# 12334zq/optical-flow-1

Measured on AMD Instinct MI355X. Metric: Mpix*warp-iters/s, TV-L1 1920x1080 5-scale, higher is better.
Workload: dtype f64; 1 GPU; tvl1flow 1920x1080 pair (synthetic P1), nscales=5 warps=5 tau=0.25 lambda=0.15 theta=0.3 zfactor=0.5 epsilon=0.01; one pair per step per GPU; workload_name=1080p, arithmetic_mode=tolerance, pairs_per_gpu=1040, pairs_in_flight_per_gpu=64, lockstep_group=16, streams_per_gpu=4, distinct_pairs=8

## Files before the change

include/ofx.h:

```cpp
#ifndef OFX_H
#define OFX_H

#include <stddef.h>

#ifdef __cplusplus
extern "C" {
#endif

#define OFX_VERSION 102

#define OFX_OK          0
#define OFX_ERR_ARG     1
#define OFX_ERR_SIGMA   2
#define OFX_ERR_NOMEM   3
#define OFX_ERR_HIP     4
#define OFX_ERR_NODEV   5

#define OFX_F64 0
#define OFX_F32 1

#define OFX_TVL1_MAX_ITERATIONS 300
#define OFX_BROX_MAX_ITERATIONS 300
#define OFX_HS_MAX_MAXITER 65536
#define OFX_MAX_SCALES 32
#define OFX_MAX_SOLVES 64

typedef struct ofx_ctx ofx_ctx;

typedef struct ofx_stats {
    int    nscales;
    int    nsolves;
    int    nx[OFX_MAX_SCALES], ny[OFX_MAX_SCALES];
    int    iters[OFX_MAX_SCALES][OFX_MAX_SOLVES];
    double error[OFX_MAX_SCALES][OFX_MAX_SOLVES];
    double iter_ms[OFX_MAX_SCALES];
    long long iter_launches[OFX_MAX_SCALES];
    double work_pix_iters;
    double total_ms;
    int    odd_stops;
    int    odd_stops_stored;
    int    fused[OFX_MAX_SCALES];
    double pyramid_ms;
} ofx_stats;

int  ofx_device_count(void);
int  ofx_ctx_create(ofx_ctx **out, int device, int precision);
void ofx_ctx_destroy(ofx_ctx *ctx);
const char *ofx_strerror(int status);
const char *ofx_last_error(const ofx_ctx *ctx);
void *ofx_ctx_stream(const ofx_ctx *ctx);
int   ofx_ctx_precision(const ofx_ctx *ctx);
int   ofx_ctx_synchronize(ofx_ctx *ctx);
int   ofx_set_option(ofx_ctx *ctx, const char *name, double value);
int   ofx_get_stats(const ofx_ctx *ctx, ofx_stats *out);

int ofx_divergence(ofx_ctx *ctx, const double *v1, const double *v2, double *div, int nx, int ny);
int ofx_forward_gradient(ofx_ctx *ctx, const double *f, double *fx, double *fy, int nx, int ny);
int ofx_centered_gradient(ofx_ctx *ctx, const double *f, double *dx, double *dy, int nx, int ny);
int ofx_dxx(ofx_ctx *ctx, const double *I, double *Ixx, int nx, int ny);
int ofx_dyy(ofx_ctx *ctx, const double *I, double *Iyy, int nx, int ny);
int ofx_dxy(ofx_ctx *ctx, const double *I, double *Ixy, int nx, int ny);
int ofx_gaussian(ofx_ctx *ctx, double *I, int nx, int ny, double sigma);

int ofx_centered_gradient3(ofx_ctx *ctx, const double *f, double *dx, double *dy, double *dz, int nx, int ny, int nz);

int ofx_bicubic_at(ofx_ctx *ctx, const double *input, const double *uu, const double *vv, double *out,
                   int n, int nx, int ny, int border_out);
int ofx_bicubic_warp(ofx_ctx *ctx, const double *input, const double *u, const double *v, double *output,
                     int nx, int ny, int border_out);
int ofx_bicubic_at_color(ofx_ctx *ctx, const double *input, const double *uu, const double *vv, double *out,
                         int n, int nx, int ny, int nz, int k, int border_out);

void ofx_zoom_size(int nx, int ny, int *nxx, int *nyy, double factor);
int  ofx_zoom_out(ofx_ctx *ctx, const double *I, double *Iout, int nx, int ny, double factor);
int  ofx_zoom_in(ofx_ctx *ctx, const double *I, double *Iout, int nx, int ny, int nxx, int nyy);
int  ofx_zoom_out_color(ofx_ctx *ctx, const double *I, double *Iout, int nx, int ny, int nz, double factor);
int  ofx_zoom_out_channels(ofx_ctx *ctx, const double *I, double *Iout, int nx, int ny, int nz, double factor);

int ofx_image_normalization_2(ofx_ctx *ctx, const double *I1, const double *I2, double *I1n, double *I2n,
                              int size);
int ofx_image_normalization_1(ofx_ctx *ctx, const double *I, double *In, int size);
int ofx_getminmax(ofx_ctx *ctx, const double *x, int n, double *min, double *max);

int ofx_tvl1_single_scale(ofx_ctx *ctx, const double *I0, const double *I1, double *u1, double *u2,
                          int nx, int ny, double tau, double lambda, double theta, int warps,
                          double epsilon, int verbose);
int ofx_tvl1_multiscale(ofx_ctx *ctx, const double *I0, const double *I1, double *u1, double *u2,
                        int nx, int ny, double tau, double lambda, double theta, int nscales,
                        double zfactor, int warps, double epsilon, int verbose);

int ofx_tvl1_multiscale_dev(ofx_ctx *ctx, const void *dI0, const void *dI1, void *d_flo,
                            int nx, int ny, double tau, double lambda, double theta, int nscales,
                            double zfactor, int warps, double epsilon, int verbose);

int ofx_tvl1_group_dev(ofx_ctx *ctx, int n_pairs, const void *const *dI0, const void *const *dI1,
                       void *const *d_flo, int nx, int ny, double tau, double lambda, double theta,
                       int nscales, double zfactor, int warps, double epsilon, ofx_stats *stats_out);

int ofx_tvl1_batch_dev(ofx_ctx *const *ctxs, int n_ctx, const void *const *dI0, const void *const *dI1,
                       void *const *d_flo, int n_pairs, int nx, int ny, double tau, double lambda,
                       double theta, int nscales, double zfactor, int warps, double epsilon,
                       double *work_pix_iters);

int ofx_tvl1_batch_group_size(ofx_ctx *const *ctxs, int n_ctx, int n_pairs, int nx, int ny, int nscales,
                              double zfactor);

int ofx_tvl1_iterations(ofx_ctx *ctx, double *u1, double *u2, double *p11, double *p12, double *p21,
                        double *p22, const double *I1wx, const double *I1wy, const double *rho_c,
                        int nx, int ny, double tau, double lambda, double theta, int n_iter,
                        double *error);

int ofx_hypot(ofx_ctx *ctx, const double *x, const double *y, double *out, int n);

int ofx_staging_route(int ctx_device, int mem_device, int can_access_peer);

int ofx_hs_single_scale(ofx_ctx *ctx, const double *I1, const double *I2, double *u, double *v,
                        int nx, int ny, double alpha, int warps, double TOL, int maxiter, int verbose);
int ofx_hs_pyramidal(ofx_ctx *ctx, const double *I1, const double *I2, double *u, double *v,
                     int nx, int ny, double alpha, int nscales, double zfactor, int warps,
                     double TOL, int maxiter, int verbose);

int ofx_hs_group_dev(ofx_ctx *ctx, int n_pairs, const void *const *dI1, const void *const *dI2, void *const *d_flo,
                     int nx, int ny, double alpha, int nscales, double zfactor, int warps, double TOL, int maxiter,
                     ofx_stats *stats_out);
int ofx_hs_batch_dev(ofx_ctx *const *ctxs, int n_ctx, const void *const *dI1, const void *const *dI2,
                     void *const *d_flo, int n_pairs, int nx, int ny, double alpha, int nscales, double zfactor,
                     int warps, double TOL, int maxiter, double *work_pix_iters);

int ofx_hs_classic(ofx_ctx *ctx, const double *a, const double *b, double *u, double *v, int w, int h, int niter,
                   double alpha);

int ofx_brox_spatial(ofx_ctx *ctx, const double *I1, const double *I2, double *u, double *v,
                     int nxx, int nyy, double alpha, double gamma, int nscales, double nu,
                     double TOL, int inner_iter, int outer_iter, int verbose);

int ofx_brox_group_dev(ofx_ctx *ctx, int n_pairs, const void *const *dI1, const void *const *dI2, void *const *d_flo,
                       int nxx, int nyy, double alpha, double gamma, int nscales, double nu, double TOL,
                       int inner_iter, int outer_iter, ofx_stats *stats_out);
int ofx_brox_batch_dev(ofx_ctx *const *ctxs, int n_ctx, const void *const *dI1, const void *const *dI2,
                       void *const *d_flo, int n_pairs, int nxx, int nyy, double alpha, double gamma, int nscales,
                       double nu, double TOL, int inner_iter, int outer_iter, double *work_pix_iters);

#define OFX_REXPO_MAX_CHANNELS 4
int ofx_robust_expo(ofx_ctx *ctx, const double *I1, const double *I2, double *u, double *v, int nxx, int nyy, int nzz,
                    int method_type, double alpha, double gamma, double lambda, int nscales, double nu, double TOL,
                    int inner_iter, int outer_iter, int verbose);
int ofx_robust_expo_pyramid(ofx_ctx *ctx, const double *I1, const double *I2, double *u, double *v, int nxx, int nyy, int nzz,
                            int method_type, double alpha, double gamma, double lambda, int nscales, double nu, double TOL,
                            int inner_iter, int outer_iter, int verbose);
int ofx_robust_expo_group_dev(ofx_ctx *ctx, int n_pairs, const void *const *dI1, const void *const *dI2, void *const *d_flo,
                              int nxx, int nyy, int nzz, int method_type, double alpha, double gamma, double lambda,
                              int nscales, double nu, double TOL, int inner_iter, int outer_iter, ofx_stats *stats_out);
int ofx_robust_expo_batch_dev(ofx_ctx *const *ctxs, int n_ctx, const void *const *dI1, const void *const *dI2,
                              void *const *d_flo, int n_pairs, int nxx, int nyy, int nzz, int method_type, double alpha,
                              double gamma, double lambda, int nscales, double nu, double TOL, int inner_iter, int outer_iter,
                              double *work_pix_iters);
double ofx_ctx_expo_host_ms(const ofx_ctx *ctx);
int ofx_robust_expo_single_scale(ofx_ctx *ctx, const double *I1, const double *I2, double *u, double *v, int nx, int ny, int nz,
                                 int method_type, double alpha, double gamma, double lambda, double TOL, int inner_iter,
                                 int outer_iter, int number_of_threads, int verbose);

int ofx_brox_temporal(ofx_ctx *ctx, const double *I, double *u, double *v, int nxx, int nyy, int frames,
                      double alpha, double gamma, int nscales, double nu, double TOL, int inner_iter,
                      int outer_iter, int verbose);

#define OFX_BROXT_MAX_FRAMES 32
int ofx_brox_temporal_dev(ofx_ctx *ctx, int frames, const void *const *dF, void *const *d_flo, int nxx, int nyy, double alpha,
                          double gamma, int nscales, double nu, double TOL, int inner_iter, int outer_iter);

int ofx_brox_temporal_batch_dev(ofx_ctx *const *ctxs, int n_ctx, int n_seq, int frames, const void *const *dF,
                                void *const *d_flo, int nxx, int nyy, double alpha, double gamma, int nscales, double nu,
                                double TOL, int inner_iter, int outer_iter, double *work_pix_iters);

int ofx_bicubic_warp_color(ofx_ctx *ctx, const double *input, const double *u, const double *v, double *output,
                           int nx, int ny, int nz, int border_out);
int ofx_image_normalization_2_color(ofx_ctx *ctx, const double *I1, const double *I2, double *I1n, double *I2n,
                                    int size, int nz);
int ofx_image_normalization_3(ofx_ctx *ctx, double *I0, double *I1, double *I2, int size);
int ofx_image_normalization_4(ofx_ctx *ctx, const double *I_1, const double *I0, const double *I1, const double *filtI0,
                              double *I_1n, double *I0n, double *I1n, double *filtI0n, int size);

int ofx_me_median_filtering(ofx_ctx *ctx, double *in, int nx, int ny, int wsize);
int ofx_solver_wrt_v(ofx_ctx *ctx, const double *u1, const double *u2, double *v1, double *v2, const double *chi,
                     const double *I1wx, const double *I1wy, const double *I_1wx, const double *I_1wy,
                     const double *rho1_c, const double *rho3_c, double *Vfwd_1, double *Vfwd_2, double *Vbck_1,
                     double *Vbck_2, const double *grad1, const double *grad3, double alpha, double theta, double lambda,
                     int nx, int ny);
int ofx_scalar_rof_box_cell_centered(ofx_ctx *ctx, double *u, const double *f, double *initialP1, double *initialP2,
                                     const double *g_function, double lambda, double omega, int nx, int ny, int nIter);
int ofx_solver_wrt_u(ofx_ctx *ctx, double *u1, double *u2, const double *v1, const double *v2, const double *chi,
                     const double *g, double theta, double beta, int nx, int ny, double *p11, double *p12, double *p21,
                     double *p22, int n_iter);
int ofx_solver_wrt_chi(ofx_ctx *ctx, const double *u1, const double *u2, double *chi, const double *I1wx,
                       const double *I1wy, const double *I_1wx, const double *I_1wy, const double *rho1_c,
                       const double *rho3_c, const double *Vfwd_1, const double *Vfwd_2, const double *Vbck_1,
                       const double *Vbck_2, const double *g, double lambda, double theta, double alpha, double beta,
                       double tau_chi, double tau_eta, int nx, int ny, double *eta1, double *eta2, int n_iter);

int ofx_tvl1occ_multiscale(ofx_ctx *ctx, const double *I_1, const double *I0, const double *I1, const double *filtI0, double *u1,
                           double *u2, double *chi, int nxx, int nyy, double lambda, double alpha, double beta, double theta,
                           int nscales, double zfactor, int warps, double epsilon, int verbose);
int ofx_tvl1occ_batch(ofx_ctx *const *ctxs, int n_ctx, int n_triples, const double *const *I_1, const double *const *I0,
                      const double *const *I1, const double *const *filtI0, double *const *u1, double *const *u2,
                      double *const *chi, int nxx, int nyy, double lambda, double alpha, double beta, double theta, int nscales,
                      double zfactor, int warps, double epsilon);

int ofx_tvl1occ_sequence_group_dev(ofx_ctx *ctx, int n_frames, const void *const *dF, void *const *d_flo,
                                   void *const *d_occ, int nxx, int nyy, double lambda, double alpha, double beta,
                                   double theta, int nscales, double zfactor, int warps, double epsilon,
                                   ofx_stats *stats_out);
int ofx_tvl1occ_sequence_dev(ofx_ctx *const *ctxs, int n_ctx, int n_frames, const void *const *dF, void *const *d_flo,
                             void *const *d_occ, int nxx, int nyy, double lambda, double alpha, double beta, double theta,
                             int nscales, double zfactor, int warps, double epsilon, double *work_pix_iters);

#ifdef __cplusplus
}
#endif
#endif
```

optical-flow-1_amd/__init__.py:

```python
import ctypes as C
import os
import subprocess

import numpy as np

HERE = os.path.dirname(os.path.abspath(__file__))
LIB_PATH = os.environ.get("OFX_LIB_PATH") or os.path.join(HERE, "libofx.so")

F64, F32 = 0, 1
MAX_SCALES, MAX_SOLVES = 32, 64

_STATUS = {1: "invalid argument", 2: "GaussianSmooth: sigma too large", 3: "out of memory",
           4: "HIP runtime error", 5: "no usable gfx950 device"}


class OfxError(RuntimeError):
    def __init__(self, status, detail=""):
        self.status = status
        super().__init__("ofx status %d (%s)%s" % (status, _STATUS.get(status, "?"), ": " + detail if detail else ""))


class Stats(C.Structure):
    _fields_ = [("nscales", C.c_int), ("nsolves", C.c_int),
                ("nx", C.c_int * MAX_SCALES), ("ny", C.c_int * MAX_SCALES),
                ("iters", (C.c_int * MAX_SOLVES) * MAX_SCALES),
                ("error", (C.c_double * MAX_SOLVES) * MAX_SCALES),
                ("iter_ms", C.c_double * MAX_SCALES),
                ("iter_launches", C.c_longlong * MAX_SCALES),
                ("work_pix_iters", C.c_double), ("total_ms", C.c_double),
                ("odd_stops", C.c_int), ("odd_stops_stored", C.c_int), ("fused", C.c_int * MAX_SCALES),
                ("pyramid_ms", C.c_double)]

    def iterations(self):
        return np.array([[self.iters[s][w] for w in range(min(self.nsolves, MAX_SOLVES))]
                         for s in range(self.nscales)])

    def errors(self):
        return np.array([[self.error[s][w] for w in range(min(self.nsolves, MAX_SOLVES))]
                         for s in range(self.nscales)])


def build(verbose=False):
    out = subprocess.run(["make", "-C", os.path.join(HERE, "csrc"), "-j4"], capture_output=True, text=True)
    if verbose or out.returncode:
        print(out.stdout, out.stderr)
    if out.returncode:
        raise RuntimeError("libofx.so build failed")


_lib = None
_dp = np.ctypeslib.ndpointer(dtype=np.float64, flags="C_CONTIGUOUS")
_vp = C.c_void_p
_i, _d = C.c_int, C.c_double


def lib():
    global _lib
    if _lib is not None:
        return _lib
    if not os.path.exists(LIB_PATH):
        raise FileNotFoundError("%s not built -- run `python -c 'import __graft_entry__ as g; g.build()'`" % LIB_PATH)
    L = C.CDLL(LIB_PATH)
    sig = {
        "ofx_device_count": (_i, []),
        "ofx_ctx_create": (_i, [C.POINTER(_vp), _i, _i]),
        "ofx_ctx_destroy": (None, [_vp]),
        "ofx_strerror": (C.c_char_p, [_i]),
        "ofx_last_error": (C.c_char_p, [_vp]),
        "ofx_ctx_stream": (_vp, [_vp]),
        "ofx_ctx_precision": (_i, [_vp]),
        "ofx_ctx_synchronize": (_i, [_vp]),
        "ofx_set_option": (_i, [_vp, C.c_char_p, _d]),
        "ofx_get_stats": (_i, [_vp, C.POINTER(Stats)]),
        "ofx_divergence": (_i, [_vp, _dp, _dp, _dp, _i, _i]),
        "ofx_forward_gradient": (_i, [_vp, _dp, _dp, _dp, _i, _i]),
        "ofx_centered_gradient": (_i, [_vp, _dp, _dp, _dp, _i, _i]),
        "ofx_dxx": (_i, [_vp, _dp, _dp, _i, _i]),
        "ofx_dyy": (_i, [_vp, _dp, _dp, _i, _i]),
        "ofx_dxy": (_i, [_vp, _dp, _dp, _i, _i]),
        "ofx_gaussian": (_i, [_vp, _dp, _i, _i, _d]),
        "ofx_bicubic_at": (_i, [_vp, _dp, _dp, _dp, _dp, _i, _i, _i, _i]),
        "ofx_hypot": (_i, [_vp, _dp, _dp, _dp, _i]),
        "ofx_robust_expo": (_i, [_vp, _dp, _dp, _dp, _dp, _i, _i, _i, _i, _d, _d, _d, _i, _d, _d, _i, _i, _i]),
        "ofx_robust_expo_single_scale": (_i, [_vp, _dp, _dp, _dp, _dp, _i, _i, _i, _i, _d, _d, _d, _d, _i, _i, _i, _i]),
        "ofx_robust_expo_pyramid": (_i, [_vp, _dp, _dp, _dp, _dp, _i, _i, _i, _i, _d, _d, _d, _i, _d, _d, _i, _i, _i]),
        "ofx_bicubic_warp": (_i, [_vp, _dp, _dp, _dp, _dp, _i, _i, _i]),
        "ofx_zoom_size": (None, [_i, _i, C.POINTER(_i), C.POINTER(_i), _d]),
        "ofx_zoom_out": (_i, [_vp, _dp, _dp, _i, _i, _d]),
        "ofx_zoom_in": (_i, [_vp, _dp, _dp, _i, _i, _i, _i]),
        "ofx_image_normalization_2": (_i, [_vp, _dp, _dp, _dp, _dp, _i]),
        "ofx_image_normalization_1": (_i, [_vp, _dp, _dp, _i]),
        "ofx_getminmax": (_i, [_vp, _dp, _i, C.POINTER(_d), C.POINTER(_d)]),
        "ofx_centered_gradient3": (_i, [_vp, _dp, _dp, _dp, _dp, _i, _i, _i]),
        "ofx_bicubic_at_color": (_i, [_vp, _dp, _dp, _dp, _dp, _i, _i, _i, _i, _i, _i]),
        "ofx_zoom_out_color": (_i, [_vp, _dp, _dp, _i, _i, _i, _d]),
        "ofx_zoom_out_channels": (_i, [_vp, _dp, _dp, _i, _i, _i, _d]),
        "ofx_tvl1_single_scale": (_i, [_vp, _dp, _dp, _dp, _dp, _i, _i, _d, _d, _d, _i, _d, _i]),
        "ofx_tvl1_multiscale": (_i, [_vp, _dp, _dp, _dp, _dp, _i, _i, _d, _d, _d, _i, _d, _i, _d, _i]),
        "ofx_tvl1_multiscale_dev": (_i, [_vp, _vp, _vp, _vp, _i, _i, _d, _d, _d, _i, _d, _i, _d, _i]),
        "ofx_tvl1_group_dev": (_i, [_vp, _i, C.POINTER(_vp), C.POINTER(_vp), C.POINTER(_vp), _i, _i, _d, _d, _d, _i, _d, _i, _d,
                                    C.POINTER(Stats)]),
        "ofx_tvl1_batch_dev": (_i, [C.POINTER(_vp), _i, C.POINTER(_vp), C.POINTER(_vp), C.POINTER(_vp), _i, _i, _i, _d, _d, _d,
                                    _i, _d, _i, _d, C.POINTER(_d)]),
        "ofx_tvl1_batch_group_size": (_i, [C.POINTER(_vp), _i, _i, _i, _i, _i, _d]),
        "ofx_tvl1_iterations": (_i, [_vp] + [_dp] * 9 + [_i, _i, _d, _d, _d, _i, C.POINTER(_d)]),
        "ofx_hs_single_scale": (_i, [_vp, _dp, _dp, _dp, _dp, _i, _i, _d, _i, _d, _i, _i]),
        "ofx_hs_pyramidal": (_i, [_vp, _dp, _dp, _dp, _dp, _i, _i, _d, _i, _d, _i, _d, _i, _i]),
        "ofx_brox_spatial": (_i, [_vp, _dp, _dp, _dp, _dp, _i, _i, _d, _d, _i, _d, _d, _i, _i, _i]),
        "ofx_hs_group_dev": (_i, [_vp, _i, C.POINTER(_vp), C.POINTER(_vp), C.POINTER(_vp), _i, _i, _d, _i, _d, _i, _d, _i,
                                  C.POINTER(Stats)]),
        "ofx_hs_batch_dev": (_i, [C.POINTER(_vp), _i, C.POINTER(_vp), C.POINTER(_vp), C.POINTER(_vp), _i, _i, _i, _d, _i, _d,
                                  _i, _d, _i, C.POINTER(_d)]),
        "ofx_brox_group_dev": (_i, [_vp, _i, C.POINTER(_vp), C.POINTER(_vp), C.POINTER(_vp), _i, _i, _d, _d, _i, _d, _d, _i,
                                    _i, C.POINTER(Stats)]),
        "ofx_brox_batch_dev": (_i, [C.POINTER(_vp), _i, C.POINTER(_vp), C.POINTER(_vp), C.POINTER(_vp), _i, _i, _i, _d, _d, _i,
                                    _d, _d, _i, _i, C.POINTER(_d)]),
        "ofx_robust_expo_group_dev": (_i, [_vp, _i, C.POINTER(_vp), C.POINTER(_vp), C.POINTER(_vp), _i, _i, _i, _i, _d, _d, _d, _i,
                                           _d, _d, _i, _i, C.POINTER(Stats)]),
        "ofx_robust_expo_batch_dev": (_i, [C.POINTER(_vp), _i, C.POINTER(_vp), C.POINTER(_vp), C.POINTER(_vp), _i, _i, _i, _i, _i,
                                           _d, _d, _d, _i, _d, _d, _i, _i, C.POINTER(_d)]),
        "ofx_ctx_expo_host_ms": (_d, [_vp]),
        "ofx_bicubic_warp_color": (_i, [_vp, _dp, _dp, _dp, _dp, _i, _i, _i, _i]),
        "ofx_image_normalization_2_color": (_i, [_vp, _dp, _dp, _dp, _dp, _i, _i]),
        "ofx_image_normalization_3": (_i, [_vp, _dp, _dp, _dp, _i]),
        "ofx_image_normalization_4": (_i, [_vp] + [_dp] * 8 + [_i]),
        "ofx_me_median_filtering": (_i, [_vp, _dp, _i, _i, _i]),
        "ofx_solver_wrt_v": (_i, [_vp] + [_dp] * 17 + [_d, _d, _d, _i, _i]),
        "ofx_scalar_rof_box_cell_centered": (_i, [_vp, _dp, _dp, _dp, _dp, _dp, _d, _d, _i, _i, _i]),
        "ofx_solver_wrt_u": (_i, [_vp] + [_dp] * 6 + [_d, _d, _i, _i] + [_dp] * 4 + [_i]),
        "ofx_solver_wrt_chi": (_i, [_vp] + [_dp] * 14 + [_d] * 6 + [_i, _i, _dp, _dp, _i]),
        "ofx_tvl1occ_multiscale": (_i, [_vp] + [_dp] * 7 + [_i, _i, _d, _d, _d, _d, _i, _d, _i, _d, _i]),
        "ofx_tvl1occ_batch": (_i, [_vp, _i, _i] + [_vp] * 7 + [_i, _i, _d, _d, _d, _d, _i, _d, _i, _d]),
        "ofx_tvl1occ_sequence_group_dev": (_i, [_vp, _i, C.POINTER(_vp), C.POINTER(_vp), C.POINTER(_vp), _i, _i, _d, _d, _d, _d, _i, _d,
                                                _i, _d, C.POINTER(Stats)]),
        "ofx_tvl1occ_sequence_dev": (_i, [C.POINTER(_vp), _i, _i, C.POINTER(_vp), C.POINTER(_vp), C.POINTER(_vp), _i, _i, _d, _d, _d,
                                          _d, _i, _d, _i, _d, C.POINTER(_d)]),
        "ofx_hs_classic": (_i, [_vp, _dp, _dp, _dp, _dp, _i, _i, _i, _d]),
        "ofx_brox_temporal": (_i, [_vp, _dp, _dp, _dp, _i, _i, _i, _d, _d, _i, _d, _d, _i, _i, _i]),
        "ofx_brox_temporal_dev": (_i, [_vp, _i, C.POINTER(_vp), C.POINTER(_vp), _i, _i, _d, _d, _i, _d, _d, _i, _i]),
        "ofx_brox_temporal_batch_dev": (_i, [C.POINTER(_vp), _i, _i, _i, C.POINTER(_vp), C.POINTER(_vp), _i, _i, _d, _d, _i, _d, _d,
                                             _i, _i, C.POINTER(_d)]),
    }
    L.ofx_missing = []
    for name, (res, args) in sig.items():
        if not hasattr(L, name):
            L.ofx_missing.append(name)
            continue
        f = getattr(L, name)
        f.restype = res
        f.argtypes = args
    _lib = L
    return L


def zoom_size(nx, ny, factor):
    a, b = _i(), _i()
    lib().ofx_zoom_size(nx, ny, C.byref(a), C.byref(b), factor)
    return a.value, b.value


def _f64(a):
    return np.ascontiguousarray(a, dtype=np.float64)


def tvl1_batch_dev(ctxs, dI0, dI1, d_flo, nx, ny, tau=0.25, lam=0.15, theta=0.3, nscales=5, zfactor=0.5, warps=5,
                   epsilon=0.01):
    n = len(dI0)
    arr = lambda xs: (_vp * len(xs))(*xs)
    work = (_d * max(n, 1))()
    s = lib().ofx_tvl1_batch_dev(arr([c.h.value for c in ctxs]), len(ctxs), arr(dI0), arr(dI1), arr(d_flo), n, nx, ny, tau,
                                 lam, theta, nscales, zfactor, warps, epsilon, work)
    if s:
        raise OfxError(s, "; ".join((c.L.ofx_last_error(c.h) or b"").decode() for c in ctxs))
    return [work[i] for i in range(n)]


def _batch_call(fn, ctxs, dA, dB, d_flo, *args):
    n = len(dA)
    arr = lambda xs: (_vp * max(len(xs), 1))(*xs)
    work = (_d * max(n, 1))()
    s = fn(arr([c.h.value for c in ctxs]), len(ctxs), arr(dA), arr(dB), arr(d_flo), n, *args, work)
    if s:
        raise OfxError(s, "; ".join((c.L.ofx_last_error(c.h) or b"").decode() for c in ctxs))
    return [work[i] for i in range(n)]


def hs_batch_dev(ctxs, dI1, dI2, d_flo, nx, ny, alpha=7.0, nscales=10, zfactor=0.5, warps=10, TOL=1e-4, maxiter=150):
    return _batch_call(lib().ofx_hs_batch_dev, ctxs, dI1, dI2, d_flo, nx, ny, alpha, nscales, zfactor, warps, TOL, maxiter)


def brox_batch_dev(ctxs, dI1, dI2, d_flo, nx, ny, alpha=50.0, gamma=10.0, nscales=10, nu=0.5, TOL=1e-4, inner=1, outer=15):
    return _batch_call(lib().ofx_brox_batch_dev, ctxs, dI1, dI2, d_flo, nx, ny, alpha, gamma, nscales, nu, TOL, inner, outer)


def robust_expo_batch_dev(ctxs, dI1, dI2, d_flo, nx, ny, nz, method=1, alpha=50.0, gamma=10.0, lam=1.0, nscales=5, nu=0.5, TOL=1e-4,
                          inner=1, outer=15):
    return _batch_call(lib().ofx_robust_expo_batch_dev, ctxs, dI1, dI2, d_flo, nx, ny, nz, method, alpha, gamma, lam, nscales, nu,
                       TOL, inner, outer)


def tvl1occ_batch(ctxs, triples, lam=0.15, alpha=0.01, beta=0.15, theta=0.3, nscales=3, zfactor=0.5, warps=2, epsilon=0.01, out=None):
    n = len(triples)
    ny, nx = triples[0][1].shape
    ins = [[_f64(t[k] if k < len(t) else t[1]) for t in triples] for k in range(4)]
    outs = [[o[k] for o in out] for k in range(3)] if out is not None else [[np.empty((ny, nx)) for _ in range(n)] for _ in range(3)]
    ptr = lambda arrs: (_vp * n)(*[a.ctypes.data for a in arrs])
    s = lib().ofx_tvl1occ_batch((_vp * len(ctxs))(*[c.h.value for c in ctxs]), len(ctxs), n, *[ptr(a) for a in ins],
                                *[ptr(a) for a in outs], nx, ny, lam, alpha, beta, theta, nscales, zfactor, warps, epsilon)
    if s:
        raise OfxError(s, "; ".join((c.L.ofx_last_error(c.h) or b"").decode() for c in ctxs))
    return list(zip(*outs))


def tvl1occ_sequence_dev(ctxs, dF, d_flo, d_occ, nx, ny, lam=0.15, alpha=0.01, beta=0.15, theta=0.3, nscales=3, zfactor=0.5, warps=2,
                         epsilon=0.01):
    n = len(dF)
    arr = lambda xs: (_vp * max(len(xs), 1))(*xs)
    work = (_d * max(n - 2, 1))()
    s = lib().ofx_tvl1occ_sequence_dev(arr([c.h.value for c in ctxs]), len(ctxs), n, arr(dF), arr(d_flo), arr(d_occ), nx, ny, lam,
                                       alpha, beta, theta, nscales, zfactor, warps, epsilon, work)
    if s:
        raise OfxError(s, "; ".join((c.L.ofx_last_error(c.h) or b"").decode() for c in ctxs))
    return [work[i] for i in range(max(n - 2, 0))]


def brox_temporal_batch_dev(ctxs, dF, d_flo, nx, ny, frames, alpha=18.0, gamma=7.0, nscales=10, nu=0.75, TOL=1e-4, inner=1, outer=15):
    n_seq = len(dF) // frames if frames > 0 else 0
    arr = lambda xs: (_vp * max(len(xs), 1))(*xs)
    work = (_d * max(n_seq, 1))()
    s = lib().ofx_brox_temporal_batch_dev(arr([c.h.value for c in ctxs]), len(ctxs), n_seq, frames, arr(dF), arr(d_flo), nx, ny,
                                          alpha, gamma, nscales, nu, TOL, inner, outer, work)
    if s:
        raise OfxError(s, "; ".join((c.L.ofx_last_error(c.h) or b"").decode() for c in ctxs))
    return [work[i] for i in range(n_seq)]


def tvl1_batch_group_size(ctxs, n_pairs, nx, ny, nscales=5, zfactor=0.5):
    g = lib().ofx_tvl1_batch_group_size((_vp * len(ctxs))(*[c.h.value for c in ctxs]), len(ctxs), n_pairs, nx, ny, nscales,
                                        zfactor)
    if g < 1:
        raise OfxError(g, "; ".join((c.L.ofx_last_error(c.h) or b"").decode() for c in ctxs))
    return g


class Ofx:

    def __init__(self, device=0, precision=F64):
        self.L = lib()
        h = _vp()
        s = self.L.ofx_ctx_create(C.byref(h), device, precision)
        if s:
            raise OfxError(s, "ofx_ctx_create(device=%d)" % device)
        self.h = h
        self.precision = precision

    def close(self):
        if getattr(self, "h", None):
            self.L.ofx_ctx_destroy(self.h)
            self.h = None

    def __del__(self):
        try:
            self.close()
        except Exception:
            pass

    def _ck(self, s):
        if s:
            raise OfxError(s, (self.L.ofx_last_error(self.h) or b"").decode())

    def set_option(self, name, value):
        self._ck(self.L.ofx_set_option(self.h, name.encode(), float(value)))

    def stats(self):
        st = Stats()
        self._ck(self.L.ofx_get_stats(self.h, C.byref(st)))
        return st

    def stream(self):
        return self.L.ofx_ctx_stream(self.h)

    def synchronize(self):
        self._ck(self.L.ofx_ctx_synchronize(self.h))

    def divergence(self, v1, v2):
        ny, nx = v1.shape
        out = np.empty((ny, nx))
        self._ck(self.L.ofx_divergence(self.h, _f64(v1), _f64(v2), out, nx, ny))
        return out

    def forward_gradient(self, f):
        ny, nx = f.shape
        fx, fy = np.empty((ny, nx)), np.empty((ny, nx))
        self._ck(self.L.ofx_forward_gradient(self.h, _f64(f), fx, fy, nx, ny))
        return fx, fy

    def centered_gradient(self, f):
        ny, nx = f.shape
        fx, fy = np.empty((ny, nx)), np.empty((ny, nx))
        self._ck(self.L.ofx_centered_gradient(self.h, _f64(f), fx, fy, nx, ny))
        return fx, fy

    def _second(self, fn, f):
        ny, nx = f.shape
        out = np.empty((ny, nx))
        self._ck(fn(self.h, _f64(f), out, nx, ny))
        return out

    def dxx(self, f): return self._second(self.L.ofx_dxx, f)
    def dyy(self, f): return self._second(self.L.ofx_dyy, f)
    def dxy(self, f): return self._second(self.L.ofx_dxy, f)

    def gaussian(self, I, sigma):
        ny, nx = I.shape
        out = _f64(I).copy()
        self._ck(self.L.ofx_gaussian(self.h, out, nx, ny, sigma))
        return out

    def bicubic_at(self, I, uu, vv, border_out=False):
        ny, nx = I.shape
        uu, vv = _f64(np.atleast_1d(uu)), _f64(np.atleast_1d(vv))
        out = np.empty(uu.shape)
        self._ck(self.L.ofx_bicubic_at(self.h, _f64(I), uu, vv, out, uu.size, nx, ny, int(border_out)))
        return out

    @staticmethod
    def _colour_shape(I1, I2, nz):
        if I1.shape != I2.shape or I1.ndim not in (2, 3):
            raise ValueError("robust_expo: images of shape %s and %s" % (I1.shape, I2.shape))
        if I1.ndim == 3:
            if nz is not None and nz != I1.shape[2]:
                raise ValueError("robust_expo: nz = %d for images of shape %s" % (nz, I1.shape))
            return I1.shape
        return I1.shape[0], I1.shape[1], (1 if nz is None else nz)

    def robust_expo(self, I1, I2, method=1, alpha=50.0, gamma=10.0, lam=1.0, nscales=5, nu=0.5, TOL=1e-4, inner=1, outer=15,
                    verbose=0, nz=None):
        ny, nx, nz = self._colour_shape(I1, I2, nz)
        if I1.ndim == 2 and nz > 1 and nscales == 1:
            raise ValueError("robust_expo: nz = %d needs (ny, nx, nz) images" % nz)
        u, v = np.zeros((ny, nx)), np.zeros((ny, nx))
        self._ck(self.L.ofx_robust_expo(self.h, _f64(I1), _f64(I2), u, v, nx, ny, nz, method, alpha, gamma, lam, nscales, nu, TOL,
                                        inner, outer, verbose))
        return u, v

    def robust_expo_pyramid(self, I1, I2, method=1, alpha=50.0, gamma=10.0, lam=1.0, nscales=5, nu=0.5, TOL=1e-4, inner=1, outer=15,
                            verbose=0, nz=None):
        ny, nx, nz = self._colour_shape(I1, I2, nz)
        if I1.ndim == 2 and nz != 1:
            raise ValueError("robust_expo_pyramid: nz = %d needs (ny, nx, nz) images" % nz)
        u, v = np.zeros((ny, nx)), np.zeros((ny, nx))
        self._ck(self.L.ofx_robust_expo_pyramid(self.h, _f64(I1), _f64(I2), u, v, nx, ny, nz, method, alpha, gamma, lam, nscales, nu,
                                                TOL, inner, outer, verbose))
        return u, v

    def robust_expo_single_scale(self, I1, I2, u, v, method=1, alpha=50.0, gamma=10.0, lam=1.0, TOL=1e-4, inner=1, outer=15,
                                 verbose=0, nz=None):
        ny, nx, nz = self._colour_shape(I1, I2, nz)
        if I1.ndim == 2 and nz != 1:
            raise ValueError("robust_expo_single_scale: nz = %d needs (ny, nx, nz) images" % nz)
        u, v = np.array(u, dtype=np.float64, order="C"), np.array(v, dtype=np.float64, order="C")
        if u.shape != (ny, nx) or v.shape != (ny, nx):
            raise ValueError("robust_expo_single_scale: flow of shape %s, %s for %dx%d images" % (u.shape, v.shape, nx, ny))
        self._ck(self.L.ofx_robust_expo_single_scale(self.h, _f64(I1), _f64(I2), u, v, nx, ny, nz, method, alpha, gamma, lam, TOL,
                                                     inner, outer, 1, verbose))
        return u, v

    def hypot(self, x, y):
        x, y = _f64(np.atleast_1d(x)).ravel(), _f64(np.atleast_1d(y)).ravel()
        out = np.empty(x.shape)
        self._ck(self.L.ofx_hypot(self.h, x, y, out, x.size))
        return out

    def bicubic_warp(self, I, u, v, border_out=False):
        ny, nx = I.shape
        out = np.empty((ny, nx))
        self._ck(self.L.ofx_bicubic_warp(self.h, _f64(I), _f64(u), _f64(v), out, nx, ny, int(border_out)))
        return out

    def zoom_out(self, I, factor):
        ny, nx = I.shape
        nxx, nyy = zoom_size(nx, ny, factor)
        out = np.empty((nyy, nxx))
        self._ck(self.L.ofx_zoom_out(self.h, _f64(I), out, nx, ny, factor))
        return out

    def zoom_in(self, I, nxx, nyy):
        ny, nx = I.shape
        out = np.empty((nyy, nxx))
        self._ck(self.L.ofx_zoom_in(self.h, _f64(I), out, nx, ny, nxx, nyy))
        return out

    def image_normalization_2(self, I1, I2):
        a, b = np.empty(I1.shape), np.empty(I2.shape)
        self._ck(self.L.ofx_image_normalization_2(self.h, _f64(I1), _f64(I2), a, b, I1.size))
        return a, b

    def tvl1_single_scale(self, I0, I1, u1, u2, tau=0.25, lam=0.15, theta=0.3, warps=5, epsilon=0.01, verbose=0):
        ny, nx = I0.shape
        u1, u2 = _f64(u1).copy(), _f64(u2).copy()
        self._ck(self.L.ofx_tvl1_single_scale(self.h, _f64(I0), _f64(I1), u1, u2, nx, ny, tau, lam, theta, warps,
                                              epsilon, verbose))
        return u1, u2

    def tvl1_multiscale(self, I0, I1, tau=0.25, lam=0.15, theta=0.3, nscales=5, zfactor=0.5, warps=5, epsilon=0.01,
                        verbose=0, out=None):
        ny, nx = I0.shape
        u1, u2 = out if out is not None else (np.zeros((ny, nx)), np.zeros((ny, nx)))
        self._ck(self.L.ofx_tvl1_multiscale(self.h, _f64(I0), _f64(I1), u1, u2, nx, ny, tau, lam, theta, nscales,
                                            zfactor, warps, epsilon, verbose))
        return u1, u2

    def tvl1_multiscale_dev(self, dI0, dI1, d_flo, nx, ny, tau=0.25, lam=0.15, theta=0.3, nscales=5, zfactor=0.5,
                            warps=5, epsilon=0.01, verbose=0):
        self._ck(self.L.ofx_tvl1_multiscale_dev(self.h, dI0, dI1, d_flo, nx, ny, tau, lam, theta, nscales, zfactor,
                                                warps, epsilon, verbose))

    def tvl1_group_dev(self, dI0, dI1, d_flo, nx, ny, tau=0.25, lam=0.15, theta=0.3, nscales=5, zfactor=0.5, warps=5,
                       epsilon=0.01):
        n = len(dI0)
        arr = lambda xs: (_vp * len(xs))(*xs)
        st = (Stats * max(n, 1))()
        self._ck(self.L.ofx_tvl1_group_dev(self.h, n, arr(dI0), arr(dI1), arr(d_flo), nx, ny, tau, lam, theta, nscales,
                                           zfactor, warps, epsilon, st))
        return [st[i] for i in range(n)]

    def _group_call(self, fn, dA, dB, d_flo, *args):
        n = len(dA)
        arr = lambda xs: (_vp * max(len(xs), 1))(*xs)
        st = (Stats * max(n, 1))()
        self._ck(fn(self.h, n, arr(dA), arr(dB), arr(d_flo), *args, st))
        return [st[i] for i in range(n)]

    def hs_group_dev(self, dI1, dI2, d_flo, nx, ny, alpha=7.0, nscales=10, zfactor=0.5, warps=10, TOL=1e-4, maxiter=150):
        return self._group_call(self.L.ofx_hs_group_dev, dI1, dI2, d_flo, nx, ny, alpha, nscales, zfactor, warps, TOL, maxiter)

    def brox_group_dev(self, dI1, dI2, d_flo, nx, ny, alpha=50.0, gamma=10.0, nscales=10, nu=0.5, TOL=1e-4, inner=1, outer=15):
        return self._group_call(self.L.ofx_brox_group_dev, dI1, dI2, d_flo, nx, ny, alpha, gamma, nscales, nu, TOL, inner, outer)

    def robust_expo_group_dev(self, dI1, dI2, d_flo, nx, ny, nz, method=1, alpha=50.0, gamma=10.0, lam=1.0, nscales=5, nu=0.5,
                              TOL=1e-4, inner=1, outer=15):
        return self._group_call(self.L.ofx_robust_expo_group_dev, dI1, dI2, d_flo, nx, ny, nz, method, alpha, gamma, lam, nscales,
                                nu, TOL, inner, outer)

    def expo_host_ms(self):
        return self.L.ofx_ctx_expo_host_ms(self.h)

    def tvl1_iterations(self, u1, u2, p11, p12, p21, p22, I1wx, I1wy, rho_c, tau, lam, theta, n_iter):
        ny, nx = u1.shape
        err = _d()
        self._ck(self.L.ofx_tvl1_iterations(self.h, u1, u2, p11, p12, p21, p22, _f64(I1wx), _f64(I1wy), _f64(rho_c),
                                            nx, ny, tau, lam, theta, n_iter, C.byref(err)))
        return err.value

    def hs_single_scale(self, I1, I2, u, v, alpha=7.0, warps=10, TOL=1e-4, maxiter=150, verbose=0):
        ny, nx = I1.shape
        u, v = _f64(u).copy(), _f64(v).copy()
        self._ck(self.L.ofx_hs_single_scale(self.h, _f64(I1), _f64(I2), u, v, nx, ny, alpha, warps, TOL, maxiter, verbose))
        return u, v

    def hs_pyramidal(self, I1, I2, alpha=7.0, nscales=10, zfactor=0.5, warps=10, TOL=1e-4, maxiter=150, verbose=0, out=None):
        ny, nx = I1.shape
        u, v = out if out is not None else (np.zeros((ny, nx)), np.zeros((ny, nx)))
        self._ck(self.L.ofx_hs_pyramidal(self.h, _f64(I1), _f64(I2), u, v, nx, ny, alpha, nscales, zfactor, warps, TOL,
                                         maxiter, verbose))
        return u, v

    def brox_spatial(self, I1, I2, alpha=50.0, gamma=10.0, nscales=10, nu=0.5, TOL=1e-4, inner=1, outer=15, verbose=0, out=None):
        ny, nx = I1.shape
        u, v = out if out is not None else (np.zeros((ny, nx)), np.zeros((ny, nx)))
        self._ck(self.L.ofx_brox_spatial(self.h, _f64(I1), _f64(I2), u, v, nx, ny, alpha, gamma, nscales, nu, TOL,
                                         inner, outer, verbose))
        return u, v

    def brox_temporal(self, I, alpha=18.0, gamma=7.0, nscales=10, nu=0.75, TOL=1e-4, inner=1, outer=15, verbose=0):
        frames, ny, nx = I.shape
        u, v = np.zeros((max(frames - 1, 0), ny, nx)), np.zeros((max(frames - 1, 0), ny, nx))
        self._ck(self.L.ofx_brox_temporal(self.h, _f64(I), u, v, nx, ny, frames, alpha, gamma, nscales, nu, TOL, inner,
                                          outer, verbose))
        return u, v

    def brox_temporal_dev(self, dF, d_flo, nx, ny, alpha=18.0, gamma=7.0, nscales=10, nu=0.75, TOL=1e-4, inner=1, outer=15):
        arr = lambda xs: (_vp * max(len(xs), 1))(*xs)
        self._ck(self.L.ofx_brox_temporal_dev(self.h, len(dF), arr(dF), arr(d_flo), nx, ny, alpha, gamma, nscales, nu, TOL, inner,
                                              outer))

    def centered_gradient3(self, f):
        nz, ny, nx = f.shape
        dx, dy, dz = np.empty((nz, ny, nx)), np.empty((nz, ny, nx)), np.empty((nz, ny, nx))
        self._ck(self.L.ofx_centered_gradient3(self.h, _f64(f), dx, dy, dz, nx, ny, nz))
        return dx, dy, dz

    def bicubic_at_color(self, I, uu, vv, k, border_out=False):
        ny, nx, nz = I.shape
        uu, vv = _f64(np.atleast_1d(uu)), _f64(np.atleast_1d(vv))
        out = np.empty(uu.shape)
        self._ck(self.L.ofx_bicubic_at_color(self.h, _f64(I), uu, vv, out, uu.size, nx, ny, nz, k, int(border_out)))
        return out

    def zoom_out_color(self, I, factor):
        ny, nx, nz = I.shape
        nxx, nyy = zoom_size(nx, ny, factor)
        out = np.empty((nyy, nxx, nz))
        self._ck(self.L.ofx_zoom_out_color(self.h, _f64(I), out, nx, ny, nz, factor))
        return out

    def zoom_out_channels(self, I, factor):
        ny, nx, nz = I.shape
        nxx, nyy = zoom_size(nx, ny, factor)
        out = np.empty((nyy, nxx, nz))
        self._ck(self.L.ofx_zoom_out_channels(self.h, _f64(I), out, nx, ny, nz, factor))
        return out

    def image_normalization_1(self, I):
        out = np.empty(I.shape)
        self._ck(self.L.ofx_image_normalization_1(self.h, _f64(I), out, I.size))
        return out

    def getminmax(self, x):
        a, b = _d(), _d()
        self._ck(self.L.ofx_getminmax(self.h, _f64(x), x.size, C.byref(a), C.byref(b)))
        return a.value, b.value

    def hs_classic(self, a, b, niter, alpha):
        h, w = a.shape
        u, v = np.zeros((h, w)), np.zeros((h, w))
        self._ck(self.L.ofx_hs_classic(self.h, _f64(a), _f64(b), u, v, w, h, niter, alpha))
        return u, v

    def bicubic_warp_color(self, I, u, v, border_out=False):
        ny, nx, nz = I.shape
        out = np.empty((ny, nx, nz))
        self._ck(self.L.ofx_bicubic_warp_color(self.h, _f64(I), _f64(u), _f64(v), out, nx, ny, nz, int(border_out)))
        return out

    def image_normalization_2_color(self, I1, I2, size=None):
        nz = I1.shape[-1]
        a, b = _f64(I1).copy(), _f64(I2).copy()
        self._ck(self.L.ofx_image_normalization_2_color(self.h, _f64(I1), _f64(I2), a, b, I1.size if size is None else size, nz))
        return a, b

    def image_normalization_3(self, I0, I1, I2):
        a, b, c = _f64(I0).copy(), _f64(I1).copy(), _f64(I2).copy()
        self._ck(self.L.ofx_image_normalization_3(self.h, a, b, c, a.size))
        return a, b, c

    def image_normalization_4(self, I_1, I0, I1, F):
        outs = [np.empty(I0.shape) for _ in range(4)]
        self._ck(self.L.ofx_image_normalization_4(self.h, _f64(I_1), _f64(I0), _f64(I1), _f64(F), *outs, I0.size))
        return outs

    def median_filtering(self, I, wsize=3):
        ny, nx = I.shape
        out = _f64(I).copy()
        self._ck(self.L.ofx_me_median_filtering(self.h, out, nx, ny, wsize))
        return out

    def occ_solver_v(self, u1, u2, chi, I1wx, I1wy, I_1wx, I_1wy, rho1_c, rho3_c, grad1, grad3, alpha, theta, lam):
        ny, nx = u1.shape
        v1, v2, f1, f2, b1, b2 = outs = [np.empty((ny, nx)) for _ in range(6)]
        self._ck(self.L.ofx_solver_wrt_v(self.h, _f64(u1), _f64(u2), v1, v2, _f64(chi), _f64(I1wx), _f64(I1wy), _f64(I_1wx),
                                         _f64(I_1wy), _f64(rho1_c), _f64(rho3_c), f1, f2, b1, b2, _f64(grad1), _f64(grad3),
                                         alpha, theta, lam, nx, ny))
        return outs

    def occ_solver_chi(self, u1, u2, chi, I1wx, I1wy, I_1wx, I_1wy, rho1_c, rho3_c, Vf1, Vf2, Vb1, Vb2, g, lam, theta, alpha,
                       beta, tau_chi, tau_eta, eta1=None, eta2=None, n_iter=100):
        ny, nx = u1.shape
        chi = _f64(chi).copy()
        eta1 = np.zeros((ny, nx)) if eta1 is None else _f64(eta1).copy()
        eta2 = np.zeros((ny, nx)) if eta2 is None else _f64(eta2).copy()
        self._ck(self.L.ofx_solver_wrt_chi(self.h, _f64(u1), _f64(u2), chi, _f64(I1wx), _f64(I1wy), _f64(I_1wx), _f64(I_1wy),
                                           _f64(rho1_c), _f64(rho3_c), _f64(Vf1), _f64(Vf2), _f64(Vb1), _f64(Vb2), _f64(g), lam,
                                           theta, alpha, beta, tau_chi, tau_eta, nx, ny, eta1, eta2, n_iter))
        return chi, eta1, eta2

    def rof_box(self, u, f, P1, P2, g, lam, omega, n_iter):
        ny, nx = u.shape
        u, P1, P2 = _f64(u).copy(), _f64(P1).copy(), _f64(P2).copy()
        self._ck(self.L.ofx_scalar_rof_box_cell_centered(self.h, u, _f64(f), P1, P2, _f64(g), lam, omega, nx, ny, n_iter))
        return u, P1, P2

    def tvl1occ_multiscale(self, I_1, I0, I1, filtI0=None, lam=0.15, alpha=0.01, beta=0.15, theta=0.3, nscales=3, zfactor=0.5,
                           warps=2, epsilon=0.01, verbose=0, out=None):
        ny, nx = I0.shape
        filtI0 = I0 if filtI0 is None else filtI0
        u1, u2, chi = out if out is not None else (np.empty((ny, nx)), np.empty((ny, nx)), np.empty((ny, nx)))
        self._ck(self.L.ofx_tvl1occ_multiscale(self.h, _f64(I_1), _f64(I0), _f64(I1), _f64(filtI0), u1, u2, chi, nx, ny, lam, alpha,
                                               beta, theta, nscales, zfactor, warps, epsilon, verbose))
        return u1, u2, chi

    def tvl1occ_sequence_group_dev(self, dF, d_flo, d_occ, nx, ny, lam=0.15, alpha=0.01, beta=0.15, theta=0.3, nscales=3, zfactor=0.5,
                                   warps=2, epsilon=0.01):
        n = len(dF)
        arr = lambda xs: (_vp * max(len(xs), 1))(*xs)
        st = (Stats * max(n - 2, 1))()
        self._ck(self.L.ofx_tvl1occ_sequence_group_dev(self.h, n, arr(dF), arr(d_flo), arr(d_occ), nx, ny, lam, alpha, beta, theta,
                                                       nscales, zfactor, warps, epsilon, st))
        return [st[i] for i in range(max(n - 2, 0))]

    def occ_solver_u(self, v1, v2, chi, g, theta, beta, p=None, n_iter=10):
        ny, nx = v1.shape
        u1, u2 = np.empty((ny, nx)), np.empty((ny, nx))
        p = [np.zeros((ny, nx)) for _ in range(4)] if p is None else [_f64(a).copy() for a in p]
        self._ck(self.L.ofx_solver_wrt_u(self.h, u1, u2, _f64(v1), _f64(v2), _f64(chi), _f64(g), theta, beta, nx, ny, *p, n_iter))
        return u1, u2, p
```

optical-flow-1_amd/csrc/ofx_ctx.cpp:

```cpp
#include "ofx_internal.h"

#include <cstdarg>
#include <cstdlib>
#include <new>

static const size_t kSlabAlign = 256;
static const size_t kMinSlab = 32u << 20;
static const size_t kMaxSlabs = 24;

int ofx_fail(ofx_ctx *ctx, int status, const char *fmt, ...)
{
    if (ctx) {
        va_list ap;
        va_start(ap, fmt);
        vsnprintf(ctx->errmsg, sizeof(ctx->errmsg), fmt, ap);
        va_end(ap);
    }
    return status;
}

extern "C" const char *ofx_strerror(int status)
{
    switch (status) {
    case OFX_OK:        return "ok";
    case OFX_ERR_ARG:   return "invalid argument";
    case OFX_ERR_SIGMA: return "GaussianSmooth: sigma too large";
    case OFX_ERR_NOMEM: return "out of memory";
    case OFX_ERR_HIP:   return "HIP runtime error";
    case OFX_ERR_NODEV: return "no usable gfx950 device";
    default:            return "unknown status";
    }
}

extern "C" const char *ofx_last_error(const ofx_ctx *ctx) { return ctx ? ctx->errmsg : ""; }

extern "C" int ofx_device_count(void)
{
    int n = 0;
    if (hipGetDeviceCount(&n) != hipSuccess) return 0;
    return n;
}

extern "C" void ofx_ctx_destroy(ofx_ctx *ctx);

extern "C" int ofx_ctx_create(ofx_ctx **out, int device, int precision)
{
    if (!out) return OFX_ERR_ARG;
    *out = nullptr;
    if (precision != OFX_F64 && precision != OFX_F32) return OFX_ERR_ARG;
    const bool trace = getenv("OFX_TRACE_INIT") != nullptr;
    double t_prev = ofx_now_ms();
    auto mark = [&](const char *what) {
        if (!trace) return;
        const double t = ofx_now_ms();
        fprintf(stderr, "ofx_ctx_create: %-28s %8.2f ms\n", what, t - t_prev);
        t_prev = t;
    };
    int n = 0;
    if (hipGetDeviceCount(&n) != hipSuccess || n <= 0 || device < 0 || device >= n) return OFX_ERR_NODEV;
    mark("hipGetDeviceCount (runtime)");
    if (hipSetDevice(device) != hipSuccess) return OFX_ERR_NODEV;
    mark("hipSetDevice");

    ofx_ctx *ctx = new (std::nothrow) ofx_ctx();
    if (!ctx) return OFX_ERR_NOMEM;
    ctx->device = device;
    ctx->precision = precision;
    ctx->cur_slab = 0;
    ctx->cur_used = 0;
    ctx->call_bytes = 0;
    ctx->profile = 0;
    ctx->rows_per_wave = 0;
    ctx->rows_per_wave2 = 0;
    ctx->fuse2 = 1;
    ctx->store_a = 1;
    ctx->concurrency = 1;
    ctx->lockstep = 0;
    ctx->warp_lds = 1;
    ctx->gauss_fused = 1;
    ctx->relaxed_dual = 0;
    ctx->tile = 0;
    ctx->tile_max_px = 0;
    ctx->nt_stores = 0;
    ctx->chunk = 0;
    ctx->spin_us = 150;
    ctx->rows_slots = 0;
    ctx->rof_pipe = 1;
    ctx->rof_window = 0;
    ctx->chi_fuse = 1;
    ctx->fuse3 = 2;
    ctx->fuse3_min_px = 0.0;
    ctx->fuse3_cursor = 1;
    ctx->fuse3_afac1 = 0;
    ctx->fuse3_afac2 = 0;
    ctx->rows_per_wave3 = 0;
    ctx->rows3_max = 32;
    ctx->fixed_work = 0;
    ctx->sor_exact = 1;
    ctx->sor_batch = 0;
    ctx->sor_fuse = 0;
    ctx->sor_tile = 0;
    ctx->sor_tile_w = 0;
    ctx->sor_wave_levels = 1;
    ctx->sor_wave_p = 0;
    ctx->sor_window = 0;
    ctx->sor_rows = 0;
    ctx->sor_spw = 0;
    ctx->sor_lds = 1;
    ctx->mem_budget = 0;
    ctx->poll_seq = 0;
    ctx->errmsg[0] = 0;
    ctx->expo_host_ms = 0.0;
    memset(&ctx->stats, 0, sizeof(ctx->stats));

    ctx->stream = nullptr;
    ctx->d_err = nullptr;
    ctx->d_state = nullptr;
    ctx->h_state = nullptr;
    ctx->h_aux = nullptr;
    ctx->ev_t0 = ctx->ev_t1 = nullptr;
    for (int i = 0; i < OFX_NPOLL; i++) ctx->ev_poll[i] = nullptr;
    bool ok = hipStreamCreateWithFlags(&ctx->stream, hipStreamNonBlocking) == hipSuccess;
    mark("hipStreamCreate");
    static_assert(sizeof(OfxLoopDev) <= OFX_STATE_BYTES && OFX_STATE_BYTES % 512 == 0, "state block too small");
    static_assert(OFX_ULOG >= OFX_TVL1_MAX_ITERATIONS + 16, "unit log too short");
    ok = ok && hipMalloc((void **) &ctx->d_state, OFX_STATE_BYTES + sizeof(double) * OFX_TVL1_MAX_ITERATIONS * OFX_NSHARD) == hipSuccess;
    if (ok) ctx->d_err = reinterpret_cast<double *>(reinterpret_cast<char *>(ctx->d_state) + OFX_STATE_BYTES);
    ctx->d_err_cap = OFX_TVL1_MAX_ITERATIONS;
    mark("hipMalloc (loop state)");
    ok = ok && hipHostMalloc((void **) &ctx->h_state, sizeof(OfxIterState) * OFX_NPOLL * OFX_MAX_GROUP + sizeof(double) * OFX_MAX_GROUP,
                             hipHostMallocDefault) == hipSuccess;
    if (ok) {
        memset(ctx->h_state, 0, sizeof(OfxIterState) * OFX_NPOLL * OFX_MAX_GROUP + sizeof(double) * OFX_MAX_GROUP);
        ctx->h_aux = reinterpret_cast<double *>(ctx->h_state + OFX_NPOLL * OFX_MAX_GROUP);
    }
    mark("hipHostMalloc (poll ring)");
    for (int i = 0; ok && i < OFX_NPOLL; i++)
        ok = hipEventCreateWithFlags(&ctx->ev_poll[i], hipEventDisableTiming) == hipSuccess;
    ok = ok && hipEventCreate(&ctx->ev_t0) == hipSuccess && hipEventCreate(&ctx->ev_t1) == hipSuccess;
    mark("hipEventCreate x 6");
    if (!ok) {
        (void) hipGetLastError();
        ofx_ctx_destroy(ctx);
        return OFX_ERR_HIP;
    }
    *out = ctx;
    return OFX_OK;
}

extern "C" void ofx_ctx_destroy(ofx_ctx *ctx)
{
    if (!ctx) return;
    (void) hipSetDevice(ctx->device);
    if (ctx->stream) (void) hipStreamSynchronize(ctx->stream);
    for (auto &s : ctx->slabs) (void) hipFree(s.base);
    if (ctx->d_state) (void) hipFree(ctx->d_state);
    if (ctx->h_state) (void) hipHostFree(ctx->h_state);
    for (int i = 0; i < OFX_NPOLL; i++)
        if (ctx->ev_poll[i]) (void) hipEventDestroy(ctx->ev_poll[i]);
    if (ctx->ev_t0) (void) hipEventDestroy(ctx->ev_t0);
    if (ctx->ev_t1) (void) hipEventDestroy(ctx->ev_t1);
    if (ctx->stream) (void) hipStreamDestroy(ctx->stream);
    (void) hipGetLastError();
    delete ctx;
}

extern "C" void *ofx_ctx_stream(const ofx_ctx *ctx) { return ctx ? (void *) ctx->stream : nullptr; }
extern "C" int ofx_ctx_precision(const ofx_ctx *ctx) { return ctx ? ctx->precision : -1; }

extern "C" int ofx_ctx_synchronize(ofx_ctx *ctx)
{
    if (!ctx) return OFX_ERR_ARG;
    OFX_HIP(ctx, hipStreamSynchronize(ctx->stream));
    return OFX_OK;
}

extern "C" int ofx_set_option(ofx_ctx *ctx, const char *name, double value)
{
    if (!ctx || !name) return OFX_ERR_ARG;
    if (!strcmp(name, "profile")) { ctx->profile = value != 0; return OFX_OK; }
    if (!strcmp(name, "fixed_work")) { ctx->fixed_work = value != 0; return OFX_OK; }
    if (!strcmp(name, "rows_per_wave")) {
        if (value < 0 || value > 4096) return ofx_fail(ctx, OFX_ERR_ARG, "rows_per_wave out of range");
        ctx->rows_per_wave = (int) value;
        return OFX_OK;
    }
    if (!strcmp(name, "rows_per_wave2")) {
        if (value < 0 || value > 4096) return ofx_fail(ctx, OFX_ERR_ARG, "rows_per_wave2 out of range");
        ctx->rows_per_wave2 = (int) value;
        return OFX_OK;
    }
    if (!strcmp(name, "concurrency")) {
        if (value < 1 || value > 64) return ofx_fail(ctx, OFX_ERR_ARG, "concurrency out of range");
        ctx->concurrency = (int) value;
        return OFX_OK;
    }
    if (!strcmp(name, "tile")) {
        if (value != 0 && value != 4 && value != 6) return ofx_fail(ctx, OFX_ERR_ARG, "tile must be 0, 4 or 6");
        ctx->tile = (int) value;
        return OFX_OK;
    }
    if (!strcmp(name, "tile_max_px")) {
        if (value < 0) return ofx_fail(ctx, OFX_ERR_ARG, "tile_max_px out of range");
        ctx->tile_max_px = value;
        return OFX_OK;
    }
    if (!strcmp(name, "relaxed_dual")) { ctx->relaxed_dual = value != 0; return OFX_OK; }
    if (!strcmp(name, "gauss_fused")) { ctx->gauss_fused = (value == 2 || value == 3) ? (int) value : (value != 0); return OFX_OK; }
    if (!strcmp(name, "warp_lds")) { ctx->warp_lds = value != 0; return OFX_OK; }
    if (!strcmp(name, "nt_stores")) { ctx->nt_stores = (int) value; return (value >= 0 && value <= 2) ? OFX_OK : ofx_fail(ctx, OFX_ERR_ARG, "nt_stores = 0 | 1 | 2"); }
    if (!strcmp(name, "lockstep")) {
        if (value < 0 || value > OFX_MAX_GROUP) return ofx_fail(ctx, OFX_ERR_ARG, "lockstep out of range");
        ctx->lockstep = (int) value;
        return OFX_OK;
    }
    if (!strcmp(name, "sor_exact")) {
        if (value != 0 && value != 1 && value != 2) return ofx_fail(ctx, OFX_ERR_ARG, "sor_exact must be 0, 1 or 2");
        ctx->sor_exact = (int) value;
        return OFX_OK;
    }
    if (!strcmp(name, "sor_fuse")) {
        if ((value < -1 || value > 4) && value != 9) return ofx_fail(ctx, OFX_ERR_ARG, "sor_fuse must be -1 .. 4 (or 9)");
        ctx->sor_fuse = (int) value;
        return OFX_OK;
    }
    if (!strcmp(name, "sor_tile")) {
        if (value < 0 || value > 3) return ofx_fail(ctx, OFX_ERR_ARG, "sor_tile must be 0 .. 3");
        ctx->sor_tile = (int) value;
        return OFX_OK;
    }
    if (!strcmp(name, "sor_tile_w")) {
        if (value < 0 || value > 65536) return ofx_fail(ctx, OFX_ERR_ARG, "sor_tile_w out of range");
        ctx->sor_tile_w = (int) value;
        return OFX_OK;
    }
    if (!strcmp(name, "sor_wave_p")) {
        if (value < 0 || value > 8) return ofx_fail(ctx, OFX_ERR_ARG, "sor_wave_p out of range");
        ctx->sor_wave_p = (int) value;
        return OFX_OK;
    }
    if (!strcmp(name, "sor_wave_levels")) {
        if (value < 0 || value > 64) return ofx_fail(ctx, OFX_ERR_ARG, "sor_wave_levels out of range");
        ctx->sor_wave_levels = (int) value;
        return OFX_OK;
    }
    if (!strcmp(name, "sor_rows")) {
        if (value < 0 || value > 4096) return ofx_fail(ctx, OFX_ERR_ARG, "sor_rows out of range");
        ctx->sor_rows = (int) value;
        return OFX_OK;
    }
    if (!strcmp(name, "sor_lds")) {
        if (value != 0 && value != 1 && value != 2) return ofx_fail(ctx, OFX_ERR_ARG, "sor_lds must be 0, 1 or 2");
        ctx->sor_lds = (int) value;
        return OFX_OK;
    }
    if (!strcmp(name, "sor_spw")) {
        if (value != 0 && value != 1 && value != 2 && value != 4) return ofx_fail(ctx, OFX_ERR_ARG, "sor_spw must be 0, 1, 2 or 4");
        ctx->sor_spw = (int) value;
        return OFX_OK;
    }
    if (!strcmp(name, "sor_window")) {
        if (value < 0 || value > 4096) return ofx_fail(ctx, OFX_ERR_ARG, "sor_window out of range");
        ctx->sor_window = (int) value;
        return OFX_OK;
    }
    if (!strcmp(name, "sor_batch")) {
        if (value < 0 || value > 4096) return ofx_fail(ctx, OFX_ERR_ARG, "sor_batch out of range");
        ctx->sor_batch = (int) value;
        return OFX_OK;
    }
    if (!strcmp(name, "mem_budget")) {
        if (value < 0) return ofx_fail(ctx, OFX_ERR_ARG, "mem_budget out of range");
        ctx->mem_budget = value;
        return OFX_OK;
    }
    if (!strcmp(name, "fuse2")) { ctx->fuse2 = value != 0; return OFX_OK; }
    if (!strcmp(name, "store_a")) {
        if (value != 0 && value != 1 && value != 2) return ofx_fail(ctx, OFX_ERR_ARG, "store_a must be 0, 1 or 2");
        ctx->store_a = (int) value;
        return OFX_OK;
    }
    if (!strcmp(name, "rows_slots")) { ctx->rows_slots = (int) value; return OFX_OK; }
    if (!strcmp(name, "rof_pipe")) { ctx->rof_pipe = value != 0; return OFX_OK; }
    if (!strcmp(name, "rof_window")) {
        if (value != 0 && value != 24 && value != 10) return ofx_fail(ctx, OFX_ERR_ARG, "rof_window must be 0, 10 or 24");
        ctx->rof_window = (int) value;
        return OFX_OK;
    }
    if (!strcmp(name, "chi_fuse")) { ctx->chi_fuse = value != 0; return OFX_OK; }
    if (!strcmp(name, "fuse3")) {
        if (value != 0 && value != 1 && value != 2) return ofx_fail(ctx, OFX_ERR_ARG, "fuse3 must be 0, 1 or 2");
        ctx->fuse3 = (int) value;
        return OFX_OK;
    }
    if (!strcmp(name, "fuse3_min_px")) { ctx->fuse3_min_px = value; return OFX_OK; }
    if (!strcmp(name, "fuse3_cursor")) { ctx->fuse3_cursor = value != 0; return OFX_OK; }
    if (!strcmp(name, "fuse3_afac1")) { ctx->fuse3_afac1 = value; return value >= 0 ? OFX_OK : ofx_fail(ctx, OFX_ERR_ARG, "fuse3_afac1 < 0"); }
    if (!strcmp(name, "fuse3_afac2")) { ctx->fuse3_afac2 = value; return value >= 0 ? OFX_OK : ofx_fail(ctx, OFX_ERR_ARG, "fuse3_afac2 < 0"); }
    if (!strcmp(name, "rows_per_wave3")) { ctx->rows_per_wave3 = (int) value; return OFX_OK; }
    if (!strcmp(name, "rows3_max")) { ctx->rows3_max = (int) value; return OFX_OK; }
    if (!strcmp(name, "spin_us")) {
        if (value < 0 || value > 1e6) return ofx_fail(ctx, OFX_ERR_ARG, "spin_us out of range");
        ctx->spin_us = (int) value;
        return OFX_OK;
    }
    if (!strcmp(name, "chunk")) {
        if (value < 0 || value > OFX_TVL1_MAX_ITERATIONS) return ofx_fail(ctx, OFX_ERR_ARG, "chunk out of range");
        ctx->chunk = (int) value;
        return OFX_OK;
    }
    return ofx_fail(ctx, OFX_ERR_ARG, "unknown option '%s'", name);
}

extern "C" int ofx_get_stats(const ofx_ctx *ctx, ofx_stats *out)
{
    if (!ctx || !out) return OFX_ERR_ARG;
    *out = ctx->stats;
    return OFX_OK;
}

void ofx_arena_reset(ofx_ctx *ctx)
{
    if (ctx->slabs.size() > kMaxSlabs) {
        size_t total = 0;
        for (auto &s : ctx->slabs) { total += s.bytes; (void) hipFree(s.base); }
        ctx->slabs.clear();
        char *p = nullptr;
        if (hipMalloc((void **) &p, total) == hipSuccess) ctx->slabs.push_back({p, total});
        else (void) hipGetLastError();
    }
    ctx->cur_slab = 0;
    ctx->cur_used = 0;
    ctx->call_bytes = 0;
}

int ofx_arena_alloc(ofx_ctx *ctx, size_t bytes, void **out)
{
    static const long skew = getenv("OFX_ARENA_SKEW") ? atol(getenv("OFX_ARENA_SKEW")) : 0;
    bytes += (size_t) skew;
    bytes = (bytes + kSlabAlign - 1) / kSlabAlign * kSlabAlign;
    if (bytes == 0) bytes = kSlabAlign;
    while (ctx->cur_slab < ctx->slabs.size()) {
        OfxSlab &s = ctx->slabs[ctx->cur_slab];
        if (ctx->cur_used + bytes <= s.bytes) {
            *out = s.base + ctx->cur_used;
            ctx->cur_used += bytes;
            ctx->call_bytes += bytes;
            return OFX_OK;
        }
        ctx->cur_slab++;
        ctx->cur_used = 0;
    }
    size_t want = bytes > kMinSlab ? bytes : kMinSlab;
    if (want < ctx->call_bytes) want = ctx->call_bytes;
    char *p = nullptr;
    hipError_t e = hipMalloc((void **) &p, want);
    if (e != hipSuccess) {
        (void) hipGetLastError();
        return ofx_fail(ctx, OFX_ERR_NOMEM, "hipMalloc(%zu) failed: %s", want, hipGetErrorString(e));
    }
    ctx->slabs.push_back({p, want});
    ctx->cur_slab = ctx->slabs.size() - 1;
    ctx->cur_used = bytes;
    ctx->call_bytes += bytes;
    *out = p;
    return OFX_OK;
}
```

optical-flow-1_amd/csrc/ofx_internal.h:

```cpp
#pragma once

#include <hip/hip_runtime.h>

#include <cstddef>
#include <cstdint>
#include <cstdio>
#include <cstring>
#include <chrono>
#include <vector>

#include "ofx.h"

#define OFX_NSHARD 64
#define OFX_NPOLL  4
#define OFX_MAX_GROUP 16

struct OfxIterState {
    int    n;
    int    done;
    double error;
    int    apred;
    int    seq;
    int    unit, k0, ucnt;
};

#define OFX_ULOG 320
struct OfxLoopDev {
    OfxIterState st[OFX_MAX_GROUP];
    int cursor[2][OFX_MAX_GROUP];
    int scanned[OFX_MAX_GROUP];
    int ulog[OFX_MAX_GROUP][OFX_ULOG];
};

#define OFX_STATE_BYTES 22016

struct OfxSlab {
    char  *base;
    size_t bytes;
};

struct ofx_ctx {
    int device;
    int precision;
    hipStream_t stream;

    std::vector<OfxSlab> slabs;
    size_t cur_slab;
    size_t cur_used;
    size_t call_bytes;

    double       *d_err;
    int           d_err_cap;
    OfxIterState *d_state;
    OfxIterState *h_state;
    double       *h_aux;
    hipEvent_t    ev_poll[OFX_NPOLL];
    hipEvent_t    ev_t0, ev_t1;

    int profile;
    int rows_per_wave;
    int rows_per_wave2;
    int fuse2;
    int store_a;
    int concurrency;
    int lockstep;
    int nt_stores;
    int relaxed_dual;
    int tile;
    double tile_max_px;
    int gauss_fused;
    int warp_lds;
    int chunk;
    int fuse3;
    double fuse3_min_px;
    int fuse3_cursor;
    double fuse3_afac1, fuse3_afac2;
    int rows_per_wave3;
    int rows3_max;
    int chi_fuse;
    int rof_window;
    int rof_pipe;
    int rows_slots;
    int spin_us;
    int fixed_work;
    int sor_exact;
    int sor_fuse;
    int sor_tile;
    int sor_tile_w;
    int sor_wave_p;
    int sor_wave_levels;
    int sor_batch;
    int sor_window;
    int sor_rows;
    int sor_lds;
    int sor_spw;
    double mem_budget;
    unsigned long long poll_seq;

    ofx_stats stats;
    double expo_host_ms;
    char errmsg[256];
};

int ofx_fail(ofx_ctx *ctx, int status, const char *fmt, ...);

#define OFX_HIP(ctx, call)                                                                       \
    do {                                                                                         \
        hipError_t e__ = (call);                                                                 \
        if (e__ != hipSuccess)                                                                   \
            return ofx_fail((ctx), e__ == hipErrorOutOfMemory ? OFX_ERR_NOMEM : OFX_ERR_HIP,     \
                            "%s failed: %s (%s:%d)", #call, hipGetErrorString(e__), __FILE__,   \
                            __LINE__);                                                           \
    } while (0)

#define OFX_TRY(expr)                                                                            \
    do {                                                                                         \
        int s__ = (expr);                                                                        \
        if (s__ != OFX_OK) return s__;                                                           \
    } while (0)

void ofx_arena_reset(ofx_ctx *ctx);
int  ofx_arena_alloc(ofx_ctx *ctx, size_t bytes, void **out);

template <typename T>
static inline int ofx_alloc(ofx_ctx *ctx, size_t count, T **out)
{
    void *p = nullptr;
    int s = ofx_arena_alloc(ctx, count * sizeof(T), &p);
    *out = static_cast<T *>(p);
    return s;
}

template <typename T> struct Pix;
template <> struct Pix<double> { using v2 = double2; using v4 = double4; };
template <> struct Pix<float>  { using v2 = float2;  using v4 = float4;  };

static inline int ofx_cdiv(int a, int b) { return (a + b - 1) / b; }

#define OFX_ENTER(ctx)                                                                           \
    do {                                                                                         \
        if (!(ctx)) return OFX_ERR_ARG;                                                          \
        if (hipSetDevice((ctx)->device) != hipSuccess)                                           \
            return ofx_fail((ctx), OFX_ERR_NODEV, "hipSetDevice(%d) failed", (ctx)->device);     \
        (ctx)->errmsg[0] = 0;                                                                    \
        (ctx)->expo_host_ms = 0.0;                                                               \
        ofx_arena_reset(ctx);                                                                    \
    } while (0)

static inline double ofx_now_ms()
{
    using namespace std::chrono;
    return duration<double, std::milli>(steady_clock::now().time_since_epoch()).count();
}
```

optical-flow-1_amd/csrc/ofx_tvl1.hip:

```cpp
#include "ofx_ops.h"
#include "ofx_device.h"
#include "ofx_loop.h"

#include <atomic>
#include <chrono>
#include <cmath>
#include <thread>

#define TVL1_GRAD_IS_ZERO 1E-10
#define TVL1_PRESMOOTHING_SIGMA 0.8
#define STRIP_OUT 62

template <typename T> OFX_DEV double rnd_to(double x);
template <> OFX_DEV double rnd_to<double>(double x) { return x; }
template <> OFX_DEV double rnd_to<float>(double x) { return (double) (float) x; }

#ifdef OFX_NO_RFL
#define OFX_WAVE_UNIFORM(x) (x)
#else
#define OFX_WAVE_UNIFORM(x) __builtin_amdgcn_readfirstlane(x)
#endif
template <typename T> struct RowIn {
    double2 u, p1, p2, a;
    double r;
};

template <typename V> OFX_DEV const V *at(const V *base, unsigned byte_off)
{
    return reinterpret_cast<const V *>(reinterpret_cast<const char *>(base) + byte_off);
}
template <typename V> OFX_DEV V *at(V *base, unsigned byte_off)
{
    return reinterpret_cast<V *>(reinterpret_cast<char *>(base) + byte_off);
}

template <typename T>
OFX_DEV RowIn<T> tvl1_load_row(const typename Pix<T>::v2 *U, const typename Pix<T>::v2 *P1,
                               const typename Pix<T>::v2 *P2, const typename Pix<T>::v2 *A, const T *R, unsigned off2)
{
    RowIn<T> r;
    r.u = ldw2(at(U, off2));
    r.p1 = ldw2(at(P1, off2));
    r.p2 = ldw2(at(P2, off2));
    r.a = ldw2(at(A, off2));
    r.r = ldw(at(R, off2 >> 1));
    return r;
}

#ifndef OFX_TOL_NEWTON
#define OFX_TOL_NEWTON 1
#endif
OFX_DEV double sqrt_tol(double x)
{
#if OFX_TOL_NEWTON >= 2
    return sqrt_unscaled(x);
#else
    const double y = __builtin_amdgcn_rsq(x);
    const double g = x * y;
    const double h = y * 0.5;
    const double r = __builtin_fma(-h, g, 0.5);
    return __builtin_fma(g, r, g);
#endif
}
OFX_DEV double rcp_tol(double d)
{
#if OFX_TOL_NEWTON >= 2
    return rcp_newton(d);
#else
    const double r = __builtin_amdgcn_rcp(d);
    const double e = __builtin_fma(-d, r, 1.0);
    return __builtin_fma(r, e, r);
#endif
}

template <typename T, bool STRICT = true>
OFX_DEV double2 tvl1_primal(double2 u, double2 a, double r, double2 p1, double2 p2, double l11, double l21, double up12,
                            double up22, bool lef, bool rig, bool top, bool bot, double l_t, double theta)
{
#ifdef OFX_CEIL_MEM
    return make_double2(u.x + 1e-300 * (a.x + r + p1.x + l11 + up12), u.y + 1e-300 * (a.y + p2.x + p1.y + p2.y + l21 + up22));
#endif
    const double div1 = div_backward(p1.x, l11, p1.y, up12, lef, rig, top, bot);
    const double div2 = div_backward(p2.x, l21, p2.y, up22, lef, rig, top, bot);
    const double ix = a.x, iy = a.y;
    const double grad = ix * ix + iy * iy;
    const double rho = r + (ix * u.x + iy * u.y);
    const double ltg = l_t * grad;
    const double fi = STRICT ? -rho / grad : -rho * rcp_tol(grad);
    double d1, d2;
    if (rho < -ltg)                     { d1 = l_t * ix;  d2 = l_t * iy; }
    else if (rho > ltg)                 { d1 = -l_t * ix; d2 = -l_t * iy; }
    else if (grad < TVL1_GRAD_IS_ZERO)  { d1 = 0.0;       d2 = 0.0; }
    else                                { d1 = fi * ix;   d2 = fi * iy; }
    const double v1 = u.x + d1, v2 = u.y + d2;
    return make_double2(rnd_to<T>(v1 + theta * div1), rnd_to<T>(v2 + theta * div2));
}

#ifdef OFX_DIV_SHARED
OFX_DEV double rcp_refined(double d)
{
    double r = __builtin_amdgcn_rcp(d);
    double e = __builtin_fma(-d, r, 1.0);
    r = __builtin_fma(r, e, r);
    e = __builtin_fma(-d, r, 1.0);
    r = __builtin_fma(r, e, r);
    return r;
}
OFX_DEV double div_by_rcp(double n, double d, double r)
{
    double q = n * r;
    const double rem = __builtin_fma(-d, q, n);
    q = __builtin_fma(rem, r, q);
    return __builtin_amdgcn_div_fixup(q, d, n);
}
#endif

template <typename T, bool STRICT>
OFX_DEV void tvl1_dual(double2 p1, double2 p2, double2 un, double r1, double r2, double2 dn, bool rig, bool lastrow,
                       double taut, double2 &q1, double2 &q2)
{
#ifdef OFX_CEIL_MEM
    q1 = make_double2(p1.x + 1e-300 * (un.x + r1), p1.y + 1e-300 * dn.x);
    q2 = make_double2(p2.x + 1e-300 * (un.y + r2), p2.y + 1e-300 * dn.y);
    return;
#endif
    const double u1x = rig ? 0.0 : r1 - un.x;
    const double u2x = rig ? 0.0 : r2 - un.y;
    const double u1y = lastrow ? 0.0 : dn.x - un.x;
    const double u2y = lastrow ? 0.0 : dn.y - un.y;
    if (STRICT) {
        const double g1 = hypot_ref(u1x, u1y);
        const double g2 = hypot_ref(u2x, u2y);
        const double ng1 = 1.0 + taut * g1;
        const double ng2 = 1.0 + taut * g2;
#ifdef OFX_DIV_SHARED
        const double n1x = p1.x + taut * u1x, n1y = p1.y + taut * u1y, n2x = p2.x + taut * u2x, n2y = p2.y + taut * u2y;
        const double r1 = rcp_refined(ng1), r2 = rcp_refined(ng2);
        q1.x = div_by_rcp(n1x, ng1, r1);
        q1.y = div_by_rcp(n1y, ng1, r1);
        q2.x = div_by_rcp(n2x, ng2, r2);
        q2.y = div_by_rcp(n2y, ng2, r2);
        const double lo = fmin(fmin(fabs(q1.x), fabs(q1.y)), fmin(fabs(q2.x), fabs(q2.y)));
        const double hi = fmax(fmax(fabs(q1.x), fabs(q1.y)), fmax(fabs(q2.x), fabs(q2.y)));
        bool ok = lo >= 0x1p-900 && hi <= 0x1p600 && fmax(ng1, ng2) <= 0x1p50;
        if (!__all(ok)) {
            ok = fmax(ng1, ng2) <= 0x1p50 && hi <= 0x1p600 && (n1x == 0.0 || fabs(q1.x) >= 0x1p-900) &&
                 (n1y == 0.0 || fabs(q1.y) >= 0x1p-900) && (n2x == 0.0 || fabs(q2.x) >= 0x1p-900) &&
                 (n2y == 0.0 || fabs(q2.y) >= 0x1p-900);
            if (!__all(ok)) {
                q1.x = n1x / ng1;
                q1.y = n1y / ng1;
                q2.x = n2x / ng2;
                q2.y = n2y / ng2;
            }
        }
#else
        q1.x = (p1.x + taut * u1x) / ng1;
        q1.y = (p1.y + taut * u1y) / ng1;
        q2.x = (p2.x + taut * u2x) / ng2;
        q2.y = (p2.y + taut * u2y) / ng2;
#endif
    } else {
        const double g1 = sqrt_tol(fmax(u1x * u1x + u1y * u1y, 0x1p-600));
        const double g2 = sqrt_tol(fmax(u2x * u2x + u2y * u2y, 0x1p-600));
        const double i1 = rcp_tol(1.0 + taut * g1);
        const double i2 = rcp_tol(1.0 + taut * g2);
        q1.x = (p1.x + taut * u1x) * i1;
        q1.y = (p1.y + taut * u1y) * i1;
        q2.x = (p2.x + taut * u2x) * i2;
        q2.y = (p2.y + taut * u2y) * i2;
    }
}

OFX_DEV bool tvl1_continues(double prev1, double prev2, int k, int size, double eps2, double &e1)
{
    e1 = 0.0;
    if (k >= 1) {
        e1 = loop_error_from_sum(wave_allreduce_sum(prev1), size, OFX_CRIT_MEAN);
        if (!(e1 > eps2)) return false;
    }
    if (k >= 2 && !(loop_error_from_sum(wave_allreduce_sum(prev2), size, OFX_CRIT_MEAN) > eps2)) return false;
    return true;
}
OFX_DEV bool tvl1_store_a(int k, double e1, double eps2, double afac) { return afac > 0.0 && k >= 1 && e1 <= eps2 * afac; }

template <typename V> struct Tri {
    V *b0, *b1, *b2;
};
template <typename V> struct TriSel {
    const V *in;
    V       *out, *alt;
};
template <typename V> OFX_DEV TriSel<V> pick3(const Tri<V> &t, unsigned code, int g, size_t n)
{
    const unsigned i = (code >> (2 * g)) & 3u;
    TriSel<V> r;
    r.in = (i == 0 ? t.b0 : (i == 1 ? t.b1 : t.b2)) + (size_t) g * n;
    r.out = (i == 0 ? t.b1 : (i == 1 ? t.b2 : t.b0)) + (size_t) g * n;
    r.alt = (i == 0 ? t.b2 : (i == 1 ? t.b0 : t.b1)) + (size_t) g * n;
    return r;
}

#ifdef OFX_ITER1_WAVES
#define OFX_ITER1_ATTR __attribute__((amdgpu_waves_per_eu(OFX_ITER1_WAVES, OFX_ITER1_WAVES)))
#else
#define OFX_ITER1_ATTR
#endif
template <typename T, bool STRICT>
__global__ __launch_bounds__(256) OFX_ITER1_ATTR void k_tvl1_iter(
    Tri<typename Pix<T>::v2> Ut, Tri<typename Pix<T>::v2> P1t, Tri<typename Pix<T>::v2> P2t,
    const typename Pix<T>::v2 *__restrict__ Ag, const T *__restrict__ Rg, double *__restrict__ errg, int check, int slot,
    int nx, int ny, int rows, int strips_x, int strips_pad, double l_t, double theta, double taut, double eps2,
    unsigned incode, unsigned runmask, int err_stride)
{
    using v2 = typename Pix<T>::v2;
    const int lane = threadIdx.x & 63;
    const int gw = OFX_WAVE_UNIFORM((int) (blockIdx.x * 4 + (threadIdx.x >> 6)));
    const int g = blockIdx.y;
    if (!((runmask >> g) & 1u)) return;
    const size_t npix = (size_t) nx * ny;
    const TriSel<v2> hu = pick3(Ut, incode, g, npix), h1 = pick3(P1t, incode, g, npix), h2 = pick3(P2t, incode, g, npix);
    const v2 *__restrict__ Uin = hu.in, *__restrict__ P1in = h1.in, *__restrict__ P2in = h2.in;
    v2 *__restrict__ Uout = hu.out, *__restrict__ P1out = h1.out, *__restrict__ P2out = h2.out;
    const v2 *__restrict__ A = Ag + (size_t) g * npix;
    const T *__restrict__ R = Rg + (size_t) g * npix;
    double *__restrict__ err = errg + (size_t) g * err_stride;

    const double prev1 = loop_fetch_prev(err, check), prev2 = loop_fetch_prev(err, check - 1);

    const int strip = gw % strips_pad, band = gw / strips_pad;
    const int y0 = band * rows;
    const bool idle = (strip >= strips_x) || (y0 >= ny);
    const int yend = (y0 + rows < ny) ? y0 + rows : ny;

    const int c = strip * STRIP_OUT - 1 + lane;
    const int cc = c < 0 ? 0 : (c > nx - 1 ? nx - 1 : c);
    const bool lef = (c == 0), rig = (c == nx - 1);
    const bool owner = (lane >= 1) && (lane <= STRIP_OUT) && (c < nx);

    const unsigned E2 = 2 * sizeof(T);
    const unsigned row2 = (unsigned) nx * E2;
    unsigned off = ((unsigned) y0 * nx + cc) * E2;
    const unsigned offs = ((unsigned) y0 * nx + (c < 0 ? 0 : c)) * E2;
    unsigned so = offs;

    double up12 = 0.0, up22 = 0.0;
    RowIn<T> cur;
    if (!idle) {
        if (y0 > 0) {
            up12 = ldw2(at(P1in, off - row2)).y;
            up22 = ldw2(at(P2in, off - row2)).y;
        }
        cur = tvl1_load_row<T>(Uin, P1in, P2in, A, R, off);
    }

    double e1;
    if (!tvl1_continues(prev1, prev2, check, nx * ny, eps2, e1)) return;
    if (idle) return;

    const unsigned level_bytes = (unsigned) nx * (unsigned) ny * E2;
    const ofx_rsrc rU = make_rsrc(Uout, level_bytes), rP1 = make_rsrc(P1out, level_bytes), rP2 = make_rsrc(P2out, level_bytes);
    double acc = 0.0;
    double2 un_prev = make_double2(0.0, 0.0);
    double2 p1_prev = make_double2(0.0, 0.0), p2_prev = make_double2(0.0, 0.0);

    for (int y = y0; y <= yend; y++) {
        RowIn<T> nxt = cur;
        if (y + 1 <= yend && y + 1 < ny) nxt = tvl1_load_row<T>(Uin, P1in, P2in, A, R, off + row2);

        double2 un = make_double2(0.0, 0.0);
        unsigned st_u = OFX_OOB, st_p = OFX_OOB;
        if (y < ny) {
            const double l11 = wave_shift_up(cur.p1.x);
            const double l21 = wave_shift_up(cur.p2.x);
            un = tvl1_primal<T, STRICT>(cur.u, cur.a, cur.r, cur.p1, cur.p2, l11, l21, up12, up22, lef, rig, y == 0, y == ny - 1,
                                        l_t, theta);
            if (owner && y < yend) {
                st_u = so;
                acc += (un.x - cur.u.x) * (un.x - cur.u.x) + (un.y - cur.u.y) * (un.y - cur.u.y);
            }
        }
        double2 q1 = make_double2(0.0, 0.0), q2 = q1;
        if (y > y0) {
            const double r1 = wave_shift_down(un_prev.x);
            const double r2 = wave_shift_down(un_prev.y);
            tvl1_dual<T, STRICT>(p1_prev, p2_prev, un_prev, r1, r2, un, rig, y - 1 == ny - 1, taut, q1, q2);
            if (owner) st_p = so - row2;
        }
        bst2<false>(rU, st_u, un, Uout);
        bst2<false>(rP1, st_p, q1, P1out);
        bst2<false>(rP2, st_p, q2, P2out);
        un_prev = un;
        p1_prev = cur.p1;
        p2_prev = cur.p2;
        up12 = cur.p1.y;
        up22 = cur.p2.y;
        cur = nxt;
        off += row2;
        so += row2;
    }
    loop_accumulate(err, slot, acc, gw);
}

#ifndef STRIP2_OUT
#define STRIP2_OUT 60
#endif
#define STRIP2_HALO ((64 - STRIP2_OUT) / 2)
#ifndef OFX_ITER2_WAVES
#define OFX_ITER2_WAVES 3
#endif
#if OFX_ITER2_WAVES >= 4
#define OFX_ITER2_BOUNDS __launch_bounds__(256, 4)
#else
#define OFX_ITER2_BOUNDS __launch_bounds__(256)
#endif
template <typename T, bool NT, bool SA, bool STRICT>
OFX_DEV void tvl1_iter2_march(const typename Pix<T>::v2 *__restrict__ Uin, const typename Pix<T>::v2 *__restrict__ P1in,
                              const typename Pix<T>::v2 *__restrict__ P2in, const typename Pix<T>::v2 *__restrict__ A,
                              const T *__restrict__ R, typename Pix<T>::v2 *Uout, typename Pix<T>::v2 *P1out,
                              typename Pix<T>::v2 *P2out, typename Pix<T>::v2 *Ualt, typename Pix<T>::v2 *P1alt,
                              typename Pix<T>::v2 *P2alt, double *__restrict__ err, int k, int gw, int nx, int ny, int y0,
                              int yend, int ys, int yl, bool lef, bool rig, bool owner, unsigned off, unsigned so,
                              double up12, double up22, RowIn<T> cur, double l_t, double theta, double taut)
{
    const unsigned E2 = 2 * sizeof(T);
    const unsigned row2 = (unsigned) nx * E2;
#ifdef OFX_CEIL_ALU
    const unsigned off0 = off;
#endif
    const double2 z2 = make_double2(0.0, 0.0);
    const unsigned level_bytes = (unsigned) nx * (unsigned) ny * E2;
    const ofx_rsrc rU = make_rsrc(Uout, level_bytes), rP1 = make_rsrc(P1out, level_bytes), rP2 = make_rsrc(P2out, level_bytes);
    const ofx_rsrc rUa = make_rsrc(Ualt, level_bytes), rP1a = make_rsrc(P1alt, level_bytes), rP2a = make_rsrc(P2alt, level_bytes);
    double accA = 0.0, accB = 0.0;
    double2 uA0 = z2, uA1 = z2, uA2 = z2;
    double2 a1 = z2, a2 = z2;
    double r1c = 0.0, r2c = 0.0;
    double2 p0a = z2, p0b = z2;
    double2 pA1a = z2, pA1b = z2, pA2a = z2, pA2b = z2;
    double2 uB0 = z2, uB1 = z2;

    for (int y = ys; y <= yend + 2; y++) {
        RowIn<T> nxt = cur;
#ifdef OFX_CEIL_ALU
        if (y + 1 <= yl) nxt = tvl1_load_row<T>(Uin, P1in, P2in, A, R, off0 + (((unsigned) (y + 1 - ys)) & 1u) * row2);
#else
        if (y + 1 <= yl) nxt = tvl1_load_row<T>(Uin, P1in, P2in, A, R, off + row2);
#endif

        const bool have1 = (y <= yl);
        unsigned sa1 = OFX_OOB, sa2 = OFX_OOB;
        if (have1) {
            const double l11 = wave_shift_up(cur.p1.x);
            const double l21 = wave_shift_up(cur.p2.x);
            uA0 = tvl1_primal<T, STRICT>(cur.u, cur.a, cur.r, cur.p1, cur.p2, l11, l21, up12, up22, lef, rig, y == 0,
                                         y == ny - 1, l_t, theta);
            if (owner && y >= y0 && y < yend) {
                accA += (uA0.x - cur.u.x) * (uA0.x - cur.u.x) + (uA0.y - cur.u.y) * (uA0.y - cur.u.y);
                sa1 = so;
            }
        }
        double2 pAna = z2, pAnb = z2;
        if (y - 1 >= ys && y - 1 <= yend && y - 1 <= ny - 1) {
            const double n1 = wave_shift_down(uA1.x);
            const double n2 = wave_shift_down(uA1.y);
            tvl1_dual<T, STRICT>(p0a, p0b, uA1, n1, n2, uA0, rig, y - 1 == ny - 1, taut, pAna, pAnb);
            pAna.x = rnd_to<T>(pAna.x); pAna.y = rnd_to<T>(pAna.y);
            pAnb.x = rnd_to<T>(pAnb.x); pAnb.y = rnd_to<T>(pAnb.y);
            if (owner && y - 1 >= y0 && y - 1 < yend) sa2 = so - row2;
        }
        unsigned st3 = OFX_OOB, st4 = OFX_OOB;
        if (y - 2 >= y0 && y - 2 <= yend && y - 2 <= ny - 1) {
            const double l11 = wave_shift_up(pA1a.x);
            const double l21 = wave_shift_up(pA1b.x);
            uB0 = tvl1_primal<T, STRICT>(uA2, a2, r2c, pA1a, pA1b, l11, l21, pA2a.y, pA2b.y, lef, rig, y - 2 == 0,
                                         y - 2 == ny - 1, l_t, theta);
            if (owner && y - 2 < yend) {
                st3 = so - 2 * row2;
                accB += (uB0.x - uA2.x) * (uB0.x - uA2.x) + (uB0.y - uA2.y) * (uB0.y - uA2.y);
            }
        }
        double2 q1 = z2, q2 = z2;
        if (y - 3 >= y0 && y - 3 < yend) {
            const double n1 = wave_shift_down(uB1.x);
            const double n2 = wave_shift_down(uB1.y);
            tvl1_dual<T, STRICT>(pA2a, pA2b, uB1, n1, n2, uB0, rig, y - 3 == ny - 1, taut, q1, q2);
            if (owner) st4 = so - 3 * row2;
        }
#ifdef OFX_CEIL_ALU
        st3 = OFX_OOB; st4 = OFX_OOB;
#endif
        bst2<NT>(rU, st3, uB0, Uout);
        bst2<NT>(rP1, st4, q1, P1out);
        bst2<NT>(rP2, st4, q2, P2out);
        if (SA) {
            bst2<NT>(rUa, sa1, uA0, Ualt);
            bst2<NT>(rP1a, sa2, pAna, P1alt);
            bst2<NT>(rP2a, sa2, pAnb, P2alt);
        }
        uA2 = uA1; uA1 = uA0;
        a2 = a1; a1 = cur.a;
        r2c = r1c; r1c = cur.r;
        p0a = cur.p1; p0b = cur.p2;
        up12 = cur.p1.y; up22 = cur.p2.y;
        pA2a = pA1a; pA2b = pA1b; pA1a = pAna; pA1b = pAnb;
        uB1 = uB0;
        cur = nxt;
        off += row2;
        so += row2;
    }
    loop_accumulate(err, k, accA, gw);
    loop_accumulate(err, k + 1, accB, gw);
}

template <typename T, bool NT, bool STRICT>
__global__ OFX_ITER2_BOUNDS void k_tvl1_iter2(
    Tri<typename Pix<T>::v2> Ut, Tri<typename Pix<T>::v2> P1t, Tri<typename Pix<T>::v2> P2t,
    const typename Pix<T>::v2 *__restrict__ Ag, const T *__restrict__ Rg, double *__restrict__ errg, int k, int nx, int ny,
    int rows, int strips_x, int strips_pad, double l_t, double theta, double taut, double eps2, unsigned incode,
    unsigned amask, double afac, int err_stride)
{
    using v2 = typename Pix<T>::v2;
    const int lane = threadIdx.x & 63;
    const int gw = OFX_WAVE_UNIFORM((int) (blockIdx.x * 4 + (threadIdx.x >> 6)));
    const int g = blockIdx.y;
    const size_t npix = (size_t) nx * ny;
    const TriSel<v2> hu = pick3(Ut, incode, g, npix), h1 = pick3(P1t, incode, g, npix), h2 = pick3(P2t, incode, g, npix);
    const v2 *__restrict__ Uin = hu.in, *__restrict__ P1in = h1.in, *__restrict__ P2in = h2.in;
    const v2 *__restrict__ A = Ag + (size_t) g * npix;
    const T *__restrict__ R = Rg + (size_t) g * npix;
    double *__restrict__ err = errg + (size_t) g * err_stride;
    const double prev1 = loop_fetch_prev(err, k), prev2 = loop_fetch_prev(err, k - 1);

    const int band = gw / strips_pad;
#ifdef OFX_XCD_ROT
    const int strip = (gw % strips_pad + 4 * OFX_XCD_ROT * band) % strips_pad;
#else
    const int strip = gw % strips_pad;
#endif
    const int y0 = band * rows;
    const bool idle = (strip >= strips_x) || (y0 >= ny);
    const int yend = (y0 + rows < ny) ? y0 + rows : ny;
    const int ys = y0 > 0 ? y0 - 1 : 0;
    const int yl = (yend + 1 < ny - 1) ? yend + 1 : ny - 1;

    const int c = strip * STRIP2_OUT - STRIP2_HALO + lane;
    const int cc = c < 0 ? 0 : (c > nx - 1 ? nx - 1 : c);
    const bool lef = (c == 0), rig = (c == nx - 1);
    const bool owner = (lane >= STRIP2_HALO) && (lane < STRIP2_OUT + STRIP2_HALO) && (c < nx);

    const unsigned E2 = 2 * sizeof(T);
    const unsigned row2 = (unsigned) nx * E2;
    const unsigned off = ((unsigned) ys * nx + cc) * E2;
    const unsigned so = ((unsigned) ys * nx + (c < 0 ? 0 : c)) * E2;

    double up12 = 0.0, up22 = 0.0;
    RowIn<T> cur;
    if (!idle) {
        if (ys > 0) {
            up12 = ldw2(at(P1in, off - row2)).y;
            up22 = ldw2(at(P2in, off - row2)).y;
        }
        cur = tvl1_load_row<T>(Uin, P1in, P2in, A, R, off);
    }
    double e1;
    if (!tvl1_continues(prev1, prev2, k, nx * ny, eps2, e1)) return;
    if (idle) return;
    if (((amask >> g) & 1u) || tvl1_store_a(k, e1, eps2, afac))
        tvl1_iter2_march<T, NT, true, STRICT>(Uin, P1in, P2in, A, R, hu.out, h1.out, h2.out, hu.alt, h1.alt, h2.alt, err, k, gw, nx, ny,
                                      y0, yend, ys, yl, lef, rig, owner, off, so, up12, up22, cur, l_t, theta, taut);
    else
        tvl1_iter2_march<T, NT, false, STRICT>(Uin, P1in, P2in, A, R, hu.out, h1.out, h2.out, hu.alt, h1.alt, h2.alt, err, k, gw, nx, ny,
                                       y0, yend, ys, yl, lef, rig, owner, off, so, up12, up22, cur, l_t, theta, taut);
}

#ifndef STRIP3_OUT
#define STRIP3_OUT 56
#endif
#define STRIP3_HALO ((64 - STRIP3_OUT) / 2)
#ifndef OFX_ITER3_WAVES
#define OFX_ITER3_WAVES 3
#endif
template <typename T, bool NT, bool STRICT, int CNT>
OFX_DEV void tvl1_iter3_march(const typename Pix<T>::v2 *__restrict__ Uin, const typename Pix<T>::v2 *__restrict__ P1in,
                              const typename Pix<T>::v2 *__restrict__ P2in, const typename Pix<T>::v2 *__restrict__ A,
                              const T *__restrict__ R, typename Pix<T>::v2 *Uout, typename Pix<T>::v2 *P1out,
                              typename Pix<T>::v2 *P2out, double *__restrict__ err, int slot0, int slot_step, int gw, int nx,
                              int ny, int y0, int yend, int ys, int yl, bool lef, bool rig, bool owner, unsigned off, unsigned so,
                              double up12, double up22, RowIn<T> cur, double l_t, double theta, double taut)
{
    const unsigned E2 = 2 * sizeof(T);
    const unsigned row2 = (unsigned) nx * E2;
    const double2 z2 = make_double2(0.0, 0.0);
    const unsigned level_bytes = (unsigned) nx * (unsigned) ny * E2;
    const ofx_rsrc rU = make_rsrc(Uout, level_bytes), rP1 = make_rsrc(P1out, level_bytes), rP2 = make_rsrc(P2out, level_bytes);
    double accA = 0.0, accB = 0.0, accC = 0.0;
    double2 uA0 = z2, uA1 = z2, uA2 = z2;
    double2 a1 = z2, a2 = z2, a3 = z2, a4 = z2;
    double r1c = 0.0, r2c = 0.0, r3c = 0.0, r4c = 0.0;
    double2 p0a = z2, p0b = z2;
    double2 pA1a = z2, pA1b = z2, pA2a = z2, pA2b = z2;
    double2 uB0 = z2, uB1 = z2, uB2 = z2;
    double2 pB1a = z2, pB1b = z2, pB2a = z2, pB2b = z2;
    double2 uC0 = z2, uC1 = z2;
    const int nyl = ny - 1;
    const int yB0 = y0 > 0 ? y0 - 1 : 0;
    const int ylc = (yend + CNT - 1 < yl) ? yend + CNT - 1 : yl;
    const int hiA = (yend + CNT - 2 < nyl) ? yend + CNT - 2 : nyl;
    const int hiB = (yend + CNT - 3 < nyl) ? yend + CNT - 3 : nyl;
    const int hiC = (yend < nyl) ? yend : nyl;
    const int ylast = yend - 1 + (2 * CNT - 1);
#ifdef OFX_CEIL_ALU
    const unsigned off0 = off;
#endif

    auto step = [&](const int y) {
        RowIn<T> nxt = cur;
#ifdef OFX_CEIL_ALU
        if (y + 1 <= ylc) nxt = tvl1_load_row<T>(Uin, P1in, P2in, A, R, off0 + ((y & 1) ? row2 : 0u));
#else
        if (y + 1 <= ylc) nxt = tvl1_load_row<T>(Uin, P1in, P2in, A, R, off + row2);
#endif
        unsigned stu = OFX_OOB, stp = OFX_OOB;
        double2 su = z2, sp1 = z2, sp2 = z2;

        if (y <= ylc) {
            const double l11 = wave_shift_up(cur.p1.x);
            const double l21 = wave_shift_up(cur.p2.x);
            uA0 = tvl1_primal<T, STRICT>(cur.u, cur.a, cur.r, cur.p1, cur.p2, l11, l21, up12, up22, lef, rig, y == 0, y == nyl, l_t,
                                         theta);
            const bool mine = owner && y >= y0 && y < yend;
            const double dA = (uA0.x - cur.u.x) * (uA0.x - cur.u.x) + (uA0.y - cur.u.y) * (uA0.y - cur.u.y);
            accA += mine ? dA : 0.0;
            if (CNT == 1 && mine) { stu = so; su = uA0; }
        }
        double2 pAna = z2, pAnb = z2;
        if (y - 1 >= ys && y - 1 <= hiA) {
            const double n1 = wave_shift_down(uA1.x);
            const double n2 = wave_shift_down(uA1.y);
            tvl1_dual<T, STRICT>(p0a, p0b, uA1, n1, n2, uA0, rig, y - 1 == nyl, taut, pAna, pAnb);
            pAna.x = rnd_to<T>(pAna.x); pAna.y = rnd_to<T>(pAna.y);
            pAnb.x = rnd_to<T>(pAnb.x); pAnb.y = rnd_to<T>(pAnb.y);
            if (CNT == 1 && owner && y - 1 >= y0 && y - 1 < yend) { stp = so - row2; sp1 = pAna; sp2 = pAnb; }
        }
        double2 pBna = z2, pBnb = z2;
        if (CNT >= 2) {
            if (y - 2 >= yB0 && y - 2 <= hiA) {
                const double l11 = wave_shift_up(pA1a.x);
                const double l21 = wave_shift_up(pA1b.x);
                uB0 = tvl1_primal<T, STRICT>(uA2, a2, r2c, pA1a, pA1b, l11, l21, pA2a.y, pA2b.y, lef, rig, y - 2 == 0, y - 2 == nyl,
                                             l_t, theta);
                const bool mine = owner && y - 2 >= y0 && y - 2 < yend;
                const double dB = (uB0.x - uA2.x) * (uB0.x - uA2.x) + (uB0.y - uA2.y) * (uB0.y - uA2.y);
                accB += mine ? dB : 0.0;
                if (CNT == 2 && mine) { stu = so - 2 * row2; su = uB0; }
            }
            if (y - 3 >= yB0 && y - 3 <= hiB) {
                const double n1 = wave_shift_down(uB1.x);
                const double n2 = wave_shift_down(uB1.y);
                tvl1_dual<T, STRICT>(pA2a, pA2b, uB1, n1, n2, uB0, rig, y - 3 == nyl, taut, pBna, pBnb);
                pBna.x = rnd_to<T>(pBna.x); pBna.y = rnd_to<T>(pBna.y);
                pBnb.x = rnd_to<T>(pBnb.x); pBnb.y = rnd_to<T>(pBnb.y);
                if (CNT == 2 && owner && y - 3 >= y0 && y - 3 < yend) { stp = so - 3 * row2; sp1 = pBna; sp2 = pBnb; }
            }
        }
        if (CNT == 3) {
            if (y - 4 >= y0 && y - 4 <= hiC) {
                const double l11 = wave_shift_up(pB1a.x);
                const double l21 = wave_shift_up(pB1b.x);
                uC0 = tvl1_primal<T, STRICT>(uB2, a4, r4c, pB1a, pB1b, l11, l21, pB2a.y, pB2b.y, lef, rig, y - 4 == 0, y - 4 == nyl,
                                             l_t, theta);
                const bool mine = owner && y - 4 < yend;
                const double dC = (uC0.x - uB2.x) * (uC0.x - uB2.x) + (uC0.y - uB2.y) * (uC0.y - uB2.y);
                accC += mine ? dC : 0.0;
                stu = mine ? so - 4 * row2 : stu;
                su = uC0;
            }
            if (y - 5 >= y0 && y - 5 < yend) {
                const double n1 = wave_shift_down(uC1.x);
                const double n2 = wave_shift_down(uC1.y);
                tvl1_dual<T, STRICT>(pB2a, pB2b, uC1, n1, n2, uC0, rig, y - 5 == nyl, taut, sp1, sp2);
                if (owner) stp = so - 5 * row2;
            }
        }
#ifdef OFX_CEIL_ALU
        stu = OFX_OOB; stp = OFX_OOB;
#endif
        bst2<NT>(rU, stu, su, Uout);
        bst2<NT>(rP1, stp, sp1, P1out);
        bst2<NT>(rP2, stp, sp2, P2out);
        uA2 = uA1; uA1 = uA0;
        a4 = a3; a3 = a2; a2 = a1; a1 = cur.a;
        r4c = r3c; r3c = r2c; r2c = r1c; r1c = cur.r;
        p0a = cur.p1; p0b = cur.p2;
        up12 = cur.p1.y; up22 = cur.p2.y;
        pA2a = pA1a; pA2b = pA1b; pA1a = pAna; pA1b = pAnb;
        uB2 = uB1; uB1 = uB0;
        pB2a = pB1a; pB2b = pB1b; pB1a = pBna; pB1b = pBnb;
        uC1 = uC0;
        cur = nxt;
        off += row2;
        so += row2;
    };
    for (int y = ys; y <= ylast; y++) step(y);
    loop_accumulate(err, slot0, accA, gw);
    if (CNT >= 2) loop_accumulate(err, slot0 + slot_step, accB, gw);
    if (CNT == 3) loop_accumulate(err, slot0 + 2 * slot_step, accC, gw);
}

template <typename T, bool NT, bool STRICT>
__global__ __launch_bounds__(256) __attribute__((amdgpu_waves_per_eu(OFX_ITER3_WAVES, OFX_ITER3_WAVES))) void k_tvl1_iter3(
    Tri<typename Pix<T>::v2> Ut, Tri<typename Pix<T>::v2> P1t, Tri<typename Pix<T>::v2> P2t,
    const typename Pix<T>::v2 *__restrict__ Ag, const T *__restrict__ Rg, double *__restrict__ errg, int k0, int check, int slot0,
    int nx, int ny, int rows, int strips_x, int strips_pad, double l_t, double theta, double taut, double eps2, unsigned incode,
    unsigned runmask, unsigned long long nit, int err_stride, OfxLoopDev *dev, int launch, double afac1, double afac2, int max_iter)
{
    using v2 = typename Pix<T>::v2;
    const int lane = threadIdx.x & 63;
    const int gw = OFX_WAVE_UNIFORM((int) (blockIdx.x * 4 + (threadIdx.x >> 6)));
    const int g = blockIdx.y;
    if (!((runmask >> g) & 1u)) return;
    int niter = (int) ((nit >> (4 * g)) & 15ull);
    const bool scribe = dev && blockIdx.x == 0 && threadIdx.x == 0;
    if (dev) {
        k0 = dev->cursor[launch & 1][g];
        slot0 = k0;
        check = 1;
        if (scribe) {
            dev->ulog[g][launch] = k0;
            dev->cursor[(launch + 1) & 1][g] = k0;
        }
        if (k0 >= max_iter) return;
    }
    const size_t npix = (size_t) nx * ny;
    const TriSel<v2> hu = pick3(Ut, incode, g, npix), h1 = pick3(P1t, incode, g, npix), h2 = pick3(P2t, incode, g, npix);
    const v2 *__restrict__ Uin = hu.in, *__restrict__ P1in = h1.in, *__restrict__ P2in = h2.in;
    const v2 *__restrict__ A = Ag + (size_t) g * npix;
    const T *__restrict__ R = Rg + (size_t) g * npix;
    double *__restrict__ err = errg + (size_t) g * err_stride;
    double prev[3];
#pragma unroll
    for (int i = 0; i < 3; i++) prev[i] = (check && k0 - i > 0) ? loop_fetch_prev(err, k0 - i) : 0.0;

    const int band = gw / strips_pad, strip = gw % strips_pad;
    const int y0 = band * rows;
    const bool idle = (strip >= strips_x) || (y0 >= ny);
    const int yend = (y0 + rows < ny) ? y0 + rows : ny;
    const int ys = y0 > 2 ? y0 - 2 : 0;
    const int yl = (yend + 2 < ny - 1) ? yend + 2 : ny - 1;
    const int c = strip * STRIP3_OUT - STRIP3_HALO + lane;
    const int cc = c < 0 ? 0 : (c > nx - 1 ? nx - 1 : c);
    const bool lef = (c == 0), rig = (c == nx - 1);
    const bool owner = (lane >= STRIP3_HALO) && (lane < STRIP3_OUT + STRIP3_HALO) && (c < nx);
    const unsigned E2 = 2 * sizeof(T);
    const unsigned row2 = (unsigned) nx * E2;
    const unsigned off = ((unsigned) ys * nx + cc) * E2;
    const unsigned so = ((unsigned) ys * nx + (c < 0 ? 0 : c)) * E2;
    double up12 = 0.0, up22 = 0.0;
    RowIn<T> cur;
    if (!idle) {
        if (ys > 0) {
            up12 = ldw2(at(P1in, off - row2)).y;
            up22 = ldw2(at(P2in, off - row2)).y;
        }
        cur = tvl1_load_row<T>(Uin, P1in, P2in, A, R, off);
    }
    if (check) {
        double e1 = 0.0;
#pragma unroll
        for (int i = 0; i < 3; i++) {
            if (k0 - i > 0) {
                const double e = loop_error_from_sum(wave_allreduce_sum(prev[i]), nx * ny, OFX_CRIT_MEAN);
                if (!(e > eps2)) return;
                if (i == 0) e1 = e;
            }
        }
        if (dev) {
            niter = (k0 > 0 && e1 <= eps2 * afac1) ? 1 : ((k0 > 0 && e1 <= eps2 * afac2) ? 2 : 3);
            if (niter > max_iter - k0) niter = max_iter - k0;
            if (scribe) dev->cursor[(launch + 1) & 1][g] = k0 + niter;
        }
    }
    if (idle) return;
    const int step = check ? 1 : 0;
    if (niter >= 3)
        tvl1_iter3_march<T, NT, STRICT, 3>(Uin, P1in, P2in, A, R, hu.out, h1.out, h2.out, err, slot0, step, gw, nx, ny, y0, yend, ys, yl,
                                           lef, rig, owner, off, so, up12, up22, cur, l_t, theta, taut);
    else if (niter == 2)
        tvl1_iter3_march<T, NT, STRICT, 2>(Uin, P1in, P2in, A, R, hu.out, h1.out, h2.out, err, slot0, step, gw, nx, ny, y0, yend, ys, yl,
                                           lef, rig, owner, off, so, up12, up22, cur, l_t, theta, taut);
    else
        tvl1_iter3_march<T, NT, STRICT, 1>(Uin, P1in, P2in, A, R, hu.out, h1.out, h2.out, err, slot0, step, gw, nx, ny, y0, yend, ys, yl,
                                           lef, rig, owner, off, so, up12, up22, cur, l_t, theta, taut);
}

#define TILE_RH 16
template <typename T, bool STRICT, int K>
__global__ __launch_bounds__(64 * TILE_RH) void k_tvl1_tile(
    Tri<typename Pix<T>::v2> Ut, Tri<typename Pix<T>::v2> P1t, Tri<typename Pix<T>::v2> P2t,
    const typename Pix<T>::v2 *__restrict__ Ag, const T *__restrict__ Rg, double *__restrict__ errg, int k0, int check, int slot0,
    int nx, int ny, int tiles_x, double l_t, double theta, double taut, double eps2, unsigned incode, unsigned runmask,
    unsigned long long nit, int err_stride)
{
    using v2 = typename Pix<T>::v2;
    static_assert(K < 16, "4 bits of `nit` per pair");
    __shared__ double2 s_p[2][TILE_RH][64];
    __shared__ double2 s_u[2][TILE_RH][64];
    const int lane = threadIdx.x & 63, w = threadIdx.x >> 6;
    const int g = blockIdx.y;
    if (!((runmask >> g) & 1u)) return;
    const int niter = (int) ((nit >> (4 * g)) & 15ull);
    const size_t npix = (size_t) nx * ny;
    const TriSel<v2> hu = pick3(Ut, incode, g, npix), h1 = pick3(P1t, incode, g, npix), h2 = pick3(P2t, incode, g, npix);
    double *__restrict__ err = errg + (size_t) g * err_stride;
    double prev[K];
#pragma unroll
    for (int i = 0; i < K; i++) prev[i] = (check && k0 - i > 0) ? loop_fetch_prev(err, k0 - i) : 0.0;

    constexpr int OW = 64 - 2 * K, OH = TILE_RH - 2 * K;
    const int tx = blockIdx.x % tiles_x, ty = blockIdx.x / tiles_x;
    const int c = tx * OW - K + lane, y = ty * OH - K + w;
    const int cc = c < 0 ? 0 : (c > nx - 1 ? nx - 1 : c), yc = y < 0 ? 0 : (y > ny - 1 ? ny - 1 : y);
    const bool inside = (c >= 0) && (c < nx) && (y >= 0) && (y < ny);
    const bool owner = inside && lane >= K && lane < 64 - K && w >= K && w < TILE_RH - K;
    const bool lef = (c == 0), rig = (c == nx - 1), top = (y == 0), bot = (y == ny - 1);
    const size_t p = (size_t) yc * nx + cc;
    double2 u = ldw2(hu.in + p), p1 = ldw2(h1.in + p), p2 = ldw2(h2.in + p);
    const double2 a = ldw2(Ag + (size_t) g * npix + p);
    const double r = ldw(Rg + (size_t) g * npix + p);
    if (check) {
#pragma unroll
        for (int i = 0; i < K; i++)
            if (k0 - i > 0 && !(loop_error_from_sum(wave_allreduce_sum(prev[i]), nx * ny, OFX_CRIT_MEAN) > eps2)) return;
    }
    double acc[K];
#pragma unroll
    for (int it = 0; it < K; it++) {
        acc[it] = 0.0;
        if (it < niter) {
            s_p[it & 1][w][lane] = make_double2(p1.y, p2.y);
            __syncthreads();
            const double2 up = s_p[it & 1][w > 0 ? w - 1 : 0][lane];
            const double l11 = wave_shift_up(p1.x), l21 = wave_shift_up(p2.x);
            const double2 un = tvl1_primal<T, STRICT>(u, a, r, p1, p2, l11, l21, up.x, up.y, lef, rig, top, bot, l_t, theta);
            if (owner) acc[it] = (un.x - u.x) * (un.x - u.x) + (un.y - u.y) * (un.y - u.y);
            s_u[it & 1][w][lane] = un;
            __syncthreads();
            const double2 dn = s_u[it & 1][w < TILE_RH - 1 ? w + 1 : w][lane];
            const double r1 = wave_shift_down(un.x), r2 = wave_shift_down(un.y);
            double2 q1, q2;
            tvl1_dual<T, STRICT>(p1, p2, un, r1, r2, dn, rig, bot, taut, q1, q2);
            u = un;
            p1 = make_double2(rnd_to<T>(q1.x), rnd_to<T>(q1.y));
            p2 = make_double2(rnd_to<T>(q2.x), rnd_to<T>(q2.y));
        }
    }
    if (owner) {
        const size_t po = (size_t) y * nx + c;
        stn2(hu.out + po, u);
        stn2(h1.out + po, p1);
        stn2(h2.out + po, p2);
    }
#pragma unroll
    for (int it = 0; it < K; it++)
        if (it < niter) loop_accumulate(err, slot0 + (check ? it : 0), acc[it], blockIdx.x * TILE_RH + w);
}

#ifndef OFX_WARP_BX
#define OFX_WARP_BX 64
#define OFX_WARP_BY 4
#endif
template <typename T>
__global__ void k_tvl1_warp(const typename Pix<T>::v2 *__restrict__ pag, const T *__restrict__ pbg, const T *__restrict__ I0g,
                            Tri<typename Pix<T>::v2> Ut,
                            typename Pix<T>::v2 *__restrict__ Ag, T *__restrict__ Rg, int nx, int ny, unsigned curcode)
{
    const int j = blockIdx.x * OFX_WARP_BX + threadIdx.x;
    const int i = blockIdx.y * OFX_WARP_BY + threadIdx.y;
    if (j >= nx || i >= ny) return;
    const int g = blockIdx.z;
    const size_t goff = (size_t) g * nx * ny;
    const typename Pix<T>::v2 *__restrict__ pa = pag + goff;
    const T *__restrict__ pb = pbg + goff;
    const T *__restrict__ I0 = I0g + goff;
    const typename Pix<T>::v2 *__restrict__ U = pick3(Ut, curcode, g, (size_t) nx * ny).in;
    typename Pix<T>::v2 *__restrict__ A = Ag + goff;
    T *__restrict__ R = Rg + goff;
    const size_t p = (size_t) i * nx + j;
    const double2 u = ldw2(U + p);
    const BicubicTaps t = bicubic_taps(j + u.x, i + u.y, nx, ny);
    double I1w = 0.0, I1wx = 0.0, I1wy = 0.0;
    if (!t.out) {
        bicubic_sample3(pa, pb, t, nx, I1w, I1wx, I1wy);
        I1wx = rnd_to<T>(I1wx);
        I1wy = rnd_to<T>(I1wy);
    }
    stn2(A + p, make_double2(I1wx, I1wy));
    stn(R + p, (I1w - I1wx * u.x - I1wy * u.y - ldw(I0 + p)));
}

#ifndef WARP_TW
#define WARP_TW 48
#define WARP_TH 16
#endif
#ifndef WARP_BY
#define WARP_BY 8
#endif
#ifndef WARP_WAVES
#define WARP_WAVES 8
#endif
#define WARP_ATTR __attribute__((amdgpu_waves_per_eu(WARP_WAVES, WARP_WAVES)))
#define WARP_NT (32 * WARP_BY)
#define WARP_NW (WARP_NT / 64)
template <typename T>
__global__ __launch_bounds__(WARP_NT) WARP_ATTR void k_tvl1_warp_lds(
    const typename Pix<T>::v2 *__restrict__ pag, const T *__restrict__ pbg, const T *__restrict__ I0g,
    Tri<typename Pix<T>::v2> Ut, typename Pix<T>::v2 *__restrict__ Ag, T *__restrict__ Rg, int nx, int ny,
    unsigned curcode)
{
    __shared__ double2 s_a[WARP_TH * WARP_TW];
    __shared__ double s_b[WARP_TH * WARP_TW];
    __shared__ int s_box[WARP_NW][4];
    const int tid = threadIdx.y * 32 + threadIdx.x, wave = tid >> 6;
    const int j = blockIdx.x * 32 + threadIdx.x;
    const int i = blockIdx.y * WARP_BY + threadIdx.y;
    const bool inside = (j < nx) && (i < ny);
    const int g = blockIdx.z;
    const size_t goff = (size_t) g * nx * ny;
    const typename Pix<T>::v2 *__restrict__ pa = pag + goff;
    const T *__restrict__ pb = pbg + goff;
    const typename Pix<T>::v2 *__restrict__ U = pick3(Ut, curcode, g, (size_t) nx * ny).in;
    const size_t p = (size_t) (inside ? i : 0) * nx + (inside ? j : 0);
    double2 u = make_double2(0.0, 0.0);
    BicubicTaps t;
    t.out = true;
    if (inside) {
        u = ldw2(U + p);
        t = bicubic_taps(j + u.x, i + u.y, nx, ny);
    }
    const bool need = inside && !t.out;
    int xlo = need ? t.col[0] : 0x7fffffff, xhi = need ? t.col[3] : -1;
    int ylo = need ? t.row[0] : 0x7fffffff, yhi = need ? t.row[3] : -1;
#pragma unroll
    for (int m = 32; m >= 1; m >>= 1) {
        xlo = min(xlo, __shfl_xor(xlo, m, 64)); xhi = max(xhi, __shfl_xor(xhi, m, 64));
        ylo = min(ylo, __shfl_xor(ylo, m, 64)); yhi = max(yhi, __shfl_xor(yhi, m, 64));
    }
    if ((tid & 63) == 0) { s_box[wave][0] = xlo; s_box[wave][1] = xhi; s_box[wave][2] = ylo; s_box[wave][3] = yhi; }
    __syncthreads();
#pragma unroll
    for (int w = 0; w < WARP_NW; w++) {
        xlo = min(xlo, s_box[w][0]); xhi = max(xhi, s_box[w][1]);
        ylo = min(ylo, s_box[w][2]); yhi = max(yhi, s_box[w][3]);
    }
    const int W = xhi - xlo + 1, H = yhi - ylo + 1;
    const bool any = (xhi >= 0);
    const bool tile = any && W <= WARP_TW && H <= WARP_TH;
    if (tile) {
        for (int k = tid; k < W * H; k += WARP_NT) {
            const int r = k / W, c = k - r * W;
            const size_t src = (size_t) (ylo + r) * nx + (xlo + c);
            s_a[r * WARP_TW + c] = ldw2(pa + src);
            s_b[r * WARP_TW + c] = ldw(pb + src);
        }
        __syncthreads();
    }
    if (!inside) return;
    double I1w = 0.0, I1wx = 0.0, I1wy = 0.0;
    if (need) {
        if (tile) {
            const int cx = t.col[0] - xlo, cy = t.row[0] - ylo;
            double c0[4], c1[4], c2[4];
#pragma unroll
            for (int k = 0; k < 4; k++) {
                const int o = cy * WARP_TW + cx + k;
                const double2 a0 = s_a[o], a1 = s_a[o + WARP_TW], a2 = s_a[o + 2 * WARP_TW], a3 = s_a[o + 3 * WARP_TW];
                const double b0 = s_b[o], b1 = s_b[o + WARP_TW], b2 = s_b[o + 2 * WARP_TW], b3 = s_b[o + 3 * WARP_TW];
                c0[k] = cubic_cell(a0.x, a1.x, a2.x, a3.x, t.fy);
                c1[k] = cubic_cell(a0.y, a1.y, a2.y, a3.y, t.fy);
                c2[k] = cubic_cell(b0, b1, b2, b3, t.fy);
            }
            I1w = cubic_cell(c0[0], c0[1], c0[2], c0[3], t.fx);
            I1wx = cubic_cell(c1[0], c1[1], c1[2], c1[3], t.fx);
            I1wy = cubic_cell(c2[0], c2[1], c2[2], c2[3], t.fx);
        } else {
            bicubic_sample3(pa, pb, t, nx, I1w, I1wx, I1wy);
        }
        I1wx = rnd_to<T>(I1wx);
        I1wy = rnd_to<T>(I1wy);
    }
    stn2(Ag + goff + p, make_double2(I1wx, I1wy));
    stn(Rg + goff + p, (I1w - I1wx * u.x - I1wy * u.y - ldw(I0g + goff + p)));
}

template <typename T>
__global__ void k_tvl1_zoom_in_g(Tri<typename Pix<T>::v2> Ut, unsigned curcode, typename Pix<T>::v2 *__restrict__ Uout, int nx,
                                 int ny, int nxx, int nyy, double fx, double fy, double scale)
{
    const int j1 = blockIdx.x * 64 + threadIdx.x;
    const int i1 = blockIdx.y * 4 + threadIdx.y;
    if (j1 >= nxx || i1 >= nyy) return;
    const int g = blockIdx.z;
    const typename Pix<T>::v2 *__restrict__ U = pick3(Ut, curcode, g, (size_t) nx * ny).in;
    const double i2 = i1 / fy, j2 = j1 / fx;
    const BicubicTaps t = bicubic_taps(j2, i2, nx, ny);
    double c1[4], c2[4];
#pragma unroll
    for (int k = 0; k < 4; k++) {
        const double2 v0 = ldw2(U + (size_t) t.row[0] * nx + t.col[k]);
        const double2 v1 = ldw2(U + (size_t) t.row[1] * nx + t.col[k]);
        const double2 v2 = ldw2(U + (size_t) t.row[2] * nx + t.col[k]);
        const double2 v3 = ldw2(U + (size_t) t.row[3] * nx + t.col[k]);
        c1[k] = cubic_cell(v0.x, v1.x, v2.x, v3.x, t.fy);
        c2[k] = cubic_cell(v0.y, v1.y, v2.y, v3.y, t.fy);
    }
    double2 r;
    r.x = cubic_cell(c1[0], c1[1], c1[2], c1[3], t.fx) * scale;
    r.y = cubic_cell(c2[0], c2[1], c2[2], c2[3], t.fx) * scale;
    stn2(Uout + (size_t) g * nxx * nyy + (size_t) i1 * nxx + j1, r);
}

template <typename T>
__global__ void k_tvl1_to_flo_g(Tri<typename Pix<T>::v2> Ut, unsigned curcode, OfxGroupPtrs out, size_t n)
{
    const size_t i = (size_t) blockIdx.x * blockDim.x + threadIdx.x;
    if (i >= n) return;
    const int g = blockIdx.y;
    const double2 v = ldw2(pick3(Ut, curcode, g, n).in + i);
    ((float2 *) out.a[g])[i] = make_float2((float) v.x, (float) v.y);
}

template <typename T> struct Tvl1Level {
    using v2 = typename Pix<T>::v2;
    using v4 = typename Pix<T>::v4;
    int nx, ny, G;
    T  *I0, *I1;
    v2 *pa;
    T  *pb;
    v2 *U[3], *P1[3], *P2[3], *A;
    T  *R;
    unsigned cur;
    int last_n[OFX_MAX_GROUP];
    size_t n() const { return (size_t) nx * ny; }
    unsigned curidx(int g) const { return (cur >> (2 * g)) & 3u; }
    v2 *Ucur(int g) const { return U[curidx(g)] + (size_t) g * n(); }
    v2 *P1cur(int g) const { return P1[curidx(g)] + (size_t) g * n(); }
    v2 *P2cur(int g) const { return P2[curidx(g)] + (size_t) g * n(); }
    Tri<v2> Ut() const { return Tri<v2>{U[0], U[1], U[2]}; }
    Tri<v2> P1t() const { return Tri<v2>{P1[0], P1[1], P1[2]}; }
    Tri<v2> P2t() const { return Tri<v2>{P2[0], P2[1], P2[2]}; }
};

struct Tvl1Params {
    double tau, lambda, theta, epsilon;
    int warps, verbose, max_iter;
    bool fixed;
};

template <typename T> static int tvl1_level_alloc(ofx_ctx *ctx, Tvl1Level<T> &L, int nx, int ny, int G, bool images)
{
    const size_t n = (size_t) nx * ny * G;
    L.nx = nx;
    L.ny = ny;
    L.G = G;
    L.cur = 0;
    for (int g = 0; g < OFX_MAX_GROUP; g++) L.last_n[g] = 0;
    L.I0 = L.I1 = nullptr;
    if (images) {
        OFX_TRY(ofx_alloc(ctx, n, &L.I0));
        OFX_TRY(ofx_alloc(ctx, n, &L.I1));
    }
    OFX_TRY(ofx_alloc(ctx, n, &L.pa));
    OFX_TRY(ofx_alloc(ctx, n, &L.pb));
    for (int h = 0; h < 3; h++) {
        OFX_TRY(ofx_alloc(ctx, n, &L.U[h]));
        OFX_TRY(ofx_alloc(ctx, n, &L.P1[h]));
        OFX_TRY(ofx_alloc(ctx, n, &L.P2[h]));
    }
    OFX_TRY(ofx_alloc(ctx, n, &L.A));
    OFX_TRY(ofx_alloc(ctx, n, &L.R));
    return OFX_OK;
}

static int tvl1_pick_rows(const ofx_ctx *ctx, int nx, int ny, int G)
{
    if (ctx->rows_per_wave > 0) return ctx->rows_per_wave;
    const long strips = (long) ofx_cdiv(nx, STRIP_OUT) * G;
    if (strips * ofx_cdiv(ny, 4) >= 2048) return 4;
    if (strips * ofx_cdiv(ny, 2) >= 1024) return 2;
    return 1;
}

static int tvl1_pick_rows2(const ofx_ctx *ctx, int nx, int ny, int G)
{
    if (ctx->rows_per_wave2 > 0) return ctx->rows_per_wave2;
    const long strips_pad = (long) ofx_cdiv(ofx_cdiv(nx, STRIP2_OUT), 4) * 4 * G;
    const int rmax = 24;
    int best = rmax;
    long best_cost = -1;
    if (ctx->concurrency > 1) {
        static const int cand[] = {1, 2, 3, 4, 5, 6, 8, 10, 12, 14, 16, 20, 24};
        for (int r : cand) {
            const long waves = strips_pad * ofx_cdiv(ny, r);
            const long slots = ctx->rows_slots > 0 ? ctx->rows_slots : 1024;
            const long cost = ((waves + slots - 1) / slots) * (r + 5);
            if (best_cost < 0 || cost < best_cost) { best_cost = cost; best = r; }
        }
        return best;
    }
    const long slots = 1024L * OFX_ITER2_WAVES;
    for (int k = 1; k <= 4; k++) {
        for (int r = 1; r <= rmax; r++) {
            if (strips_pad * ofx_cdiv(ny, r) > k * slots) continue;
            const long cost = (long) k * (r + 5);
            if (best_cost < 0 || cost < best_cost) { best_cost = cost; best = r; }
            break;
        }
    }
    if (best < 3 && strips_pad * ofx_cdiv(ny, 3) >= 512) best = 3;
    return best;
}

static int tvl1_pick_chunk(const ofx_ctx *ctx, int nx, int ny, int G)
{
    if (ctx->chunk > 0) return ctx->chunk;
    const double est_us = fmax(5.0, (double) nx * ny * G * 120.0 / 4.0e6);
    int c = (int) (40.0 / est_us);
    return c < 4 ? 4 : (c > 50 ? 50 : c);
}

static int tvl1_pick_tile(const ofx_ctx *ctx, int nx, int ny, int G)
{
    if (!ctx->tile || !ctx->fuse2) return 0;
    const double lim = ctx->tile_max_px > 0 ? ctx->tile_max_px : 200000.0;
    if ((double) nx * ny * G > lim) return 0;
    return ctx->tile == 6 ? 6 : 4;
}

template <typename T> struct Tvl1Level;
struct Tvl1Params;
template <typename T>
static int tvl1_run_iterations_tile(ofx_ctx *ctx, Tvl1Level<T> &L, const Tvl1Params &P, LoopSpec S, int K, int *n_out,
                                    double *err_out, float *ms_out, int *alt_out);
template <typename T>
static int tvl1_run_iterations_tri(ofx_ctx *ctx, Tvl1Level<T> &L, const Tvl1Params &P, LoopSpec S, int *n_out, double *err_out,
                                   float *ms_out, int *alt_out);

static int tvl1_pick_rows3(const ofx_ctx *ctx, int nx, int ny, int G)
{
    if (ctx->rows_per_wave3 > 0) return ctx->rows_per_wave3;
    {
        static const char *tab = getenv("OFX_ROWS3");
        for (const char *q = tab; q && *q;) {
            int lny = 0, r = 0;
            if (sscanf(q, "%d:%d", &lny, &r) == 2 && lny == ny && r > 0) return r;
            q = strchr(q, '/');
            if (q) q++;
        }
    }
    const long strips_pad = (long) ofx_cdiv(ofx_cdiv(nx, STRIP3_OUT), 4) * 4 * G;
    const int rmax = 32;
    int best = rmax;
    long best_cost = -1;
    if (ctx->concurrency > 1) {
        static const int cand[] = {2, 3, 4, 5, 6, 8, 10, 12, 14, 16, 20, 24, 28, 32, 36, 40, 48, 54, 64, 72, 80, 96};
        for (int r : cand) {
            if (r > ctx->rows3_max) break;
            const long waves = strips_pad * ofx_cdiv(ny, r);
            const long slots = ctx->rows_slots > 0 ? ctx->rows_slots : 1024;
            const long cost = ((waves + slots - 1) / slots) * (r + 7);
            if (best_cost < 0 || cost < best_cost) { best_cost = cost; best = r; }
        }
        return best;
    }
    const long slots = 1024L * OFX_ITER3_WAVES;
    for (int k = 1; k <= 4; k++) {
        for (int r = 1; r <= rmax; r++) {
            if (strips_pad * ofx_cdiv(ny, r) > k * slots) continue;
            const long cost = (long) k * (r + 7);
            if (best_cost < 0 || cost < best_cost) { best_cost = cost; best = r; }
            break;
        }
    }
    if (best < 4 && strips_pad * ofx_cdiv(ny, 4) >= 512) best = 4;
    return best;
}

template <typename T>
static int tvl1_run_iterations(ofx_ctx *ctx, Tvl1Level<T> &L, const Tvl1Params &P, int *n_out, double *err_out,
                               float *ms_out, int *alt_out = nullptr,
                               int *unit_out = nullptr)
{
    const int nx = L.nx, ny = L.ny, G = L.G;
    if ((long long) nx * ny >= (1LL << 27)) return ofx_fail(ctx, OFX_ERR_ARG, "tvl1: image larger than 2^27 pixels");
    const double l_t = P.lambda * P.theta, taut = P.tau / P.theta, theta = P.theta;
    const bool pairs = ctx->fuse2 != 0;
    const int rows = tvl1_pick_rows(ctx, nx, ny, G);
    const int strips_x = ofx_cdiv(nx, STRIP_OUT), strips_pad = ofx_cdiv(strips_x, 4) * 4;
    const unsigned gx1 = (unsigned) (strips_pad / 4) * ofx_cdiv(ny, rows);
    const dim3 block(256);
    const int rows2 = tvl1_pick_rows2(ctx, nx, ny, G);
    const int strips2_x = ofx_cdiv(nx, STRIP2_OUT), strips2_pad = ofx_cdiv(strips2_x, 4) * 4;
    const dim3 grid2((unsigned) (strips2_pad / 4) * ofx_cdiv(ny, rows2), G);
    LoopSpec S;
    S.max_iter = P.max_iter;
    S.size = nx * ny;
    S.thr = P.epsilon * P.epsilon;
    S.crit = OFX_CRIT_MEAN;
    S.chunk = tvl1_pick_chunk(ctx, nx, ny, G);
    S.fixed = P.fixed;
    S.pairs = pairs;
    const int tileK = tvl1_pick_tile(ctx, nx, ny, G);
    if (unit_out) *unit_out = tileK ? tileK : (pairs ? 2 : 1);
    if (tileK) return tvl1_run_iterations_tile<T>(ctx, L, P, S, tileK, n_out, err_out, ms_out, alt_out);
    {
        const bool strict_mode = sizeof(T) == sizeof(double) && !ctx->relaxed_dual;
        const double px = (double) nx * ny * G;
        const bool tri = ctx->fuse3 == 1 ? px >= ctx->fuse3_min_px
                                         : (ctx->fuse3 == 2 && !strict_mode && (G >= 2 || ctx->concurrency > 1) &&
                                            px >= (ctx->fuse3_min_px > 0 ? ctx->fuse3_min_px : 5e5));
        if (pairs && tri) {
            if (unit_out) *unit_out = 3;
            return tvl1_run_iterations_tri<T>(ctx, L, P, S, n_out, err_out, ms_out, alt_out);
        }
    }
    const int err_stride = (S.max_iter + 1) * OFX_NSHARD;
    const unsigned all = (G >= 32) ? 0xFFFFFFFFu : ((1u << G) - 1u);
    const bool nt_stores = ctx->nt_stores ? ctx->nt_stores == 1 : (double) nx * ny * G * 15.0 * sizeof(T) > 300e6;
    unsigned b0[OFX_MAX_GROUP];
    for (int g = 0; g < G; g++) b0[g] = L.curidx(g);
    auto code_of = [&](unsigned unit) -> unsigned {
        unsigned c = 0;
        for (int g = 0; g < G; g++) c |= ((b0[g] + unit) % 3u) << (2 * g);
        return c;
    };
    const bool sa = pairs && !P.fixed && ctx->store_a != 0;
    S.afac = sa ? (ctx->store_a == 2 ? 1e300 : 1.5) : 0.0;
    unsigned amask0 = 0;
    if (sa)
        for (int g = 0; g < G; g++)
            if (ctx->store_a == 2 || (L.last_n[g] >= 1 && L.last_n[g] <= 2)) amask0 |= 1u << g;
    const bool strict = sizeof(T) == sizeof(double) && !ctx->relaxed_dual;
    auto single = [&](unsigned incode, unsigned runmask, int check, int slot, double thr) -> int {
        auto kern = k_tvl1_iter<T, false>;
        if constexpr (sizeof(T) == sizeof(double)) { if (strict) kern = k_tvl1_iter<T, true>; }
        hipLaunchKernelGGL(kern, dim3(gx1, G), block, 0, ctx->stream, L.Ut(), L.P1t(), L.P2t(), L.A, (const T *) L.R,
                           ctx->d_err, check, slot, nx, ny, rows, strips_x, strips_pad, l_t, theta, taut, thr, incode, runmask,
                           err_stride);
        OFX_LAUNCH_CHECK(ctx);
        return OFX_OK;
    };
    auto launch = [&](int k, int cnt, double thr) -> int {
        const unsigned incode = code_of((unsigned) (pairs ? k / 2 : k));
        if (cnt == 1) return single(incode, all, k, k, thr);
        const unsigned amask = k == 0 ? amask0 : 0u;
        auto kern = nt_stores ? k_tvl1_iter2<T, true, false> : k_tvl1_iter2<T, false, false>;
        if constexpr (sizeof(T) == sizeof(double)) {
            if (strict) kern = nt_stores ? k_tvl1_iter2<T, true, true> : k_tvl1_iter2<T, false, true>;
        }
        hipLaunchKernelGGL(kern, grid2, block, 0, ctx->stream, L.Ut(), L.P1t(), L.P2t(), L.A, (const T *) L.R, ctx->d_err, k, nx,
                           ny, rows2, strips2_x, strips2_pad, l_t, theta, taut, thr, incode, amask, S.afac, err_stride);
        OFX_LAUNCH_CHECK(ctx);
        return OFX_OK;
    };
    auto redo = [&](const int *k_of) -> int {
        unsigned incode = 0, runmask = 0;
        for (int g = 0; g < G; g++) {
            if (k_of[g] < 0) continue;
            runmask |= 1u << g;
            incode |= ((b0[g] + (unsigned) (k_of[g] / 2)) % 3u) << (2 * g);
        }
        return single(incode, runmask, 0, S.max_iter, -1.0);
    };
    int took_alt[OFX_MAX_GROUP];
    OFX_TRY(ofx_run_loop_group(ctx, S, G, launch, redo, n_out, err_out, ms_out, amask0, took_alt));
    unsigned cur = 0;
    for (int g = 0; g < G; g++) {
        const unsigned units = (unsigned) (pairs ? (n_out[g] + 1) / 2 : n_out[g]);
        cur |= ((b0[g] + units + (took_alt[g] ? 1u : 0u)) % 3u) << (2 * g);
        L.last_n[g] = n_out[g];
        if (alt_out) alt_out[g] = (pairs && (n_out[g] & 1) && n_out[g] != S.max_iter) ? (took_alt[g] ? 2 : 1) : 0;
    }
    L.cur = cur;
    return OFX_OK;
}

static_assert(OFX_MAX_GROUP * 4 <= 64 && OFX_MAX_GROUP * 2 <= 32,
              "k_tvl1_tile / k_tvl1_iter3 pack 4 bits of iteration count (`nit`, 64 bits) and 2 bits of buffer index (`incode`, 32 bits) per pair");
template <typename T>
static int tvl1_run_iterations_tile(ofx_ctx *ctx, Tvl1Level<T> &L, const Tvl1Params &P, LoopSpec S, int K, int *n_out,
                                    double *err_out, float *ms_out, int *alt_out)
{
    const int nx = L.nx, ny = L.ny, G = L.G;
    const double l_t = P.lambda * P.theta, taut = P.tau / P.theta, theta = P.theta;
    const bool strict = sizeof(T) == sizeof(double) && !ctx->relaxed_dual;
    const int OW = 64 - 2 * K, OH = TILE_RH - 2 * K;
    const int tiles_x = ofx_cdiv(nx, OW), tiles_y = ofx_cdiv(ny, OH);
    const dim3 grid((unsigned) (tiles_x * tiles_y), G), block(64 * TILE_RH);
    S.pairs = false;
    S.fuse = K;
    S.afac = 0.0;
    if (ctx->chunk <= 0) S.chunk = 6 * K;
    const int err_stride = (S.max_iter + 1) * OFX_NSHARD;
    const unsigned all = (G >= 32) ? 0xFFFFFFFFu : ((1u << G) - 1u);
    unsigned b0[OFX_MAX_GROUP];
    for (int g = 0; g < G; g++) b0[g] = L.curidx(g);
    auto go = [&](int k0, int check, int slot0, double thr, unsigned incode, unsigned runmask, unsigned long long nit) -> int {
        auto kern = K == 6 ? k_tvl1_tile<T, false, 6> : k_tvl1_tile<T, false, 4>;
        if constexpr (sizeof(T) == sizeof(double)) {
            if (strict) kern = K == 6 ? k_tvl1_tile<T, true, 6> : k_tvl1_tile<T, true, 4>;
        }
        hipLaunchKernelGGL(kern, grid, block, 0, ctx->stream, L.Ut(), L.P1t(), L.P2t(), L.A, (const T *) L.R, ctx->d_err, k0, check,
                           slot0, nx, ny, tiles_x, l_t, theta, taut, thr, incode, runmask, nit, err_stride);
        OFX_LAUNCH_CHECK(ctx);
        return OFX_OK;
    };
    auto launch = [&](int k, int cnt, double thr) -> int {
        unsigned incode = 0;
        unsigned long long nit = 0;
        for (int g = 0; g < G; g++) {
            incode |= ((b0[g] + (unsigned) (k / K)) % 3u) << (2 * g);
            nit |= (unsigned long long) cnt << (4 * g);
        }
        return go(k, 1, k, thr, incode, all, nit);
    };
    auto redo = [&](const int *k_of) -> int {
        unsigned incode = 0, runmask = 0;
        unsigned long long nit = 0;
        for (int g = 0; g < G; g++) {
            if (k_of[g] < 0) continue;
            const int n = k_of[g] + 1, j = (n - 1) / K;
            runmask |= 1u << g;
            incode |= ((b0[g] + (unsigned) j) % 3u) << (2 * g);
            nit |= (unsigned long long) (n - j * K) << (4 * g);
        }
        return go(0, 0, S.max_iter, -1.0, incode, runmask, nit);
    };
    int took_alt[OFX_MAX_GROUP];
    OFX_TRY(ofx_run_loop_group(ctx, S, G, launch, redo, n_out, err_out, ms_out, 0u, took_alt));
    unsigned cur = 0;
    for (int g = 0; g < G; g++) {
        const unsigned units = (unsigned) ((n_out[g] + K - 1) / K);
        cur |= ((b0[g] + units) % 3u) << (2 * g);
        L.last_n[g] = n_out[g];
        if (alt_out) alt_out[g] = 0;
    }
    L.cur = cur;
    return OFX_OK;
}

template <typename T>
static int tvl1_run_iterations_tri(ofx_ctx *ctx, Tvl1Level<T> &L, const Tvl1Params &P, LoopSpec S, int *n_out, double *err_out,
                                   float *ms_out, int *alt_out)
{
    const int nx = L.nx, ny = L.ny, G = L.G;
    const double l_t = P.lambda * P.theta, taut = P.tau / P.theta, theta = P.theta;
    const bool strict = sizeof(T) == sizeof(double) && !ctx->relaxed_dual;
    const int rows = tvl1_pick_rows3(ctx, nx, ny, G);
    const int strips_x = ofx_cdiv(nx, STRIP3_OUT), strips_pad = ofx_cdiv(strips_x, 4) * 4;
    const dim3 grid((unsigned) (strips_pad / 4) * ofx_cdiv(ny, rows), G), block(256);
    const bool nt_stores = ctx->nt_stores ? ctx->nt_stores == 1 : (double) nx * ny * G * 15.0 * sizeof(T) > 300e6;
    S.pairs = false;
    S.fuse = 3;
    S.afac = 0.0;
    const int err_stride = (S.max_iter + 1) * OFX_NSHARD;
    const unsigned all = (G >= 32) ? 0xFFFFFFFFu : ((1u << G) - 1u);
    unsigned b0[OFX_MAX_GROUP];
    for (int g = 0; g < G; g++) b0[g] = L.curidx(g);
    const bool cursor = ctx->fuse3_cursor != 0 && !S.fixed;
    const double afac2 = ctx->fuse3_afac2 > 0 ? ctx->fuse3_afac2 : 1.5, afac1 = ctx->fuse3_afac1 > 0 ? ctx->fuse3_afac1 : 1.2;
    auto go = [&](int k0, int check, int slot0, double thr, unsigned incode, unsigned runmask, unsigned long long nit, OfxLoopDev *dev,
                  int launch) -> int {
        auto kern = nt_stores ? k_tvl1_iter3<T, true, false> : k_tvl1_iter3<T, false, false>;
        if constexpr (sizeof(T) == sizeof(double)) {
            if (strict) kern = nt_stores ? k_tvl1_iter3<T, true, true> : k_tvl1_iter3<T, false, true>;
        }
        hipLaunchKernelGGL(kern, grid, block, 0, ctx->stream, L.Ut(), L.P1t(), L.P2t(), L.A, (const T *) L.R, ctx->d_err, k0, check,
                           slot0, nx, ny, rows, strips_x, strips_pad, l_t, theta, taut, thr, incode, runmask, nit, err_stride, dev, launch,
                           afac1, afac2, S.max_iter);
        OFX_LAUNCH_CHECK(ctx);
        return OFX_OK;
    };
    auto code_of_unit = [&](unsigned unit) -> unsigned {
        unsigned c = 0;
        for (int g = 0; g < G; g++) c |= ((b0[g] + unit) % 3u) << (2 * g);
        return c;
    };
    int unit_of[OFX_MAX_GROUP];
    int inside[OFX_MAX_GROUP];
    if (cursor) {
        auto launch = [&](int Lidx, double thr) -> int {
            return go(0, 1, 0, thr, code_of_unit((unsigned) Lidx), all, 0ull, reinterpret_cast<OfxLoopDev *>(ctx->d_state), Lidx);
        };
        auto redo = [&](const int *n_of, const int *k0_of, const int *u_of) -> int {
            unsigned incode = 0, runmask = 0;
            unsigned long long nit = 0;
            for (int g = 0; g < G; g++) {
                if (n_of[g] < 0) continue;
                runmask |= 1u << g;
                incode |= ((b0[g] + (unsigned) u_of[g]) % 3u) << (2 * g);
                nit |= (unsigned long long) (n_of[g] - k0_of[g]) << (4 * g);
            }
            return go(0, 0, S.max_iter, -1.0, incode, runmask, nit, nullptr, 0);
        };
        const int upc = (S.chunk + 2) / 3 < 1 ? 1 : (S.chunk + 2) / 3;
        OFX_TRY(ofx_run_loop_cursor(ctx, S, G, upc, 3, launch, redo, n_out, err_out, unit_of, inside, ms_out));
    } else {
        auto launch = [&](int k, int cnt, double thr) -> int {
            unsigned long long nit = 0;
            for (int g = 0; g < G; g++) nit |= (unsigned long long) cnt << (4 * g);
            return go(k, 1, k, thr, code_of_unit((unsigned) (k / 3)), all, nit, nullptr, 0);
        };
        auto redo = [&](const int *k_of) -> int {
            unsigned incode = 0, runmask = 0;
            unsigned long long nit = 0;
            for (int g = 0; g < G; g++) {
                if (k_of[g] < 0) continue;
                const int n = k_of[g] + 1, j = (n - 1) / 3;
                runmask |= 1u << g;
                incode |= ((b0[g] + (unsigned) j) % 3u) << (2 * g);
                nit |= (unsigned long long) (n - j * 3) << (4 * g);
            }
            return go(0, 0, S.max_iter, -1.0, incode, runmask, nit, nullptr, 0);
        };
        int took_alt[OFX_MAX_GROUP];
        OFX_TRY(ofx_run_loop_group(ctx, S, G, launch, redo, n_out, err_out, ms_out, 0u, took_alt));
        for (int g = 0; g < G; g++) {
            unit_of[g] = n_out[g] > 0 ? (n_out[g] - 1) / 3 : -1;
            inside[g] = (n_out[g] % 3 != 0 && n_out[g] != S.max_iter) ? 1 : 0;
        }
    }
    unsigned cur = 0;
    for (int g = 0; g < G; g++) {
        const unsigned units = (unsigned) (unit_of[g] + 1);
        cur |= ((b0[g] + units) % 3u) << (2 * g);
        L.last_n[g] = n_out[g];
        if (alt_out) alt_out[g] = inside[g] ? 1 : 0;
    }
    L.cur = cur;
    return OFX_OK;
}

template <typename T>
static int tvl1_single_scale_dev(ofx_ctx *ctx, Tvl1Level<T> &L, const Tvl1Params &P, int scale, ofx_stats *stats)
{
    const int nx = L.nx, ny = L.ny, G = L.G;
    const size_t n = L.n();
    const dim3 g2(ofx_cdiv(nx, OFX_WARP_BX), ofx_cdiv(ny, OFX_WARP_BY), G), b2(OFX_WARP_BX, OFX_WARP_BY);
    if (nx < 2 || ny < 2) return ofx_fail(ctx, OFX_ERR_ARG, "tvl1: level %dx%d too small", nx, ny);

    OFX_TRY(op_grad_pack<T>(ctx, L.I1, L.pa, L.pb, nx, ny, G));
    for (int h = 0; h < 3; h++) {
        bool used = false;
        for (int g = 0; g < G; g++) used = used || (L.curidx(g) == (unsigned) h);
        if (!used) continue;
        OFX_TRY(op_fill2<T>(ctx, L.P1[h], n * G));
        OFX_TRY(op_fill2<T>(ctx, L.P2[h], n * G));
    }
    for (int g = 0; g < G; g++) L.last_n[g] = 0;

    for (int w = 0; w < P.warps; w++) {
        if (ctx->warp_lds)
            hipLaunchKernelGGL(k_tvl1_warp_lds<T>, dim3(ofx_cdiv(nx, 32), ofx_cdiv(ny, WARP_BY), G), dim3(32, WARP_BY), 0, ctx->stream, L.pa,
                               (const T *) L.pb, (const T *) L.I0, L.Ut(), L.A, L.R, nx, ny, L.cur);
        else
            hipLaunchKernelGGL(k_tvl1_warp<T>, g2, b2, 0, ctx->stream, L.pa, (const T *) L.pb, (const T *) L.I0, L.Ut(),
                               L.A, L.R, nx, ny, L.cur);
        OFX_LAUNCH_CHECK(ctx);
        int it[OFX_MAX_GROUP];
        double error[OFX_MAX_GROUP];
        float ms = 0.f;
        int odd[OFX_MAX_GROUP], unit = 0;
        OFX_TRY(tvl1_run_iterations<T>(ctx, L, P, it, error, ctx->profile ? &ms : nullptr, odd, &unit));
        if (P.verbose && G == 1) fprintf(stderr, "Warping: %d, Iterations: %d, Error: %f\n", w, it[0], error[0]);
        for (int g = 0; g < G; g++) {
            ofx_stats &S = stats[g];
            S.odd_stops += odd[g] != 0;
            S.odd_stops_stored += odd[g] == 2;
            if (scale < OFX_MAX_SCALES) {
                S.fused[scale] = unit;
                if (w < OFX_MAX_SOLVES) { S.iters[scale][w] = it[g]; S.error[scale][w] = error[g]; }
                S.iter_ms[scale] += ms;
                S.iter_launches[scale] += it[g];
            }
            S.work_pix_iters += (double) it[g] * nx * ny;
        }
    }
    return OFX_OK;
}

static void stats_begin(ofx_stats *st, int nscales, int nsolves)
{
    memset(st, 0, sizeof(*st));
    st->nscales = nscales;
    st->nsolves = nsolves;
}

template <typename T>
static int tvl1_multiscale_dev(ofx_ctx *ctx, int G, const T *const *dI0, const T *const *dI1, int nxx, int nyy,
                               const Tvl1Params &P, int nscales, double zfactor, std::vector<Tvl1Level<T>> &lv,
                               ofx_stats *stats)
{
    if (P.warps < 1) return ofx_fail(ctx, OFX_ERR_ARG, "tvl1: warps=%d", P.warps);
    if (G < 1 || G > OFX_MAX_GROUP) return ofx_fail(ctx, OFX_ERR_ARG, "tvl1: group of %d pairs", G);

    std::vector<int> nxs, nys;
    OFX_TRY(op_pyramid_sizes(ctx, nxx, nyy, nscales, zfactor, nxs, nys));
    for (int g = 0; g < G; g++) {
        stats_begin(&stats[g], nscales, P.warps);
        for (int s = 0; s < nscales && s < OFX_MAX_SCALES; s++) { stats[g].nx[s] = nxs[s]; stats[g].ny[s] = nys[s]; }
    }
    lv.resize(nscales);
    for (int s = 0; s < nscales; s++) OFX_TRY(tvl1_level_alloc<T>(ctx, lv[s], nxs[s], nys[s], G, true));
    {
        T *tmpA, *tmpB;
        double *scr;
        OFX_TRY(ofx_alloc(ctx, (size_t) 2 * G * nxx * nyy, &tmpA));
        OFX_TRY(ofx_alloc(ctx, (size_t) 2 * G * nxx * nyy, &tmpB));
        OFX_TRY(ofx_alloc(ctx, (size_t) G * op_pyramid_scratch_doubles(), &scr));
        std::vector<T *> lA(nscales), lB(nscales);
        for (int s = 0; s < nscales; s++) { lA[s] = lv[s].I0; lB[s] = lv[s].I1; }
        OFX_TRY(op_build_pyramid_group<T>(ctx, G, (const void *const *) dI0, (const void *const *) dI1, nscales, zfactor,
                                          TVL1_PRESMOOTHING_SIGMA, nxs.data(), nys.data(), lA.data(), lB.data(), tmpA, tmpB, scr));
    }
    Tvl1Level<T> &C = lv[nscales - 1];
    OFX_TRY(op_fill2<T>(ctx, C.U[0], C.n() * G));

    for (int s = nscales - 1; s >= 0; s--) {
        if (P.verbose && G == 1) fprintf(stderr, "Scale %d: %dx%d\n", s, lv[s].nx, lv[s].ny);
        OFX_TRY(tvl1_single_scale_dev<T>(ctx, lv[s], P, s, stats));
        if (!s) break;
        lv[s - 1].cur = 0;
        {
            const int nxf = lv[s - 1].nx, nyf = lv[s - 1].ny;
            hipLaunchKernelGGL(k_tvl1_zoom_in_g<T>, dim3(ofx_cdiv(nxf, 64), ofx_cdiv(nyf, 4), G), dim3(64, 4), 0, ctx->stream,
                               lv[s].Ut(), lv[s].cur, lv[s - 1].U[0], lv[s].nx, lv[s].ny, nxf, nyf, (double) nxf / lv[s].nx,
                               (double) nyf / lv[s].ny, 1.0 / zfactor);
            OFX_LAUNCH_CHECK(ctx);
        }
    }
    return OFX_OK;
}

static Tvl1Params make_params(const ofx_ctx *ctx, double tau, double lambda, double theta, int warps,
                               double epsilon, int verbose)
{
    Tvl1Params P;
    P.tau = tau; P.lambda = lambda; P.theta = theta; P.epsilon = epsilon;
    P.warps = warps; P.verbose = verbose;
    P.max_iter = OFX_TVL1_MAX_ITERATIONS;
    P.fixed = ctx->fixed_work != 0;
    return P;
}

template <typename T>
static int upload_image(ofx_ctx *ctx, const double *h, size_t n, T **out)
{
    double *stage;
    OFX_TRY(ofx_alloc(ctx, n, &stage));
    OFX_TRY(ofx_alloc(ctx, n, out));
    OFX_HIP(ctx, hipMemcpyAsync(stage, h, n * sizeof(double), hipMemcpyHostToDevice, ctx->stream));
    return op_convert_in<T>(ctx, stage, *out, n);
}

template <typename T>
static int tvl1_multiscale_host(ofx_ctx *ctx, const double *I0, const double *I1, double *u1, double *u2, int nx,
                                int ny, const Tvl1Params &P, int nscales, double zfactor)
{
    const size_t n = (size_t) nx * ny;
    T *dI0, *dI1;
    OFX_TRY(upload_image<T>(ctx, I0, n, &dI0));
    OFX_TRY(upload_image<T>(ctx, I1, n, &dI1));
    std::vector<Tvl1Level<T>> lv;
    const T *a = dI0, *b = dI1;
    OFX_TRY(tvl1_multiscale_dev<T>(ctx, 1, &a, &b, nx, ny, P, nscales, zfactor, lv, &ctx->stats));
    double *d1, *d2;
    OFX_TRY(ofx_alloc(ctx, n, &d1));
    OFX_TRY(ofx_alloc(ctx, n, &d2));
    OFX_TRY(op_deinterleave2<T>(ctx, lv[0].Ucur(0), d1, d2, n));
    OFX_HIP(ctx, hipMemcpyAsync(u1, d1, n * sizeof(double), hipMemcpyDeviceToHost, ctx->stream));
    OFX_HIP(ctx, hipMemcpyAsync(u2, d2, n * sizeof(double), hipMemcpyDeviceToHost, ctx->stream));
    OFX_HIP(ctx, hipStreamSynchronize(ctx->stream));
    return OFX_OK;
}

extern "C" int ofx_tvl1_multiscale(ofx_ctx *ctx, const double *I0, const double *I1, double *u1, double *u2, int nx,
                                   int ny, double tau, double lambda, double theta, int nscales, double zfactor,
                                   int warps, double epsilon, int verbose)
{
    OFX_ENTER(ctx);
    if (!I0 || !I1 || !u1 || !u2) return ofx_fail(ctx, OFX_ERR_ARG, "tvl1: NULL pointer");
    const double t0 = ofx_now_ms();
    const Tvl1Params P = make_params(ctx, tau, lambda, theta, warps, epsilon, verbose);
    int s = ctx->precision == OFX_F64
                ? tvl1_multiscale_host<double>(ctx, I0, I1, u1, u2, nx, ny, P, nscales, zfactor)
                : tvl1_multiscale_host<float>(ctx, I0, I1, u1, u2, nx, ny, P, nscales, zfactor);
    ctx->stats.total_ms = ofx_now_ms() - t0;
    return s;
}

static bool ofx_ptr_is_local(const ofx_ctx *ctx, const void *p)
{
    hipPointerAttribute_t a;
    if (hipPointerGetAttributes(&a, p) != hipSuccess) {
        (void) hipGetLastError();
        return false;
    }
    return a.type == hipMemoryTypeDevice && a.device == ctx->device;
}
extern "C" int ofx_staging_route(int ctx_device, int mem_device, int can_access_peer)
{
    if (mem_device == ctx_device) return 0;
    if (mem_device < 0) return 1;
    return can_access_peer ? 1 : 2;
}
static int ofx_copy_staged(ofx_ctx *ctx, void *dst, const void *src, size_t bytes)
{
    const void *other = ofx_ptr_is_local(ctx, dst) ? src : dst;
    int mem_device = -1, can = 1;
    hipPointerAttribute_t a;
    if (hipPointerGetAttributes(&a, other) == hipSuccess) {
        if (a.type == hipMemoryTypeDevice) mem_device = a.device;
    } else {
        (void) hipGetLastError();
    }
    if (mem_device >= 0 && mem_device != ctx->device && hipDeviceCanAccessPeer(&can, ctx->device, mem_device) != hipSuccess) {
        (void) hipGetLastError();
        can = 0;
    }
    if (ofx_staging_route(ctx->device, mem_device, can) < 2) {
        OFX_HIP(ctx, hipMemcpyAsync(dst, src, bytes, hipMemcpyDefault, ctx->stream));
        return OFX_OK;
    }
    void *bounce = nullptr;
    OFX_HIP(ctx, hipHostMalloc(&bounce, bytes, hipHostMallocDefault));
    hipError_t e = hipStreamSynchronize(ctx->stream);
    if (e == hipSuccess) e = hipMemcpy(bounce, src, bytes, hipMemcpyDefault);
    if (e == hipSuccess) e = hipMemcpy(dst, bounce, bytes, hipMemcpyDefault);
    (void) hipHostFree(bounce);
    if (e != hipSuccess) return ofx_fail(ctx, OFX_ERR_HIP, "staging through the host failed: %s", hipGetErrorString(e));
    snprintf(ctx->errmsg, sizeof(ctx->errmsg), "note: GPU %d cannot address GPU %d, buffers were staged through the host", ctx->device,
             mem_device);
    return OFX_OK;
}

template <typename T>
static int tvl1_group_devapi(ofx_ctx *ctx, int G, const void *const *dI0_in, const void *const *dI1_in, void *const *d_flo_in,
                             int nx, int ny, const Tvl1Params &P, int nscales, double zfactor, ofx_stats *stats)
{
    const size_t n = (size_t) nx * ny;
    const void *dI0[OFX_MAX_GROUP], *dI1[OFX_MAX_GROUP];
    void *d_flo[OFX_MAX_GROUP];
    for (int g = 0; g < G; g++) {
        const void *src[2] = {dI0_in[g], dI1_in[g]};
        const void **dst[2] = {&dI0[g], &dI1[g]};
        for (int k = 0; k < 2; k++) {
            if (ofx_ptr_is_local(ctx, src[k])) { *dst[k] = src[k]; continue; }
            T *stage;
            OFX_TRY(ofx_alloc(ctx, n, &stage));
            OFX_TRY(ofx_copy_staged(ctx, stage, src[k], n * sizeof(T)));
            *dst[k] = stage;
        }
        d_flo[g] = d_flo_in[g];
        if (!ofx_ptr_is_local(ctx, d_flo_in[g])) {
            float2 *stage;
            OFX_TRY(ofx_alloc(ctx, n, &stage));
            d_flo[g] = stage;
        }
    }
    std::vector<Tvl1Level<T>> lv;
    OFX_TRY(tvl1_multiscale_dev<T>(ctx, G, (const T *const *) dI0, (const T *const *) dI1, nx, ny, P, nscales, zfactor, lv,
                                   stats));
    OfxGroupPtrs out;
    for (int g = 0; g < OFX_MAX_GROUP; g++) { out.a[g] = g < G ? d_flo[g] : nullptr; out.b[g] = nullptr; }
    hipLaunchKernelGGL(k_tvl1_to_flo_g<T>, dim3((unsigned) ((n + 255) / 256), G), dim3(256), 0, ctx->stream, lv[0].Ut(), lv[0].cur,
                       out, n);
    OFX_LAUNCH_CHECK(ctx);
    for (int g = 0; g < G; g++)
        if (d_flo[g] != d_flo_in[g]) OFX_TRY(ofx_copy_staged(ctx, d_flo_in[g], d_flo[g], n * sizeof(float2)));
    return OFX_OK;
}

extern "C" int ofx_tvl1_multiscale_dev(ofx_ctx *ctx, const void *dI0, const void *dI1, void *d_flo, int nx, int ny,
                                       double tau, double lambda, double theta, int nscales, double zfactor,
                                       int warps, double epsilon, int verbose)
{
    OFX_ENTER(ctx);
    if (!dI0 || !dI1 || !d_flo) return ofx_fail(ctx, OFX_ERR_ARG, "tvl1: NULL pointer");
    const double t0 = ofx_now_ms();
    const Tvl1Params P = make_params(ctx, tau, lambda, theta, warps, epsilon, verbose);
    int s = ctx->precision == OFX_F64
                ? tvl1_group_devapi<double>(ctx, 1, &dI0, &dI1, &d_flo, nx, ny, P, nscales, zfactor, &ctx->stats)
                : tvl1_group_devapi<float>(ctx, 1, &dI0, &dI1, &d_flo, nx, ny, P, nscales, zfactor, &ctx->stats);
    ctx->stats.total_ms = ofx_now_ms() - t0;
    return s;
}

extern "C" int ofx_tvl1_group_dev(ofx_ctx *ctx, int n_pairs, const void *const *dI0, const void *const *dI1,
                                  void *const *d_flo, int nx, int ny, double tau, double lambda, double theta,
                                  int nscales, double zfactor, int warps, double epsilon, ofx_stats *stats_out)
{
    OFX_ENTER(ctx);
    if (!dI0 || !dI1 || !d_flo) return ofx_fail(ctx, OFX_ERR_ARG, "tvl1: NULL pointer");
    if (n_pairs < 1 || n_pairs > OFX_MAX_GROUP)
        return ofx_fail(ctx, OFX_ERR_ARG, "tvl1: a lockstep group holds 1..%d pairs (got %d)", OFX_MAX_GROUP, n_pairs);
    for (int g = 0; g < n_pairs; g++)
        if (!dI0[g] || !dI1[g] || !d_flo[g]) return ofx_fail(ctx, OFX_ERR_ARG, "tvl1: NULL pointer (pair %d)", g);
    const double t0 = ofx_now_ms();
    const Tvl1Params P = make_params(ctx, tau, lambda, theta, warps, epsilon, 0);
    std::vector<ofx_stats> local(stats_out ? 0 : n_pairs);
    ofx_stats *st = stats_out ? stats_out : local.data();
    int s = ctx->precision == OFX_F64
                ? tvl1_group_devapi<double>(ctx, n_pairs, dI0, dI1, d_flo, nx, ny, P, nscales, zfactor, st)
                : tvl1_group_devapi<float>(ctx, n_pairs, dI0, dI1, d_flo, nx, ny, P, nscales, zfactor, st);
    const double ms = ofx_now_ms() - t0;
    for (int g = 0; g < n_pairs; g++) st[g].total_ms = ms;
    ctx->stats = st[0];
    return s;
}

template <typename T>
static int tvl1_single_scale_host(ofx_ctx *ctx, const double *I0, const double *I1, double *u1, double *u2, int nx,
                                  int ny, const Tvl1Params &P)
{
    const size_t n = (size_t) nx * ny;
    stats_begin(&ctx->stats, 1, P.warps);
    ctx->stats.nx[0] = nx;
    ctx->stats.ny[0] = ny;
    Tvl1Level<T> L;
    OFX_TRY(tvl1_level_alloc<T>(ctx, L, nx, ny, 1, false));
    OFX_TRY(upload_image<T>(ctx, I0, n, &L.I0));
    OFX_TRY(upload_image<T>(ctx, I1, n, &L.I1));
    double *d1, *d2;
    OFX_TRY(ofx_alloc(ctx, n, &d1));
    OFX_TRY(ofx_alloc(ctx, n, &d2));
    OFX_HIP(ctx, hipMemcpyAsync(d1, u1, n * sizeof(double), hipMemcpyHostToDevice, ctx->stream));
    OFX_HIP(ctx, hipMemcpyAsync(d2, u2, n * sizeof(double), hipMemcpyHostToDevice, ctx->stream));
    OFX_TRY(op_interleave2<T>(ctx, d1, d2, L.U[0], n));
    OFX_TRY(tvl1_single_scale_dev<T>(ctx, L, P, 0, &ctx->stats));
    OFX_TRY(op_deinterleave2<T>(ctx, L.Ucur(0), d1, d2, n));
    OFX_HIP(ctx, hipMemcpyAsync(u1, d1, n * sizeof(double), hipMemcpyDeviceToHost, ctx->stream));
    OFX_HIP(ctx, hipMemcpyAsync(u2, d2, n * sizeof(double), hipMemcpyDeviceToHost, ctx->stream));
    OFX_HIP(ctx, hipStreamSynchronize(ctx->stream));
    return OFX_OK;
}

extern "C" int ofx_tvl1_single_scale(ofx_ctx *ctx, const double *I0, const double *I1, double *u1, double *u2,
                                     int nx, int ny, double tau, double lambda, double theta, int warps,
                                     double epsilon, int verbose)
{
    OFX_ENTER(ctx);
    if (!I0 || !I1 || !u1 || !u2) return ofx_fail(ctx, OFX_ERR_ARG, "tvl1: NULL pointer");
    if (nx < 2 || ny < 2 || warps < 1) return ofx_fail(ctx, OFX_ERR_ARG, "tvl1: bad size / warps");
    const double t0 = ofx_now_ms();
    const Tvl1Params P = make_params(ctx, tau, lambda, theta, warps, epsilon, verbose);
    int s = ctx->precision == OFX_F64 ? tvl1_single_scale_host<double>(ctx, I0, I1, u1, u2, nx, ny, P)
                                      : tvl1_single_scale_host<float>(ctx, I0, I1, u1, u2, nx, ny, P);
    ctx->stats.total_ms = ofx_now_ms() - t0;
    return s;
}

template <typename T>
static int tvl1_iterations_host(ofx_ctx *ctx, double *u1, double *u2, double *p11, double *p12, double *p21,
                                double *p22, const double *I1wx, const double *I1wy, const double *rho_c, int nx,
                                int ny, const Tvl1Params &P, double *error)
{
    const size_t n = (size_t) nx * ny;
    stats_begin(&ctx->stats, 1, 1);
    ctx->stats.nx[0] = nx;
    ctx->stats.ny[0] = ny;
    Tvl1Level<T> L;
    OFX_TRY(tvl1_level_alloc<T>(ctx, L, nx, ny, 1, false));
    double *d[2];
    OFX_TRY(ofx_alloc(ctx, n, &d[0]));
    OFX_TRY(ofx_alloc(ctx, n, &d[1]));
    struct { const double *a, *b; typename Pix<T>::v2 *dst; } up[4] = {
        {u1, u2, L.U[0]}, {p11, p12, L.P1[0]}, {p21, p22, L.P2[0]}, {I1wx, I1wy, L.A}};
    for (auto &e : up) {
        OFX_HIP(ctx, hipMemcpyAsync(d[0], e.a, n * sizeof(double), hipMemcpyHostToDevice, ctx->stream));
        OFX_HIP(ctx, hipMemcpyAsync(d[1], e.b, n * sizeof(double), hipMemcpyHostToDevice, ctx->stream));
        OFX_TRY(op_interleave2<T>(ctx, d[0], d[1], e.dst, n));
    }
    OFX_HIP(ctx, hipMemcpyAsync(d[0], rho_c, n * sizeof(double), hipMemcpyHostToDevice, ctx->stream));
    OFX_TRY(op_convert_in<T>(ctx, d[0], L.R, n));

    int it = 0;
    double err = 0.0;
    float ms = 0.f;
    OFX_TRY(tvl1_run_iterations<T>(ctx, L, P, &it, &err, ctx->profile ? &ms : nullptr));
    ctx->stats.iters[0][0] = it;
    ctx->stats.error[0][0] = err;
    ctx->stats.iter_ms[0] = ms;
    ctx->stats.iter_launches[0] = it;
    ctx->stats.work_pix_iters = (double) it * nx * ny;
    if (error) *error = err;

    struct { double *a, *b; typename Pix<T>::v2 *src; } down[3] = {
        {u1, u2, L.Ucur(0)}, {p11, p12, L.P1cur(0)}, {p21, p22, L.P2cur(0)}};
    for (auto &e : down) {
        OFX_TRY(op_deinterleave2<T>(ctx, e.src, d[0], d[1], n));
        OFX_HIP(ctx, hipMemcpyAsync(e.a, d[0], n * sizeof(double), hipMemcpyDeviceToHost, ctx->stream));
        OFX_HIP(ctx, hipMemcpyAsync(e.b, d[1], n * sizeof(double), hipMemcpyDeviceToHost, ctx->stream));
    }
    OFX_HIP(ctx, hipStreamSynchronize(ctx->stream));
    return OFX_OK;
}

extern "C" int ofx_tvl1_iterations(ofx_ctx *ctx, double *u1, double *u2, double *p11, double *p12, double *p21,
                                   double *p22, const double *I1wx, const double *I1wy, const double *rho_c, int nx,
                                   int ny, double tau, double lambda, double theta, int n_iter, double *error)
{
    OFX_ENTER(ctx);
    if (!u1 || !u2 || !p11 || !p12 || !p21 || !p22 || !I1wx || !I1wy || !rho_c)
        return ofx_fail(ctx, OFX_ERR_ARG, "tvl1_iterations: NULL pointer");
    if (nx < 2 || ny < 2 || n_iter < 1 || n_iter > OFX_TVL1_MAX_ITERATIONS)
        return ofx_fail(ctx, OFX_ERR_ARG, "tvl1_iterations: bad size / n_iter");
    const double t0 = ofx_now_ms();
    Tvl1Params P = make_params(ctx, tau, lambda, theta, 1, 0.0, 0);
    P.max_iter = n_iter;
    P.fixed = true;
    int s = ctx->precision == OFX_F64
                ? tvl1_iterations_host<double>(ctx, u1, u2, p11, p12, p21, p22, I1wx, I1wy, rho_c, nx, ny, P, error)
                : tvl1_iterations_host<float>(ctx, u1, u2, p11, p12, p21, p22, I1wx, I1wy, rho_c, nx, ny, P, error);
    ctx->stats.total_ms = ofx_now_ms() - t0;
    return s;
}

extern "C" int ofx_tvl1_batch_group_size(ofx_ctx *const *ctxs, int n_ctx, int n_pairs, int nx, int ny, int nscales,
                                         double zfactor)
{
    if (!ctxs || n_ctx < 1 || !ctxs[0] || n_pairs < 0 || nx < 1 || ny < 1) return -OFX_ERR_ARG;
    int G = ctxs[0]->lockstep;
    if (G > 0) return G > OFX_MAX_GROUP ? OFX_MAX_GROUP : G;
    if (n_pairs <= 1) return 1;
    std::vector<int> nxs, nys;
    const int st = op_pyramid_sizes(ctxs[0], nx, ny, nscales, zfactor, nxs, nys);
    if (st != OFX_OK) return -st;
    double px = 0;
    for (int s = 0; s < nscales; s++) px += (double) nxs[s] * nys[s];
    const double elem = ctxs[0]->precision == OFX_F32 ? 4.0 : 8.0;
    const double per_pair = (26.0 * px + 4.0 * (double) nx * ny) * elem;
    const double per_ctx = 64e6;
    int dev_now = 0;
    (void) hipGetDevice(&dev_now);
    int cap = OFX_MAX_GROUP;
    for (int w = 0; w < n_ctx; w++) {
        if (!ctxs[w]) return -OFX_ERR_ARG;
        int on_dev = 0;
        bool seen = false;
        for (int v = 0; v < n_ctx; v++) {
            if (!ctxs[v] || ctxs[v]->device != ctxs[w]->device) continue;
            on_dev++;
            seen = seen || v < w;
        }
        if (seen) continue;
        double budget = ctxs[w]->mem_budget > 0 ? ctxs[w]->mem_budget * on_dev / n_ctx : -1.0;
        if (budget < 0) {
            size_t mfree = 0, mtotal = 0;
            (void) hipSetDevice(ctxs[w]->device);
            if (hipMemGetInfo(&mfree, &mtotal) == hipSuccess) budget = 0.5 * (double) mfree;
            else (void) hipGetLastError();
        }
        if (budget >= 0) {
            const double fit = (budget / on_dev - per_ctx) / per_pair;
            if (fit < cap) cap = fit < 1.0 ? 1 : (int) fit;
        }
    }
    (void) hipSetDevice(dev_now);
    const int rounds = (n_pairs + n_ctx * cap - 1) / (n_ctx * cap);
    G = (n_pairs + n_ctx * rounds - 1) / (n_ctx * rounds);
    return G < 1 ? 1 : G;
}

__global__ void k_hypot(const double *__restrict__ x, const double *__restrict__ y, double *__restrict__ out, int n)
{
    const int i = blockIdx.x * blockDim.x + threadIdx.x;
    if (i < n) out[i] = hypot_ref(x[i], y[i]);
}
extern "C" int ofx_hypot(ofx_ctx *ctx, const double *x, const double *y, double *out, int n)
{
    OFX_ENTER(ctx);
    if (!x || !y || !out || n < 1) return ofx_fail(ctx, OFX_ERR_ARG, "hypot: NULL pointer / n < 1");
    double *dx, *dy, *dz;
    OFX_TRY(ofx_alloc(ctx, (size_t) n, &dx));
    OFX_TRY(ofx_alloc(ctx, (size_t) n, &dy));
    OFX_TRY(ofx_alloc(ctx, (size_t) n, &dz));
    OFX_HIP(ctx, hipMemcpyAsync(dx, x, sizeof(double) * n, hipMemcpyHostToDevice, ctx->stream));
    OFX_HIP(ctx, hipMemcpyAsync(dy, y, sizeof(double) * n, hipMemcpyHostToDevice, ctx->stream));
    hipLaunchKernelGGL(k_hypot, dim3((n + 255) / 256), dim3(256), 0, ctx->stream, (const double *) dx, (const double *) dy, dz, n);
    OFX_LAUNCH_CHECK(ctx);
    OFX_HIP(ctx, hipMemcpyAsync(out, dz, sizeof(double) * n, hipMemcpyDeviceToHost, ctx->stream));
    OFX_HIP(ctx, hipStreamSynchronize(ctx->stream));
    return OFX_OK;
}

extern "C" int ofx_tvl1_batch_dev(ofx_ctx *const *ctxs, int n_ctx, const void *const *dI0, const void *const *dI1,
                                  void *const *d_flo, int n_pairs, int nx, int ny, double tau, double lambda,
                                  double theta, int nscales, double zfactor, int warps, double epsilon,
                                  double *work_pix_iters)
{
    if (!ctxs || n_ctx < 1 || n_pairs < 0 || !dI0 || !dI1 || !d_flo) return OFX_ERR_ARG;
    for (int w = 0; w < n_ctx; w++)
        if (!ctxs[w] || ctxs[w]->precision != ctxs[0]->precision) return OFX_ERR_ARG;
    const int G = ofx_tvl1_batch_group_size(ctxs, n_ctx, n_pairs, nx, ny, nscales, zfactor);
    if (G < 1) return G < 0 ? -G : OFX_ERR_ARG;
    const int n_groups = (n_pairs + G - 1) / G;
    std::atomic<int> status(OFX_OK);
    auto worker = [&](int w) {
        std::vector<ofx_stats> st(G);
        for (int q = w; q < n_groups; q += n_ctx) {
            if (status.load() != OFX_OK) return;
            const int first = q * G, cnt = (n_pairs - first < G) ? n_pairs - first : G;
            const int s = ofx_tvl1_group_dev(ctxs[w], cnt, dI0 + first, dI1 + first, d_flo + first, nx, ny, tau, lambda, theta,
                                             nscales, zfactor, warps, epsilon, st.data());
            if (s != OFX_OK) { int expected = OFX_OK; status.compare_exchange_strong(expected, s); return; }
            if (work_pix_iters)
                for (int g = 0; g < cnt; g++) work_pix_iters[first + g] = st[g].work_pix_iters;
        }
        (void) hipStreamSynchronize(ctxs[w]->stream);
    };
    std::vector<std::thread> th;
    for (int w = 1; w < n_ctx && w < n_groups; w++) th.emplace_back(worker, w);
    worker(0);
    for (auto &t : th) t.join();
    return status.load();
}
```

Measured before the change: 78810 Mpix*warp-iters/s.

## Skip dual zero-fill and loads on first warp; add image-based warp kernel

Adds a PZ template flag to the TV-L1 iteration kernels. When the dual variables are known to be zero (first warp of each scale), the kernels skip loading P1/P2 and the host skips the per-scale dual clearing fills. Launches are split by group mask into zero-dual and normal variants. An optional warp kernel that computes gradients straight from the image in an LDS tile, with fallback counting, is added but disabled by default. The cost is more kernel instantiations and possibly two launches per step when groups are mixed.

```diff
diff --git a/include/ofx.h b/include/ofx.h
--- a/include/ofx.h
+++ b/include/ofx.h
@@ -41,6 +41,7 @@
     int    odd_stops_stored;
     int    fused[OFX_MAX_SCALES];
     double pyramid_ms;
+    long long warp_fallbacks;
 } ofx_stats;
 
 int  ofx_device_count(void);
diff --git a/optical-flow-1_amd/__init__.py b/optical-flow-1_amd/__init__.py
--- a/optical-flow-1_amd/__init__.py
+++ b/optical-flow-1_amd/__init__.py
@@ -29,7 +29,7 @@
                 ("iter_launches", C.c_longlong * MAX_SCALES),
                 ("work_pix_iters", C.c_double), ("total_ms", C.c_double),
                 ("odd_stops", C.c_int), ("odd_stops_stored", C.c_int), ("fused", C.c_int * MAX_SCALES),
-                ("pyramid_ms", C.c_double)]
+                ("pyramid_ms", C.c_double), ("warp_fallbacks", C.c_longlong)]
 
     def iterations(self):
         return np.array([[self.iters[s][w] for w in range(min(self.nsolves, MAX_SOLVES))]
diff --git a/optical-flow-1_amd/csrc/ofx_ctx.cpp b/optical-flow-1_amd/csrc/ofx_ctx.cpp
--- a/optical-flow-1_amd/csrc/ofx_ctx.cpp
+++ b/optical-flow-1_amd/csrc/ofx_ctx.cpp
@@ -77,6 +77,8 @@
     ctx->concurrency = 1;
     ctx->lockstep = 0;
     ctx->warp_lds = 1;
+    ctx->warp_image = 0;
+    ctx->implicit_zero_duals = 1;
     ctx->gauss_fused = 1;
     ctx->relaxed_dual = 0;
     ctx->tile = 0;
@@ -116,6 +118,7 @@
     ctx->stream = nullptr;
     ctx->d_err = nullptr;
     ctx->d_state = nullptr;
+    ctx->d_warp_fb = nullptr;
     ctx->h_state = nullptr;
     ctx->h_aux = nullptr;
     ctx->ev_t0 = ctx->ev_t1 = nullptr;
@@ -127,6 +130,9 @@
     ok = ok && hipMalloc((void **) &ctx->d_state, OFX_STATE_BYTES + sizeof(double) * OFX_TVL1_MAX_ITERATIONS * OFX_NSHARD) == hipSuccess;
     if (ok) ctx->d_err = reinterpret_cast<double *>(reinterpret_cast<char *>(ctx->d_state) + OFX_STATE_BYTES);
     ctx->d_err_cap = OFX_TVL1_MAX_ITERATIONS;
+    ok = ok && hipMalloc((void **) &ctx->d_warp_fb, sizeof(unsigned) * OFX_MAX_GROUP) == hipSuccess;
+    ok = ok && hipMemsetAsync(ctx->d_warp_fb, 0, sizeof(unsigned) * OFX_MAX_GROUP, ctx->stream) == hipSuccess;
+    ok = ok && hipStreamSynchronize(ctx->stream) == hipSuccess;
     mark("hipMalloc (loop state)");
     ok = ok && hipHostMalloc((void **) &ctx->h_state, sizeof(OfxIterState) * OFX_NPOLL * OFX_MAX_GROUP + sizeof(double) * OFX_MAX_GROUP,
                              hipHostMallocDefault) == hipSuccess;
@@ -155,6 +161,7 @@
     if (ctx->stream) (void) hipStreamSynchronize(ctx->stream);
     for (auto &s : ctx->slabs) (void) hipFree(s.base);
     if (ctx->d_state) (void) hipFree(ctx->d_state);
+    if (ctx->d_warp_fb) (void) hipFree(ctx->d_warp_fb);
     if (ctx->h_state) (void) hipHostFree(ctx->h_state);
     for (int i = 0; i < OFX_NPOLL; i++)
         if (ctx->ev_poll[i]) (void) hipEventDestroy(ctx->ev_poll[i]);
@@ -208,6 +215,8 @@
     if (!strcmp(name, "relaxed_dual")) { ctx->relaxed_dual = value != 0; return OFX_OK; }
     if (!strcmp(name, "gauss_fused")) { ctx->gauss_fused = (value == 2 || value == 3) ? (int) value : (value != 0); return OFX_OK; }
     if (!strcmp(name, "warp_lds")) { ctx->warp_lds = value != 0; return OFX_OK; }
+    if (!strcmp(name, "warp_image")) { ctx->warp_image = value != 0; return OFX_OK; }
+    if (!strcmp(name, "implicit_zero_duals")) { ctx->implicit_zero_duals = value != 0; return OFX_OK; }
     if (!strcmp(name, "nt_stores")) { ctx->nt_stores = (int) value; return (value >= 0 && value <= 2) ? OFX_OK : ofx_fail(ctx, OFX_ERR_ARG, "nt_stores = 0 | 1 | 2"); }
     if (!strcmp(name, "lockstep")) {
         if (value < 0 || value > OFX_MAX_GROUP) return ofx_fail(ctx, OFX_ERR_ARG, "lockstep out of range");
diff --git a/optical-flow-1_amd/csrc/ofx_internal.h b/optical-flow-1_amd/csrc/ofx_internal.h
--- a/optical-flow-1_amd/csrc/ofx_internal.h
+++ b/optical-flow-1_amd/csrc/ofx_internal.h
@@ -56,6 +56,7 @@
     double       *h_aux;
     hipEvent_t    ev_poll[OFX_NPOLL];
     hipEvent_t    ev_t0, ev_t1;
+    unsigned     *d_warp_fb;
 
     int profile;
     int rows_per_wave;
@@ -70,6 +71,8 @@
     double tile_max_px;
     int gauss_fused;
     int warp_lds;
+    int warp_image;
+    int implicit_zero_duals;
     int chunk;
     int fuse3;
     double fuse3_min_px;
diff --git a/optical-flow-1_amd/csrc/ofx_tvl1.hip b/optical-flow-1_amd/csrc/ofx_tvl1.hip
--- a/optical-flow-1_amd/csrc/ofx_tvl1.hip
+++ b/optical-flow-1_amd/csrc/ofx_tvl1.hip
@@ -34,14 +34,14 @@
     return reinterpret_cast<V *>(reinterpret_cast<char *>(base) + byte_off);
 }
 
-template <typename T>
+template <typename T, bool PZ = false>
 OFX_DEV RowIn<T> tvl1_load_row(const typename Pix<T>::v2 *U, const typename Pix<T>::v2 *P1,
                                const typename Pix<T>::v2 *P2, const typename Pix<T>::v2 *A, const T *R, unsigned off2)
 {
     RowIn<T> r;
     r.u = ldw2(at(U, off2));
-    r.p1 = ldw2(at(P1, off2));
-    r.p2 = ldw2(at(P2, off2));
+    r.p1 = PZ ? make_double2(0.0, 0.0) : ldw2(at(P1, off2));
+    r.p2 = PZ ? make_double2(0.0, 0.0) : ldw2(at(P2, off2));
     r.a = ldw2(at(A, off2));
     r.r = ldw(at(R, off2 >> 1));
     return r;
@@ -206,7 +206,7 @@
 #else
 #define OFX_ITER1_ATTR
 #endif
-template <typename T, bool STRICT>
+template <typename T, bool STRICT, bool PZ>
 __global__ __launch_bounds__(256) OFX_ITER1_ATTR void k_tvl1_iter(
     Tri<typename Pix<T>::v2> Ut, Tri<typename Pix<T>::v2> P1t, Tri<typename Pix<T>::v2> P2t,
     const typename Pix<T>::v2 *__restrict__ Ag, const T *__restrict__ Rg, double *__restrict__ errg, int check, int slot,
@@ -247,11 +247,11 @@
     double up12 = 0.0, up22 = 0.0;
     RowIn<T> cur;
     if (!idle) {
-        if (y0 > 0) {
+        if (!PZ && y0 > 0) {
             up12 = ldw2(at(P1in, off - row2)).y;
             up22 = ldw2(at(P2in, off - row2)).y;
         }
-        cur = tvl1_load_row<T>(Uin, P1in, P2in, A, R, off);
+        cur = tvl1_load_row<T, PZ>(Uin, P1in, P2in, A, R, off);
     }
 
     double e1;
@@ -266,7 +266,7 @@
 
     for (int y = y0; y <= yend; y++) {
         RowIn<T> nxt = cur;
-        if (y + 1 <= yend && y + 1 < ny) nxt = tvl1_load_row<T>(Uin, P1in, P2in, A, R, off + row2);
+        if (y + 1 <= yend && y + 1 < ny) nxt = tvl1_load_row<T, PZ>(Uin, P1in, P2in, A, R, off + row2);
 
         double2 un = make_double2(0.0, 0.0);
         unsigned st_u = OFX_OOB, st_p = OFX_OOB;
@@ -314,7 +314,7 @@
 #else
 #define OFX_ITER2_BOUNDS __launch_bounds__(256)
 #endif
-template <typename T, bool NT, bool SA, bool STRICT>
+template <typename T, bool NT, bool SA, bool STRICT, bool PZ>
 OFX_DEV void tvl1_iter2_march(const typename Pix<T>::v2 *__restrict__ Uin, const typename Pix<T>::v2 *__restrict__ P1in,
                               const typename Pix<T>::v2 *__restrict__ P2in, const typename Pix<T>::v2 *__restrict__ A,
                               const T *__restrict__ R, typename Pix<T>::v2 *Uout, typename Pix<T>::v2 *P1out,
@@ -343,9 +343,9 @@
     for (int y = ys; y <= yend + 2; y++) {
         RowIn<T> nxt = cur;
 #ifdef OFX_CEIL_ALU
-        if (y + 1 <= yl) nxt = tvl1_load_row<T>(Uin, P1in, P2in, A, R, off0 + (((unsigned) (y + 1 - ys)) & 1u) * row2);
+        if (y + 1 <= yl) nxt = tvl1_load_row<T, PZ>(Uin, P1in, P2in, A, R, off0 + (((unsigned) (y + 1 - ys)) & 1u) * row2);
 #else
-        if (y + 1 <= yl) nxt = tvl1_load_row<T>(Uin, P1in, P2in, A, R, off + row2);
+        if (y + 1 <= yl) nxt = tvl1_load_row<T, PZ>(Uin, P1in, P2in, A, R, off + row2);
 #endif
 
         const bool have1 = (y <= yl);
@@ -413,7 +413,7 @@
     loop_accumulate(err, k + 1, accB, gw);
 }
 
-template <typename T, bool NT, bool STRICT>
+template <typename T, bool NT, bool STRICT, bool PZ>
 __global__ OFX_ITER2_BOUNDS void k_tvl1_iter2(
     Tri<typename Pix<T>::v2> Ut, Tri<typename Pix<T>::v2> P1t, Tri<typename Pix<T>::v2> P2t,
     const typename Pix<T>::v2 *__restrict__ Ag, const T *__restrict__ Rg, double *__restrict__ errg, int k, int nx, int ny,
@@ -457,20 +457,20 @@
     double up12 = 0.0, up22 = 0.0;
     RowIn<T> cur;
     if (!idle) {
-        if (ys > 0) {
+        if (!PZ && ys > 0) {
             up12 = ldw2(at(P1in, off - row2)).y;
             up22 = ldw2(at(P2in, off - row2)).y;
         }
-        cur = tvl1_load_row<T>(Uin, P1in, P2in, A, R, off);
+        cur = tvl1_load_row<T, PZ>(Uin, P1in, P2in, A, R, off);
     }
     double e1;
     if (!tvl1_continues(prev1, prev2, k, nx * ny, eps2, e1)) return;
     if (idle) return;
     if (((amask >> g) & 1u) || tvl1_store_a(k, e1, eps2, afac))
-        tvl1_iter2_march<T, NT, true, STRICT>(Uin, P1in, P2in, A, R, hu.out, h1.out, h2.out, hu.alt, h1.alt, h2.alt, err, k, gw, nx, ny,
+        tvl1_iter2_march<T, NT, true, STRICT, PZ>(Uin, P1in, P2in, A, R, hu.out, h1.out, h2.out, hu.alt, h1.alt, h2.alt, err, k, gw, nx, ny,
                                       y0, yend, ys, yl, lef, rig, owner, off, so, up12, up22, cur, l_t, theta, taut);
     else
-        tvl1_iter2_march<T, NT, false, STRICT>(Uin, P1in, P2in, A, R, hu.out, h1.out, h2.out, hu.alt, h1.alt, h2.alt, err, k, gw, nx, ny,
+        tvl1_iter2_march<T, NT, false, STRICT, PZ>(Uin, P1in, P2in, A, R, hu.out, h1.out, h2.out, hu.alt, h1.alt, h2.alt, err, k, gw, nx, ny,
                                        y0, yend, ys, yl, lef, rig, owner, off, so, up12, up22, cur, l_t, theta, taut);
 }
 
@@ -481,7 +481,7 @@
 #ifndef OFX_ITER3_WAVES
 #define OFX_ITER3_WAVES 3
 #endif
-template <typename T, bool NT, bool STRICT, int CNT>
+template <typename T, bool NT, bool STRICT, int CNT, bool PZ>
 OFX_DEV void tvl1_iter3_march(const typename Pix<T>::v2 *__restrict__ Uin, const typename Pix<T>::v2 *__restrict__ P1in,
                               const typename Pix<T>::v2 *__restrict__ P2in, const typename Pix<T>::v2 *__restrict__ A,
                               const T *__restrict__ R, typename Pix<T>::v2 *Uout, typename Pix<T>::v2 *P1out,
@@ -517,9 +517,9 @@
     auto step = [&](const int y) {
         RowIn<T> nxt = cur;
 #ifdef OFX_CEIL_ALU
-        if (y + 1 <= ylc) nxt = tvl1_load_row<T>(Uin, P1in, P2in, A, R, off0 + ((y & 1) ? row2 : 0u));
+        if (y + 1 <= ylc) nxt = tvl1_load_row<T, PZ>(Uin, P1in, P2in, A, R, off0 + ((y & 1) ? row2 : 0u));
 #else
-        if (y + 1 <= ylc) nxt = tvl1_load_row<T>(Uin, P1in, P2in, A, R, off + row2);
+        if (y + 1 <= ylc) nxt = tvl1_load_row<T, PZ>(Uin, P1in, P2in, A, R, off + row2);
 #endif
         unsigned stu = OFX_OOB, stp = OFX_OOB;
         double2 su = z2, sp1 = z2, sp2 = z2;
@@ -608,7 +608,7 @@
     if (CNT == 3) loop_accumulate(err, slot0 + 2 * slot_step, accC, gw);
 }
 
-template <typename T, bool NT, bool STRICT>
+template <typename T, bool NT, bool STRICT, bool PZ>
 __global__ __launch_bounds__(256) __attribute__((amdgpu_waves_per_eu(OFX_ITER3_WAVES, OFX_ITER3_WAVES))) void k_tvl1_iter3(
     Tri<typename Pix<T>::v2> Ut, Tri<typename Pix<T>::v2> P1t, Tri<typename Pix<T>::v2> P2t,
     const typename Pix<T>::v2 *__restrict__ Ag, const T *__restrict__ Rg, double *__restrict__ errg, int k0, int check, int slot0,
@@ -659,11 +659,11 @@
     double up12 = 0.0, up22 = 0.0;
     RowIn<T> cur;
     if (!idle) {
-        if (ys > 0) {
+        if (!PZ && ys > 0) {
             up12 = ldw2(at(P1in, off - row2)).y;
             up22 = ldw2(at(P2in, off - row2)).y;
         }
-        cur = tvl1_load_row<T>(Uin, P1in, P2in, A, R, off);
+        cur = tvl1_load_row<T, PZ>(Uin, P1in, P2in, A, R, off);
     }
     if (check) {
         double e1 = 0.0;
@@ -684,13 +684,13 @@
     if (idle) return;
     const int step = check ? 1 : 0;
     if (niter >= 3)
-        tvl1_iter3_march<T, NT, STRICT, 3>(Uin, P1in, P2in, A, R, hu.out, h1.out, h2.out, err, slot0, step, gw, nx, ny, y0, yend, ys, yl,
+        tvl1_iter3_march<T, NT, STRICT, 3, PZ>(Uin, P1in, P2in, A, R, hu.out, h1.out, h2.out, err, slot0, step, gw, nx, ny, y0, yend, ys, yl,
                                            lef, rig, owner, off, so, up12, up22, cur, l_t, theta, taut);
     else if (niter == 2)
-        tvl1_iter3_march<T, NT, STRICT, 2>(Uin, P1in, P2in, A, R, hu.out, h1.out, h2.out, err, slot0, step, gw, nx, ny, y0, yend, ys, yl,
+        tvl1_iter3_march<T, NT, STRICT, 2, PZ>(Uin, P1in, P2in, A, R, hu.out, h1.out, h2.out, err, slot0, step, gw, nx, ny, y0, yend, ys, yl,
                                            lef, rig, owner, off, so, up12, up22, cur, l_t, theta, taut);
     else
-        tvl1_iter3_march<T, NT, STRICT, 1>(Uin, P1in, P2in, A, R, hu.out, h1.out, h2.out, err, slot0, step, gw, nx, ny, y0, yend, ys, yl,
+        tvl1_iter3_march<T, NT, STRICT, 1, PZ>(Uin, P1in, P2in, A, R, hu.out, h1.out, h2.out, err, slot0, step, gw, nx, ny, y0, yend, ys, yl,
                                            lef, rig, owner, off, so, up12, up22, cur, l_t, theta, taut);
 }
 
@@ -893,6 +893,134 @@
     stn(Rg + goff + p, (I1w - I1wx * u.x - I1wy * u.y - ldw(I0g + goff + p)));
 }
 
+template <typename T, typename Ld>
+OFX_DEV void tvl1_sample3_image(const Ld &ld, const unsigned (&rr)[6], const unsigned (&cc)[6], double fx, double fy, double &o0,
+                                double &o1, double &o2)
+{
+    double prev[4], cur[6], nxt[6];
+    double c0[4], c1[4], c2[4];
+#pragma unroll
+    for (int m = 0; m < 4; m++) prev[m] = ld(rr[m + 1], cc[0]);
+#pragma unroll
+    for (int m = 0; m < 6; m++) cur[m] = ld(rr[m], cc[1]);
+#pragma unroll
+    for (int k = 0; k < 4; k++) {
+#pragma unroll
+        for (int m = 1; m < 5; m++) nxt[m] = ld(rr[m], cc[k + 2]);
+        nxt[0] = nxt[5] = 0.0;
+        if (k < 3) { nxt[0] = ld(rr[0], cc[k + 2]); nxt[5] = ld(rr[5], cc[k + 2]); }
+        double gx[4], gy[4];
+#pragma unroll
+        for (int m = 0; m < 4; m++) {
+            gx[m] = rnd_to<T>(0.5 * (nxt[m + 1] - prev[m]));
+            gy[m] = rnd_to<T>(0.5 * (cur[m + 2] - cur[m]));
+        }
+        c0[k] = cubic_cell(cur[1], cur[2], cur[3], cur[4], fy);
+        c1[k] = cubic_cell(gx[0], gx[1], gx[2], gx[3], fy);
+        c2[k] = cubic_cell(gy[0], gy[1], gy[2], gy[3], fy);
+#pragma unroll
+        for (int m = 0; m < 4; m++) prev[m] = cur[m + 1];
+#pragma unroll
+        for (int m = 0; m < 6; m++) cur[m] = nxt[m];
+    }
+    o0 = cubic_cell(c0[0], c0[1], c0[2], c0[3], fx);
+    o1 = cubic_cell(c1[0], c1[1], c1[2], c1[3], fx);
+    o2 = cubic_cell(c2[0], c2[1], c2[2], c2[3], fx);
+}
+
+template <typename T>
+__global__ __launch_bounds__(WARP_NT) WARP_ATTR void k_tvl1_warp_img(
+    const T *__restrict__ I1g, const T *__restrict__ I0g, Tri<typename Pix<T>::v2> Ut, typename Pix<T>::v2 *__restrict__ Ag,
+    T *__restrict__ Rg, int nx, int ny, unsigned curcode, unsigned *__restrict__ fallbacks)
+{
+    __shared__ double2 s_a[WARP_TH * WARP_TW];
+    __shared__ double s_b[WARP_TH * WARP_TW];
+    __shared__ int s_box[WARP_NW][4];
+    const int tid = threadIdx.y * 32 + threadIdx.x, wave = tid >> 6;
+    const int j = blockIdx.x * 32 + threadIdx.x;
+    const int i = blockIdx.y * WARP_BY + threadIdx.y;
+    const bool inside = (j < nx) && (i < ny);
+    const int g = blockIdx.z;
+    const size_t goff = (size_t) g * nx * ny;
+    const T *__restrict__ I1 = I1g + goff;
+    const typename Pix<T>::v2 *__restrict__ U = pick3(Ut, curcode, g, (size_t) nx * ny).in;
+    const size_t p = (size_t) (inside ? i : 0) * nx + (inside ? j : 0);
+    double2 u = make_double2(0.0, 0.0);
+    BicubicTaps t;
+    t.out = true;
+    if (inside) {
+        u = ldw2(U + p);
+        t = bicubic_taps(j + u.x, i + u.y, nx, ny);
+    }
+    const bool need = inside && !t.out;
+    int xlo = need ? t.col[0] : 0x7fffffff, xhi = need ? t.col[3] : -1;
+    int ylo = need ? t.row[0] : 0x7fffffff, yhi = need ? t.row[3] : -1;
+#pragma unroll
+    for (int m = 32; m >= 1; m >>= 1) {
+        xlo = min(xlo, __shfl_xor(xlo, m, 64)); xhi = max(xhi, __shfl_xor(xhi, m, 64));
+        ylo = min(ylo, __shfl_xor(ylo, m, 64)); yhi = max(yhi, __shfl_xor(yhi, m, 64));
+    }
+    if ((tid & 63) == 0) { s_box[wave][0] = xlo; s_box[wave][1] = xhi; s_box[wave][2] = ylo; s_box[wave][3] = yhi; }
+    __syncthreads();
+#pragma unroll
+    for (int w = 0; w < WARP_NW; w++) {
+        xlo = min(xlo, s_box[w][0]); xhi = max(xhi, s_box[w][1]);
+        ylo = min(ylo, s_box[w][2]); yhi = max(yhi, s_box[w][3]);
+    }
+    const int W = xhi - xlo + 1, H = yhi - ylo + 1;
+    const bool any = (xhi >= 0);
+    const bool tile = any && W <= WARP_TW && H <= WARP_TH;
+    if (tile) {
+        for (int k = tid; k < W * H; k += WARP_NT) {
+            const int r = k / W, c = k - r * W;
+            const int y = ylo + r, x = xlo + c;
+            const int xl = x > 0 ? x - 1 : 0, xr = x < nx - 1 ? x + 1 : nx - 1;
+            const int yu = y > 0 ? y - 1 : 0, yd = y < ny - 1 ? y + 1 : ny - 1;
+            const T *row = I1 + (size_t) y * nx;
+            const double gx = rnd_to<T>(0.5 * (ldw(row + xr) - ldw(row + xl)));
+            const double gy = rnd_to<T>(0.5 * (ldw(I1 + (size_t) yd * nx + x) - ldw(I1 + (size_t) yu * nx + x)));
+            s_a[r * WARP_TW + c] = make_double2(ldw(row + x), gx);
+            s_b[r * WARP_TW + c] = gy;
+        }
+        __syncthreads();
+    } else if (any && tid == 0) {
+        atomicAdd(fallbacks + g, 1u);
+    }
+    if (!inside) return;
+    double I1w = 0.0, I1wx = 0.0, I1wy = 0.0;
+    if (need) {
+        if (tile) {
+            const int cx = t.col[0] - xlo, cy = t.row[0] - ylo;
+            double c0[4], c1[4], c2[4];
+#pragma unroll
+            for (int k = 0; k < 4; k++) {
+                const int o = cy * WARP_TW + cx + k;
+                const double2 a0 = s_a[o], a1 = s_a[o + WARP_TW], a2 = s_a[o + 2 * WARP_TW], a3 = s_a[o + 3 * WARP_TW];
+                const double b0 = s_b[o], b1 = s_b[o + WARP_TW], b2 = s_b[o + 2 * WARP_TW], b3 = s_b[o + 3 * WARP_TW];
+                c0[k] = cubic_cell(a0.x, a1.x, a2.x, a3.x, t.fy);
+                c1[k] = cubic_cell(a0.y, a1.y, a2.y, a3.y, t.fy);
+                c2[k] = cubic_cell(b0, b1, b2, b3, t.fy);
+            }
+            I1w = cubic_cell(c0[0], c0[1], c0[2], c0[3], t.fx);
+            I1wx = cubic_cell(c1[0], c1[1], c1[2], c1[3], t.fx);
+            I1wy = cubic_cell(c2[0], c2[1], c2[2], c2[3], t.fx);
+        } else {
+            unsigned rr[6], cc[6];
+#pragma unroll
+            for (int m = 0; m < 4; m++) { rr[m + 1] = (unsigned) t.row[m] * (unsigned) nx; cc[m + 1] = (unsigned) t.col[m]; }
+            rr[0] = (unsigned) (t.row[0] > 0 ? t.row[0] - 1 : 0) * (unsigned) nx;
+            rr[5] = (unsigned) (t.row[3] < ny - 1 ? t.row[3] + 1 : ny - 1) * (unsigned) nx;
+            cc[0] = (unsigned) (t.col[0] > 0 ? t.col[0] - 1 : 0);
+            cc[5] = (unsigned) (t.col[3] < nx - 1 ? t.col[3] + 1 : nx - 1);
+            tvl1_sample3_image<T>([&](unsigned ro, unsigned c) { return ldw(I1 + (ro + c)); }, rr, cc, t.fx, t.fy, I1w, I1wx, I1wy);
+        }
+        I1wx = rnd_to<T>(I1wx);
+        I1wy = rnd_to<T>(I1wy);
+    }
+    stn2(Ag + goff + p, make_double2(I1wx, I1wy));
+    stn(Rg + goff + p, (I1w - I1wx * u.x - I1wy * u.y - ldw(I0g + goff + p)));
+}
+
 template <typename T>
 __global__ void k_tvl1_zoom_in_g(Tri<typename Pix<T>::v2> Ut, unsigned curcode, typename Pix<T>::v2 *__restrict__ Uout, int nx,
                                  int ny, int nxx, int nyy, double fx, double fy, double scale)
@@ -957,6 +1085,8 @@
     bool fixed;
 };
 
+static bool tvl1_warp_from_image(const ofx_ctx *ctx) { return ctx->warp_image && ctx->warp_lds; }
+
 template <typename T> static int tvl1_level_alloc(ofx_ctx *ctx, Tvl1Level<T> &L, int nx, int ny, int G, bool images)
 {
     const size_t n = (size_t) nx * ny * G;
@@ -970,8 +1100,12 @@
         OFX_TRY(ofx_alloc(ctx, n, &L.I0));
         OFX_TRY(ofx_alloc(ctx, n, &L.I1));
     }
-    OFX_TRY(ofx_alloc(ctx, n, &L.pa));
-    OFX_TRY(ofx_alloc(ctx, n, &L.pb));
+    L.pa = nullptr;
+    L.pb = nullptr;
+    if (!tvl1_warp_from_image(ctx)) {
+        OFX_TRY(ofx_alloc(ctx, n, &L.pa));
+        OFX_TRY(ofx_alloc(ctx, n, &L.pb));
+    }
     for (int h = 0; h < 3; h++) {
         OFX_TRY(ofx_alloc(ctx, n, &L.U[h]));
         OFX_TRY(ofx_alloc(ctx, n, &L.P1[h]));
@@ -1044,7 +1178,7 @@
                                     double *err_out, float *ms_out, int *alt_out);
 template <typename T>
 static int tvl1_run_iterations_tri(ofx_ctx *ctx, Tvl1Level<T> &L, const Tvl1Params &P, LoopSpec S, int *n_out, double *err_out,
-                                   float *ms_out, int *alt_out);
+                                   float *ms_out, int *alt_out, bool p_zero);
 
 static int tvl1_pick_rows3(const ofx_ctx *ctx, int nx, int ny, int G)
 {
@@ -1086,10 +1220,16 @@
     return best;
 }
 
+static bool tvl1_takes_zero_duals(const ofx_ctx *ctx, int nx, int ny, int G)
+{
+    return ctx->implicit_zero_duals && tvl1_pick_tile(ctx, nx, ny, G) == 0;
+}
+
 template <typename T>
 static int tvl1_run_iterations(ofx_ctx *ctx, Tvl1Level<T> &L, const Tvl1Params &P, int *n_out, double *err_out,
                                float *ms_out, int *alt_out = nullptr,
-                               int *unit_out = nullptr)
+                               int *unit_out = nullptr,
+                               bool p_zero = false)
 {
     const int nx = L.nx, ny = L.ny, G = L.G;
     if ((long long) nx * ny >= (1LL << 27)) return ofx_fail(ctx, OFX_ERR_ARG, "tvl1: image larger than 2^27 pixels");
@@ -1112,7 +1252,10 @@
     S.pairs = pairs;
     const int tileK = tvl1_pick_tile(ctx, nx, ny, G);
     if (unit_out) *unit_out = tileK ? tileK : (pairs ? 2 : 1);
-    if (tileK) return tvl1_run_iterations_tile<T>(ctx, L, P, S, tileK, n_out, err_out, ms_out, alt_out);
+    if (tileK) {
+        if (p_zero) return ofx_fail(ctx, OFX_ERR_ARG, "tvl1: the tile kernel reads its duals");
+        return tvl1_run_iterations_tile<T>(ctx, L, P, S, tileK, n_out, err_out, ms_out, alt_out);
+    }
     {
         const bool strict_mode = sizeof(T) == sizeof(double) && !ctx->relaxed_dual;
         const double px = (double) nx * ny * G;
@@ -1121,11 +1264,12 @@
                                             px >= (ctx->fuse3_min_px > 0 ? ctx->fuse3_min_px : 5e5));
         if (pairs && tri) {
             if (unit_out) *unit_out = 3;
-            return tvl1_run_iterations_tri<T>(ctx, L, P, S, n_out, err_out, ms_out, alt_out);
+            return tvl1_run_iterations_tri<T>(ctx, L, P, S, n_out, err_out, ms_out, alt_out, p_zero);
         }
     }
     const int err_stride = (S.max_iter + 1) * OFX_NSHARD;
     const unsigned all = (G >= 32) ? 0xFFFFFFFFu : ((1u << G) - 1u);
+    const unsigned pz0 = p_zero ? all : 0u;
     const bool nt_stores = ctx->nt_stores ? ctx->nt_stores == 1 : (double) nx * ny * G * 15.0 * sizeof(T) > 300e6;
     unsigned b0[OFX_MAX_GROUP];
     for (int g = 0; g < G; g++) b0[g] = L.curidx(g);
@@ -1141,22 +1285,33 @@
         for (int g = 0; g < G; g++)
             if (ctx->store_a == 2 || (L.last_n[g] >= 1 && L.last_n[g] <= 2)) amask0 |= 1u << g;
     const bool strict = sizeof(T) == sizeof(double) && !ctx->relaxed_dual;
-    auto single = [&](unsigned incode, unsigned runmask, int check, int slot, double thr) -> int {
-        auto kern = k_tvl1_iter<T, false>;
-        if constexpr (sizeof(T) == sizeof(double)) { if (strict) kern = k_tvl1_iter<T, true>; }
-        hipLaunchKernelGGL(kern, dim3(gx1, G), block, 0, ctx->stream, L.Ut(), L.P1t(), L.P2t(), L.A, (const T *) L.R,
-                           ctx->d_err, check, slot, nx, ny, rows, strips_x, strips_pad, l_t, theta, taut, thr, incode, runmask,
-                           err_stride);
-        OFX_LAUNCH_CHECK(ctx);
+    auto single = [&](unsigned incode, unsigned runmask, int check, int slot, double thr, unsigned pzero) -> int {
+        for (int z = 0; z < 2; z++) {
+            const unsigned mask = z ? (runmask & pzero) : (runmask & ~pzero);
+            if (!mask) continue;
+            auto kern = z ? k_tvl1_iter<T, false, true> : k_tvl1_iter<T, false, false>;
+            if constexpr (sizeof(T) == sizeof(double)) {
+                if (strict) kern = z ? k_tvl1_iter<T, true, true> : k_tvl1_iter<T, true, false>;
+            }
+            hipLaunchKernelGGL(kern, dim3(gx1, G), block, 0, ctx->stream, L.Ut(), L.P1t(), L.P2t(), L.A, (const T *) L.R,
+                               ctx->d_err, check, slot, nx, ny, rows, strips_x, strips_pad, l_t, theta, taut, thr, incode, mask,
+                               err_stride);
+            OFX_LAUNCH_CHECK(ctx);
+        }
         return OFX_OK;
     };
     auto launch = [&](int k, int cnt, double thr) -> int {
         const unsigned incode = code_of((unsigned) (pairs ? k / 2 : k));
-        if (cnt == 1) return single(incode, all, k, k, thr);
+        const bool pz = k == 0 && p_zero;
+        if (cnt == 1) return single(incode, all, k, k, thr, pz ? all : 0u);
         const unsigned amask = k == 0 ? amask0 : 0u;
-        auto kern = nt_stores ? k_tvl1_iter2<T, true, false> : k_tvl1_iter2<T, false, false>;
+        auto kern = nt_stores ? k_tvl1_iter2<T, true, false, false> : k_tvl1_iter2<T, false, false, false>;
+        if (pz) kern = nt_stores ? k_tvl1_iter2<T, true, false, true> : k_tvl1_iter2<T, false, false, true>;
         if constexpr (sizeof(T) == sizeof(double)) {
-            if (strict) kern = nt_stores ? k_tvl1_iter2<T, true, true> : k_tvl1_iter2<T, false, true>;
+            if (strict) {
+                kern = nt_stores ? k_tvl1_iter2<T, true, true, false> : k_tvl1_iter2<T, false, true, false>;
+                if (pz) kern = nt_stores ? k_tvl1_iter2<T, true, true, true> : k_tvl1_iter2<T, false, true, true>;
+            }
         }
         hipLaunchKernelGGL(kern, grid2, block, 0, ctx->stream, L.Ut(), L.P1t(), L.P2t(), L.A, (const T *) L.R, ctx->d_err, k, nx,
                            ny, rows2, strips2_x, strips2_pad, l_t, theta, taut, thr, incode, amask, S.afac, err_stride);
@@ -1164,13 +1319,14 @@
         return OFX_OK;
     };
     auto redo = [&](const int *k_of) -> int {
-        unsigned incode = 0, runmask = 0;
+        unsigned incode = 0, runmask = 0, pzero = 0;
         for (int g = 0; g < G; g++) {
             if (k_of[g] < 0) continue;
             runmask |= 1u << g;
             incode |= ((b0[g] + (unsigned) (k_of[g] / 2)) % 3u) << (2 * g);
-        }
-        return single(incode, runmask, 0, S.max_iter, -1.0);
+            if (k_of[g] / 2 == 0) pzero |= pz0 & (1u << g);
+        }
+        return single(incode, runmask, 0, S.max_iter, -1.0, pzero);
     };
     int took_alt[OFX_MAX_GROUP];
     OFX_TRY(ofx_run_loop_group(ctx, S, G, launch, redo, n_out, err_out, ms_out, amask0, took_alt));
@@ -1251,7 +1407,7 @@
 
 template <typename T>
 static int tvl1_run_iterations_tri(ofx_ctx *ctx, Tvl1Level<T> &L, const Tvl1Params &P, LoopSpec S, int *n_out, double *err_out,
-                                   float *ms_out, int *alt_out)
+                                   float *ms_out, int *alt_out, bool p_zero)
 {
     const int nx = L.nx, ny = L.ny, G = L.G;
     const double l_t = P.lambda * P.theta, taut = P.tau / P.theta, theta = P.theta;
@@ -1265,20 +1421,29 @@
     S.afac = 0.0;
     const int err_stride = (S.max_iter + 1) * OFX_NSHARD;
     const unsigned all = (G >= 32) ? 0xFFFFFFFFu : ((1u << G) - 1u);
+    const unsigned pz0 = p_zero ? all : 0u;
     unsigned b0[OFX_MAX_GROUP];
     for (int g = 0; g < G; g++) b0[g] = L.curidx(g);
     const bool cursor = ctx->fuse3_cursor != 0 && !S.fixed;
     const double afac2 = ctx->fuse3_afac2 > 0 ? ctx->fuse3_afac2 : 1.5, afac1 = ctx->fuse3_afac1 > 0 ? ctx->fuse3_afac1 : 1.2;
     auto go = [&](int k0, int check, int slot0, double thr, unsigned incode, unsigned runmask, unsigned long long nit, OfxLoopDev *dev,
-                  int launch) -> int {
-        auto kern = nt_stores ? k_tvl1_iter3<T, true, false> : k_tvl1_iter3<T, false, false>;
-        if constexpr (sizeof(T) == sizeof(double)) {
-            if (strict) kern = nt_stores ? k_tvl1_iter3<T, true, true> : k_tvl1_iter3<T, false, true>;
-        }
-        hipLaunchKernelGGL(kern, grid, block, 0, ctx->stream, L.Ut(), L.P1t(), L.P2t(), L.A, (const T *) L.R, ctx->d_err, k0, check,
-                           slot0, nx, ny, rows, strips_x, strips_pad, l_t, theta, taut, thr, incode, runmask, nit, err_stride, dev, launch,
-                           afac1, afac2, S.max_iter);
-        OFX_LAUNCH_CHECK(ctx);
+                  int launch, unsigned pzero) -> int {
+        for (int z = 0; z < 2; z++) {
+            const unsigned mask = z ? (runmask & pzero) : (runmask & ~pzero);
+            if (!mask) continue;
+            auto kern = nt_stores ? k_tvl1_iter3<T, true, false, false> : k_tvl1_iter3<T, false, false, false>;
+            if (z) kern = nt_stores ? k_tvl1_iter3<T, true, false, true> : k_tvl1_iter3<T, false, false, true>;
+            if constexpr (sizeof(T) == sizeof(double)) {
+                if (strict) {
+                    kern = nt_stores ? k_tvl1_iter3<T, true, true, false> : k_tvl1_iter3<T, false, true, false>;
+                    if (z) kern = nt_stores ? k_tvl1_iter3<T, true, true, true> : k_tvl1_iter3<T, false, true, true>;
+                }
+            }
+            hipLaunchKernelGGL(kern, grid, block, 0, ctx->stream, L.Ut(), L.P1t(), L.P2t(), L.A, (const T *) L.R, ctx->d_err, k0, check,
+                               slot0, nx, ny, rows, strips_x, strips_pad, l_t, theta, taut, thr, incode, mask, nit, err_stride, dev, launch,
+                               afac1, afac2, S.max_iter);
+            OFX_LAUNCH_CHECK(ctx);
+        }
         return OFX_OK;
     };
     auto code_of_unit = [&](unsigned unit) -> unsigned {
@@ -1290,18 +1455,20 @@
     int inside[OFX_MAX_GROUP];
     if (cursor) {
         auto launch = [&](int Lidx, double thr) -> int {
-            return go(0, 1, 0, thr, code_of_unit((unsigned) Lidx), all, 0ull, reinterpret_cast<OfxLoopDev *>(ctx->d_state), Lidx);
+            return go(0, 1, 0, thr, code_of_unit((unsigned) Lidx), all, 0ull, reinterpret_cast<OfxLoopDev *>(ctx->d_state), Lidx,
+                      Lidx == 0 ? pz0 : 0u);
         };
         auto redo = [&](const int *n_of, const int *k0_of, const int *u_of) -> int {
-            unsigned incode = 0, runmask = 0;
+            unsigned incode = 0, runmask = 0, pzero = 0;
             unsigned long long nit = 0;
             for (int g = 0; g < G; g++) {
                 if (n_of[g] < 0) continue;
                 runmask |= 1u << g;
                 incode |= ((b0[g] + (unsigned) u_of[g]) % 3u) << (2 * g);
                 nit |= (unsigned long long) (n_of[g] - k0_of[g]) << (4 * g);
+                if (u_of[g] == 0) pzero |= pz0 & (1u << g);
             }
-            return go(0, 0, S.max_iter, -1.0, incode, runmask, nit, nullptr, 0);
+            return go(0, 0, S.max_iter, -1.0, incode, runmask, nit, nullptr, 0, pzero);
         };
         const int upc = (S.chunk + 2) / 3 < 1 ? 1 : (S.chunk + 2) / 3;
         OFX_TRY(ofx_run_loop_cursor(ctx, S, G, upc, 3, launch, redo, n_out, err_out, unit_of, inside, ms_out));
@@ -1309,10 +1476,10 @@
         auto launch = [&](int k, int cnt, double thr) -> int {
             unsigned long long nit = 0;
             for (int g = 0; g < G; g++) nit |= (unsigned long long) cnt << (4 * g);
-            return go(k, 1, k, thr, code_of_unit((unsigned) (k / 3)), all, nit, nullptr, 0);
+            return go(k, 1, k, thr, code_of_unit((unsigned) (k / 3)), all, nit, nullptr, 0, k == 0 ? pz0 : 0u);
         };
         auto redo = [&](const int *k_of) -> int {
-            unsigned incode = 0, runmask = 0;
+            unsigned incode = 0, runmask = 0, pzero = 0;
             unsigned long long nit = 0;
             for (int g = 0; g < G; g++) {
                 if (k_of[g] < 0) continue;
@@ -1320,8 +1487,9 @@
                 runmask |= 1u << g;
                 incode |= ((b0[g] + (unsigned) j) % 3u) << (2 * g);
                 nit |= (unsigned long long) (n - j * 3) << (4 * g);
+                if (j == 0) pzero |= pz0 & (1u << g);
             }
-            return go(0, 0, S.max_iter, -1.0, incode, runmask, nit, nullptr, 0);
+            return go(0, 0, S.max_iter, -1.0, incode, runmask, nit, nullptr, 0, pzero);
         };
         int took_alt[OFX_MAX_GROUP];
         OFX_TRY(ofx_run_loop_group(ctx, S, G, launch, redo, n_out, err_out, ms_out, 0u, took_alt));
@@ -1349,8 +1517,10 @@
     const dim3 g2(ofx_cdiv(nx, OFX_WARP_BX), ofx_cdiv(ny, OFX_WARP_BY), G), b2(OFX_WARP_BX, OFX_WARP_BY);
     if (nx < 2 || ny < 2) return ofx_fail(ctx, OFX_ERR_ARG, "tvl1: level %dx%d too small", nx, ny);
 
-    OFX_TRY(op_grad_pack<T>(ctx, L.I1, L.pa, L.pb, nx, ny, G));
-    for (int h = 0; h < 3; h++) {
+    const bool from_image = tvl1_warp_from_image(ctx);
+    if (!from_image) OFX_TRY(op_grad_pack<T>(ctx, L.I1, L.pa, L.pb, nx, ny, G));
+    const bool p_zero = tvl1_takes_zero_duals(ctx, nx, ny, G);
+    for (int h = 0; h < 3 && !p_zero; h++) {
         bool used = false;
         for (int g = 0; g < G; g++) used = used || (L.curidx(g) == (unsigned) h);
         if (!used) continue;
@@ -1360,7 +1530,10 @@
     for (int g = 0; g < G; g++) L.last_n[g] = 0;
 
     for (int w = 0; w < P.warps; w++) {
-        if (ctx->warp_lds)
+        if (from_image)
+            hipLaunchKernelGGL(k_tvl1_warp_img<T>, dim3(ofx_cdiv(nx, 32), ofx_cdiv(ny, WARP_BY), G), dim3(32, WARP_BY), 0, ctx->stream,
+                               (const T *) L.I1, (const T *) L.I0, L.Ut(), L.A, L.R, nx, ny, L.cur, ctx->d_warp_fb);
+        else if (ctx->warp_lds)
             hipLaunchKernelGGL(k_tvl1_warp_lds<T>, dim3(ofx_cdiv(nx, 32), ofx_cdiv(ny, WARP_BY), G), dim3(32, WARP_BY), 0, ctx->stream, L.pa,
                                (const T *) L.pb, (const T *) L.I0, L.Ut(), L.A, L.R, nx, ny, L.cur);
         else
@@ -1371,7 +1544,7 @@
         double error[OFX_MAX_GROUP];
         float ms = 0.f;
         int odd[OFX_MAX_GROUP], unit = 0;
-        OFX_TRY(tvl1_run_iterations<T>(ctx, L, P, it, error, ctx->profile ? &ms : nullptr, odd, &unit));
+        OFX_TRY(tvl1_run_iterations<T>(ctx, L, P, it, error, ctx->profile ? &ms : nullptr, odd, &unit, p_zero && w == 0));
         if (P.verbose && G == 1) fprintf(stderr, "Warping: %d, Iterations: %d, Error: %f\n", w, it[0], error[0]);
         for (int g = 0; g < G; g++) {
             ofx_stats &S = stats[g];
@@ -1396,6 +1569,21 @@
     st->nsolves = nsolves;
 }
 
+static int tvl1_fallbacks_begin(ofx_ctx *ctx)
+{
+    if (ctx->profile) OFX_HIP(ctx, hipMemsetAsync(ctx->d_warp_fb, 0, sizeof(unsigned) * OFX_MAX_GROUP, ctx->stream));
+    return OFX_OK;
+}
+static int tvl1_fallbacks_end(ofx_ctx *ctx, int G, ofx_stats *stats)
+{
+    if (!ctx->profile) return OFX_OK;
+    unsigned h[OFX_MAX_GROUP];
+    OFX_HIP(ctx, hipMemcpyAsync(h, ctx->d_warp_fb, sizeof(unsigned) * OFX_MAX_GROUP, hipMemcpyDeviceToHost, ctx->stream));
+    OFX_HIP(ctx, hipStreamSynchronize(ctx->stream));
+    for (int g = 0; g < G; g++) stats[g].warp_fallbacks = h[g];
+    return OFX_OK;
+}
+
 template <typename T>
 static int tvl1_multiscale_dev(ofx_ctx *ctx, int G, const T *const *dI0, const T *const *dI1, int nxx, int nyy,
                                const Tvl1Params &P, int nscales, double zfactor, std::vector<Tvl1Level<T>> &lv,
@@ -1425,6 +1613,7 @@
     }
     Tvl1Level<T> &C = lv[nscales - 1];
     OFX_TRY(op_fill2<T>(ctx, C.U[0], C.n() * G));
+    OFX_TRY(tvl1_fallbacks_begin(ctx));
 
     for (int s = nscales - 1; s >= 0; s--) {
         if (P.verbose && G == 1) fprintf(stderr, "Scale %d: %dx%d\n", s, lv[s].nx, lv[s].ny);
@@ -1439,7 +1628,7 @@
             OFX_LAUNCH_CHECK(ctx);
         }
     }
-    return OFX_OK;
+    return tvl1_fallbacks_end(ctx, G, stats);
 }
 
 static Tvl1Params make_params(const ofx_ctx *ctx, double tau, double lambda, double theta, int warps,
@@ -1637,7 +1826,9 @@
     OFX_HIP(ctx, hipMemcpyAsync(d1, u1, n * sizeof(double), hipMemcpyHostToDevice, ctx->stream));
     OFX_HIP(ctx, hipMemcpyAsync(d2, u2, n * sizeof(double), hipMemcpyHostToDevice, ctx->stream));
     OFX_TRY(op_interleave2<T>(ctx, d1, d2, L.U[0], n));
+    OFX_TRY(tvl1_fallbacks_begin(ctx));
     OFX_TRY(tvl1_single_scale_dev<T>(ctx, L, P, 0, &ctx->stats));
+    OFX_TRY(tvl1_fallbacks_end(ctx, 1, &ctx->stats));
     OFX_TRY(op_deinterleave2<T>(ctx, L.Ucur(0), d1, d2, n));
     OFX_HIP(ctx, hipMemcpyAsync(u1, d1, n * sizeof(double), hipMemcpyDeviceToHost, ctx->stream));
     OFX_HIP(ctx, hipMemcpyAsync(u2, d2, n * sizeof(double), hipMemcpyDeviceToHost, ctx->stream));
```

New measurement: 79640 Mpix*warp-iters/s, median of 6. 1.1% higher.
